# yosungho/LineTR

Measured on AMD Instinct MI355X. Metric: line_descriptors_per_sec, higher is better.
Workload: dtype f32 in/out; GEMMs as 6 bf16-split MFMA products, fp32 accumulate (fp32-faithful); 1 GPU; cfg3: 64 pairs/GPU of 640x480, 200 lines/image -> 199 sub-lines x 21 tokens, d_model=256, seeded weights; pairs_per_gpu=64, collective=none

## Files before the change

### include/linetr_hip.h

```cpp
#ifndef LINETR_HIP_H
#define LINETR_HIP_H

#include <stdint.h>

#ifdef __cplusplus
extern "C" {
#endif

#define LINETR_ABI_VERSION 6

enum {
  LINETR_OK = 0,
  LINETR_E_ARG = -1,
  LINETR_E_HIP = -2,
  LINETR_E_WEIGHTS = -3,
  LINETR_E_ASSERT = -4,
  LINETR_E_WORKSPACE = -5,
  LINETR_E_CAPACITY = -6
};

typedef struct LinetrHandle LinetrHandle;

typedef struct {
  int32_t d_model;
// ... 256 lines not shown
                                int32_t Kin, float* d_dW, float* d_db, void* d_workspace, int64_t workspace_bytes, void* stream);

int64_t linetr_token_assemble_backward_workspace_bytes(int64_t L);
int linetr_token_assemble_forward(LinetrHandle* h, const float* d_desc, const float* d_pos, const float* d_cls, int64_t L, int32_t S,
                                  float* d_x, void* stream);
int linetr_token_assemble_backward(LinetrHandle* h, const float* d_dx, int64_t L, int32_t S, float* d_dtok, float* d_dcls,
                                   void* d_workspace, int64_t workspace_bytes, void* stream);


enum { LINETR_COORD_F32 = 0, LINETR_COORD_F64 = 1 };
int64_t linetr_gt_assign_workspace_bytes(int32_t B, int32_t n0, int32_t n1);
int linetr_gt_assign(LinetrHandle* h, int32_t coord_type, const void* d_lines0, int32_t n0, const void* d_lines1, int32_t n1,
                     const double* d_H, int32_t B, const int32_t* d_count0, const int32_t* d_count1, double thres_reprojected,
                     double thres_angdiff, double min_overlap_ratio, int32_t pad, float* d_assign, int32_t* d_lmatches, int32_t M,
                     int32_t* d_found, uint8_t* d_match_dir, void* d_overlap_dir, void* d_proj0, void* d_proj1, void* d_workspace,
                     int64_t workspace_bytes, void* stream);


int linetr_make_pseudo_lines(uint64_t seed, int32_t image_index, int32_t n, double shape0, double shape1, double min_length,
                             double* h_lines);

int linetr_find_line_attributes(const double* h_lines, int32_t n, double min_length, int32_t max_sublines, double* h_klines,
                                double* h_length, double* h_angles, int32_t* n_out);

int64_t linetr_fixed_size_workspace_bytes(int32_t n_images, int32_t height, int32_t width, int32_t dense_is_nhwc);
int linetr_fixed_size(LinetrHandle* h, const LinetrLineRec* d_recs, const int32_t* h_cu_k, const int32_t* h_cu_n,
                      const LinetrLineRec* d_pseudo, const LinetrLineRec* h_pseudo, const int32_t* h_cu_p, int32_t n_images,
                      int32_t max_sublines, int32_t max_tokens, double token_distance, const float* d_dense_desc,
                      const float* d_dense_score, int32_t height, int32_t width, int32_t clip_height, int32_t clip_width,
                      int32_t pseudo_clip_height, int32_t pseudo_clip_width, int32_t align_corners, int32_t dense_is_nhwc,
                      LinetrTokens out, int32_t* d_num_klns, int32_t* d_num_slns, void* d_workspace, int64_t workspace_bytes,
                      void* stream);


typedef struct {
  float* p;
  const float* g;
  float* m;
  float* v;
  int64_t n;
  float step_size;
  float bc2_sqrt;
} LinetrAdamTensor;
typedef struct {
  double beta1, beta2, eps, weight_decay, lr;
  int32_t decoupled;
} LinetrAdamHyper;

int64_t linetr_adam_workspace_bytes(int32_t n_tensors, int64_t n_total);
int linetr_adam_step(LinetrHandle* h, const LinetrAdamTensor* h_table, int32_t n_tensors, const LinetrAdamHyper* hyper,
                     const float* d_grad_scale, void* d_workspace, int64_t workspace_bytes, void* stream);

int64_t linetr_grad_norm_workspace_bytes(int32_t n_tensors, int64_t n_total);
int linetr_grad_norm(LinetrHandle* h, const LinetrAdamTensor* h_table, int32_t n_tensors, double max_norm, double* d_norm,
                     float* d_scale, void* d_workspace, int64_t workspace_bytes, void* stream);


int linetr_superpoint_heads(LinetrHandle* h, const float* d_score_logits, const float* d_desc_raw, int32_t B,
                            int32_t Hc, int32_t Wc, float* d_dense_score, float* d_dense_desc_nhwc,
                            float* d_dense_desc_nchw, void* stream);


int64_t linetr_superpoint_keypoints_workspace_bytes(int32_t B, int32_t H, int32_t W, int32_t cap_per_image);
int linetr_superpoint_keypoints(LinetrHandle* h, const float* d_dense_score, int32_t B, int32_t H, int32_t W, int32_t nms_radius,
                                float keypoint_threshold, int32_t remove_borders, int32_t max_keypoints, int32_t cap_per_image,
                                float* d_keypoints, float* d_scores, int32_t* d_cu_kp, int32_t* d_found, void* d_workspace,
                                int64_t workspace_bytes, void* stream);

int64_t linetr_point_descriptors_workspace_bytes(int32_t B, int32_t Hc, int32_t Wc, int32_t dense_is_nhwc);
int linetr_point_descriptors(LinetrHandle* h, const float* d_keypoints, const int32_t* d_cu_kp, int32_t B, int64_t n_total,
                             const float* d_dense_desc, int32_t Hc, int32_t Wc, int32_t align_corners, int32_t dense_is_nhwc,
                             float* d_desc_cn, void* d_workspace, int64_t workspace_bytes, void* stream);

int linetr_superpoint_heads_rows(LinetrHandle* h, const float* d_score_rows, int64_t ld_score, const float* d_desc_rows, int64_t ld_desc,
                                 int32_t B, int32_t Hc, int32_t Wc, float* d_dense_score, float* d_dense_desc_nhwc,
                                 float* d_dense_desc_nchw, void* stream);


int linetr_warp_images(LinetrHandle* h, const float* d_src, int32_t B, int32_t C, int32_t H, int32_t W, const double* h_mat, int32_t mode,
                       float* d_dst, uint8_t* d_valid, void* stream);
int linetr_warp_tile(int32_t* tile_h, int32_t* tile_w, int32_t* erode_tile_h, int32_t* erode_tile_w);

int linetr_mask_erode(LinetrHandle* h, const uint8_t* d_mask, int32_t B, int32_t H, int32_t W, int32_t radius, uint8_t* d_out, void* stream);


typedef struct LinetrDetectConfig {
  int32_t n_octaves;
  int32_t scale;
  int32_t grad_threshold;
  int32_t min_region_size;
  double density;
} LinetrDetectConfig;

int64_t linetr_detect_lines_workspace_bytes(int32_t B, int32_t H, int32_t W, int32_t n_octaves);
int linetr_detect_lines(LinetrHandle* h, const void* d_images, int32_t images_are_float, int32_t B, int32_t H, int32_t W,
                        const LinetrDetectConfig* cfg, int32_t capacity, double* d_rows, int32_t* h_counts, int64_t* d_debug_regions,
                        void* d_workspace, int64_t workspace_bytes, void* stream);
int linetr_detect_tile(int32_t* tile_h, int32_t* tile_w);

int64_t linetr_detect_debug_labels_workspace_bytes(int32_t B, int32_t H, int32_t W);
int linetr_detect_debug_labels(LinetrHandle* h, const int8_t* d_buckets, int32_t B, int32_t H, int32_t W, int32_t* d_labels, void* d_workspace,
                               int64_t workspace_bytes, void* stream);
int linetr_detect_debug_gradient(LinetrHandle* h, const void* d_images, int32_t images_are_float, int32_t B, int32_t H, int32_t W,
                                 const LinetrDetectConfig* cfg, int32_t octave, int32_t* d_m2, int8_t* d_bucket_a, int8_t* d_bucket_b,
                                 void* d_workspace, int64_t workspace_bytes, void* stream);


int linetr_sp_conv3x3_tile(int32_t* tile_h, int32_t* tile_w);
int64_t linetr_sp_conv3x3_pack_bytes(int32_t Cin, int32_t Cout);
int linetr_sp_conv3x3_pack(const float* d_w, int32_t Cin, int32_t Cout, float* d_packed, void* stream);
int linetr_sp_conv3x3(LinetrHandle* h, const float* d_x, int32_t B, int32_t H, int32_t W, int32_t Cin, const float* d_packed_w,
                      const float* d_bias, int32_t Cout, int32_t pool, float* d_y, void* stream);
int linetr_sp_conv1a(LinetrHandle* h, const float* d_image, int32_t B, int32_t H, int32_t W, const float* d_w, const float* d_bias,
                     float* d_y, void* stream);

#define LINETR_SP_SCORE_LD 68
typedef struct LinetrSpEncoder LinetrSpEncoder;
int linetr_sp_encoder_create(int32_t device, LinetrSpEncoder** out);
void linetr_sp_encoder_destroy(LinetrSpEncoder* enc);
int linetr_sp_encoder_set_weights(LinetrSpEncoder* enc, const float* const* d_weights, const float* const* d_biases, void* stream);
int64_t linetr_sp_encoder_workspace_bytes(int32_t B, int32_t H, int32_t W);
int linetr_sp_encoder_forward(LinetrSpEncoder* enc, const float* d_image, int32_t B, int32_t H, int32_t W, float* d_score_rows,
                              float* d_desc_rows, float* d_feat, void* d_workspace, int64_t workspace_bytes, void* stream);


enum { LINETR_PREC_F32 = 0, LINETR_PREC_BF16X3 = 1, LINETR_PREC_BF16X6 = 2, LINETR_PREC_F16X3 = 3 };
int linetr_set_precision(LinetrHandle* h, int32_t mode);
int linetr_get_precision(const LinetrHandle* h);


int linetr_debug_posenc(LinetrHandle* h, int32_t which, const float* d_in0, const float* d_in1, const float* d_in2,
                           int64_t rows, float* d_out, void* stream);

int linetr_debug_gemm(LinetrHandle* h, const float* d_A, int32_t lda, const float* d_W, const float* d_bias,
                      const float* d_residual, float* d_Y, int32_t ldy, int32_t M, int32_t N, int32_t K,
                      int32_t act, int32_t cache_weights, void* stream);

#define LINETR_GEMM_TILE_WS 100
typedef struct {
  const float* A;   int32_t lda;
  const float* A2;  int32_t lda2;  int32_t K1;
  const float* W;
  const float* bias;
  const float* R;
  float* Y;         int32_t ldy;
  int32_t M, N, K, act;
  int32_t groups;   int64_t gA, gY;
  int32_t norm;     const float* gamma;  const float* beta;  const float* add2;  float eps;
  int32_t via_row_norm;
  int32_t tile;
} LinetrGemmCase;
int linetr_debug_gemm_case(LinetrHandle* h, const LinetrGemmCase* c, int32_t* tile_used, void* stream);

int linetr_debug_sig_attention(LinetrHandle* h, int32_t kernel, int32_t layer, const float* d_in, int32_t ld_in,
                               const int32_t* h_cu_sub, int32_t n_images, float* d_msg, int32_t* kernel_used, void* stream);

int linetr_debug_tok_mlp(LinetrHandle* h, int32_t variant, const float* d_pnt, const float* d_score, int64_t rows_word,
                         const float* d_sublines, const float* d_resp, const float* d_angle, int64_t rows_line,
                         float* d_out_word, float* d_out_line, int32_t max_blocks, int32_t* variant_used, void* stream);

int64_t linetr_debug_bn_train_workspace_bytes(const LinetrHandle* h, int32_t which, int64_t rows);
int linetr_debug_bn_train(LinetrHandle* h, int32_t which, float* d_z, int64_t rows, int32_t C, int32_t ld, const float* d_gamma,
                          const float* d_beta, const float* d_in0, const float* d_in1, const float* d_in2, float* d_out,
                          float momentum, float* d_running, float* d_batch, float* d_affine, int32_t* nb_used, void* d_ws,
                          int64_t ws_bytes, void* stream);

int linetr_debug_cls_pool(LinetrHandle* h, int32_t kernel, const LinetrLineRec* d_recs, int32_t K, const int32_t* d_sub2line,
                          int32_t N, int32_t T, const float* d_cpnt, const float* d_a4, int64_t first_pad, int32_t n_images,
                          const float* d_map, int32_t dense_is_nhwc, int32_t Hc, int32_t Wc, int32_t align_corners,
                          const float* d_desc_dense, float* d_pooled, int32_t* kernel_used, void* stream);

int linetr_debug_match(LinetrHandle* h, int32_t P, const int32_t* dims, const float* d_desc0, const int64_t* off_n0,
                       const int32_t* d_s2l0, const float* d_desc1, const int64_t* off_n1, const int32_t* d_s2l1, float thr,
                       int32_t mutual, float* d_dk, const int64_t* off_dk, int32_t* d_match01, const int64_t* off_k0, void* d_ws,
                       int64_t ws_bytes, int32_t path, int32_t seg1_global, int32_t cache_dk, int32_t device_table,
                       int32_t* path_used, void* stream);

enum { LINETR_STAGE_TAIL = 0, LINETR_STAGE_SIG = 1, LINETR_STAGE_FOLD_NEXT = 8 };
int64_t linetr_debug_stage_workspace_bytes(const LinetrHandle* h, int32_t N, int32_t n_images);
int linetr_debug_stage(LinetrHandle* h, int32_t stage, int32_t N, const float* d_in0, const float* d_in1, const int32_t* h_cu_sub,
                       int32_t n_images, int32_t plan, float* d_out0, float* d_out1, float* d_out2, int32_t* plan_used, void* d_ws,
                       int64_t ws_bytes, void* stream);

#ifdef LINETR_EXPERIMENTS
int64_t linetr_st_bytes(int64_t rows, int32_t K);
int linetr_debug_to_st(LinetrHandle* h, const float* d_X, int32_t ld, int32_t rows, int32_t K, void* d_st, void* stream);
int linetr_debug_from_st(LinetrHandle* h, const void* d_st, int32_t rows, int32_t K, float* d_X, int32_t ld, void* stream);
int linetr_debug_gemm_st(LinetrHandle* h, const void* d_A1, int32_t K1, const void* d_A2, int32_t K2, const void* d_W,
                         const float* d_bias, const void* d_R, void* d_Yst, float* d_Y, int32_t ldy, int32_t M, int32_t N,
                         int32_t act, void* stream);
int linetr_debug_pairnet_stamps(LinetrHandle* h, unsigned long long* d_buf);
#endif

int linetr_allgather_desc(void* nccl_comm, const void* d_slab, void* d_out, int64_t slab_bytes, void* stream);

int linetr_set_allgather_fn(void* nccl_allgather_fn);

int linetr_pack_slab(const float* d_line_desc, int32_t N, const int32_t* d_cu_n, const int32_t* d_cu_k, int32_t n_images,
                     const int32_t* d_sub2line, int32_t n_images_cap, int32_t rows_cap, int32_t zero_tail, float* d_slab,
                     void* stream);


typedef struct {
  const char* name;
  int32_t calls;
  float ms;
  double flops;
  double bytes;
} LinetrProfileEntry;
int linetr_set_profiling(LinetrHandle* h, int32_t on);
int linetr_get_profile(LinetrHandle* h, LinetrProfileEntry* out, int32_t max_entries, int32_t* n_out);

#ifdef __cplusplus
}
#endif
#endif
```

### linetr_amd/_native.py

```python
from __future__ import annotations

import ctypes as C
import os

import numpy as np

_HERE = os.path.dirname(os.path.abspath(__file__))
LIB_PATH = os.path.join(_HERE, "csrc", "liblinetr_hip.so")
EXPERIMENTS_LIB_PATH = os.path.join(os.path.dirname(_HERE), "experiments", "liblinetr_hip_experiments.so")

E_ARG, E_ASSERT, E_WORKSPACE = -1, -4, -5


class ModelConfig(C.Structure):
    _fields_ = [("d_model", C.c_int32), ("n_heads", C.c_int32), ("d_inner", C.c_int32),
                ("n_sig_layers", C.c_int32), ("n_desc_layers", C.c_int32), ("enc_channels", C.c_int32 * 4),
                ("norm_height", C.c_int32), ("norm_width", C.c_int32), ("bn_batch_stats", C.c_int32)]


class LineRec(C.Structure):
    _fields_ = [("sp", C.c_double * 2), ("ep", C.c_double * 2), ("length", C.c_double),
                ("angle", C.c_double * 2), ("first_sub", C.c_int32), ("n_tok", C.c_int32),
                ("n_sub", C.c_int32), ("image", C.c_int32), ("line_local", C.c_int32), ("first_tok", C.c_int32)]

# ... 29 lines not shown
            raise ValueError(f"dropout seed {seed} / call {call}: a 64-bit seed and a 32-bit call index")
        return cls(int(seed), int(call), int(p * 4294967296.0), 1.0 / (1.0 - p))


ADAM_TENSOR_DTYPE = np.dtype([("p", "<u8"), ("g", "<u8"), ("m", "<u8"), ("v", "<u8"), ("n", "<i8"), ("step_size", "<f4"), ("bc2_sqrt", "<f4")])
assert ADAM_TENSOR_DTYPE.itemsize == 48


def adam_bias_corrections(lr: float, beta1: float, beta2: float, step: float):
    step = float(step)
    return float(lr) / (1.0 - float(beta1) ** step), (1.0 - float(beta2) ** step) ** 0.5


class AdamHyper(C.Structure):
    _fields_ = [("beta1", C.c_double), ("beta2", C.c_double), ("eps", C.c_double), ("weight_decay", C.c_double), ("lr", C.c_double),
                ("decoupled", C.c_int32)]


class DetectConfig(C.Structure):
    _fields_ = [("n_octaves", C.c_int32), ("scale", C.c_int32), ("grad_threshold", C.c_int32), ("min_region_size", C.c_int32),
                ("density", C.c_double)]


class ProfileEntry(C.Structure):
    _fields_ = [("name", C.c_char_p), ("calls", C.c_int32), ("ms", C.c_float), ("flops", C.c_double),
                ("bytes", C.c_double)]


vp, i32, i64, f64, f32 = C.c_void_p, C.c_int32, C.c_int64, C.c_double, C.c_float
_P = C.POINTER

ABI = {
    "linetr_abi_version": (i32, []),
    "linetr_last_error": (C.c_char_p, []),
    "linetr_create": (i32, [_P(ModelConfig), i32, _P(C.c_char_p), _P(vp), _P(i64), i32, _P(vp)]),
    "linetr_destroy": (None, [vp]),
    "linetr_prefilter": (i32, [vp, i32, i32, i32, i32, f64, i32, vp, f64, i32, i32, i32, i32, vp, i32, _P(i32), _P(i32)]),
    "linetr_prefilter_batch": (i32, [vp, vp, i32, i32, i32, i32, f64, i32, vp, f64, i32, i32, vp, i32, vp, vp]),
    "linetr_prefilter_tied_images": (i32, [vp, i32]),
    "linetr_pack_lines": (i32, [vp, vp, vp, i32, f64, i32, i32, i32, i32, vp, _P(i32)]),
    "linetr_tokenize_workspace_bytes": (i64, [i32, i32, i32, i32]),
    "linetr_tokenize": (i32, [vp, vp, i32, i32, f64, i32, vp, vp, i32, i32, i32, i32, i32, i32, i32, Tokens, vp, vp, i64, vp]),
    "linetr_sample_descriptors_workspace_bytes": (i64, [i32, i32, i32]),
    "linetr_sample_descriptors": (i32, [vp, vp, i64, vp, i32, i32, i32, i32, vp, vp, i64, vp]),
    "linetr_forward_workspace_bytes": (i64, [vp, i32, i32]),
    "linetr_forward": (i32, [vp, _P(Tokens), vp, vp, i32, i32, vp, vp, i64, vp]),
    "linetr_bn_stats_floats": (i64, [vp]),
    "linetr_forward_train_workspace_bytes": (i64, [vp, i32, i32]),
    "linetr_forward_train": (i32, [vp, _P(Tokens), vp, vp, i32, i32, f32, vp, vp, vp, vp, i64, vp]),
    "linetr_describe_workspace_bytes": (i64, [vp, i32, i32, i32, i32, i64]),
    "linetr_describe": (i32, [vp, vp, i32, i32, i64, vp, vp, i32, f64, i32, vp, vp, i32, i32, i32, i32, Tokens, vp, vp, vp, i64, vp]),
    "linetr_describe_submit": (i32, [vp, vp, i32, i32, i64, vp, vp, i32, f64, i32, vp, vp, i32, i32, i32, i32, Tokens, vp, vp, vp, i64, i32,
                                     i32, vp]),
    "linetr_pipeline_max_slots": (i32, []),
    "linetr_describe_join": (i32, [vp, i32, vp]),
    "linetr_match_workspace_bytes": (i64, [i32, i64, i64, i64]),
    "linetr_match": (i32, [vp, i32, vp, vp, vp, vp, vp, vp, vp, f32, i32, vp, vp, vp, vp, vp, i64, vp]),
    "linetr_match_gathered": (i32, [vp, i32, vp, vp, vp, vp, vp, vp, vp, vp, vp, f32, i32, vp, vp, vp, vp, vp, i64, vp]),
    "linetr_match_distmat_workspace_bytes": (i64, [i32, i32]),
    "linetr_match_distmat": (i32, [vp, vp, i32, i32, f32, i32, vp, vp, i64, vp]),
    "linetr_match_distmat_f64_workspace_bytes": (i64, [i32, i32]),
    "linetr_match_distmat_f64": (i32, [vp, vp, i32, i32, f64, i32, vp, vp, i64, vp]),
    "linetr_pool_distmat_workspace_bytes": (i64, [i32, i32]),
    "linetr_pool_distmat": (i32, [vp, vp, i32, i32, vp, i32, vp, i32, vp, vp, i64, vp]),
    "linetr_pool_distmat_dense_workspace_bytes": (i64, [i32, i32, i32, i32]),
    "linetr_pool_distmat_dense": (i32, [vp, vp, i32, i32, vp, i32, vp, i32, vp, vp, i64, vp]),
    "linetr_match_points_workspace_bytes": (i64, [i32, i32]),
    "linetr_match_points": (i32, [vp, vp, i32, vp, i32, f32, i32, vp, vp, vp, i64, vp]),
    "linetr_pair_tail_workspace_bytes": (i64, [i32, i32, i32, i32, i32, i32]),
    "linetr_pair_tail_output_bytes": (i64, [i32, i32, i32, i32, vp]),
    "linetr_pair_tail": (i32, [vp, vp, i32, vp, i32, f32, vp, i32, vp, i32, vp, i32, vp, i32, f32, i32, vp, i64, vp, i64, vp]),
    "linetr_val_step_workspace_bytes": (i64, [i32, i32]),
    "linetr_val_step_output_bytes": (i64, [i32, vp]),
    "linetr_val_step": (i32, [vp, vp, i32, vp, i32, vp, i32, f64, i32, vp, vp, vp, vp, i64, vp, i64, vp]),
    "linetr_assign_from_matches": (i32, [vp, vp, i32, i32, i32, vp, vp]),
    "linetr_desc_loss_grad_workspace_bytes": (i64, [i32, i32]),
    "linetr_desc_loss_grad": (i32, [vp, vp, i32, vp, i32, vp, i32, vp, vp, vp, vp, i64, vp, i64, vp]),
    "linetr_linear_backward_chunk_rows": (i32, []),
    "linetr_linear_backward_workspace_bytes": (i64, [i64, i32, i32]),
    "linetr_linear_forward": (i32, [vp, vp, i64, vp, vp, i64, i32, i32, i32, vp, i64, vp]),
    "linetr_linear_backward": (i32, [vp, vp, i64, vp, vp, i64, vp, i64, i32, i32, vp, vp, vp, vp, i64, vp]),
    "linetr_head_backward_workspace_bytes": (i64, [i64]),
    "linetr_head_forward": (i32, [vp, vp, vp, vp, i64, vp, vp]),
    "linetr_head_backward": (i32, [vp, vp, vp, vp, vp, i64, vp, vp, vp, vp, i64, vp]),
    "linetr_sig_attention_backward_workspace_bytes": (i64, [i64]),
    "linetr_sig_attention_forward": (i32, [vp, vp, i64, vp, i64, vp, i64, vp, i32, i64, vp, i64, vp, vp]),
    "linetr_sig_attention_backward": (i32, [vp, vp, i64, vp, i64, vp, i64, vp, i64, vp, vp, i64, vp, i32, i64, vp, i64, vp, i64, vp, i64, vp, i64,
                                            vp]),
    "linetr_bn_forward_workspace_bytes": (i64, [i64, i32]),
    "linetr_bn_forward": (i32, [vp, vp, i64, i64, i32, vp, vp, f32, f32, vp, i32, i32, vp, i64, vp, vp, i64, vp]),
    "linetr_bn_backward_workspace_bytes": (i64, [i64, i32]),
    "linetr_bn_backward": (i32, [vp, vp, i64, vp, i64, vp, i64, vp, vp, i64, i32, i32, vp, i64, vp, vp, vp, i64, vp]),
    "linetr_cls_pool_train_forward": (i32, [vp, vp, i64, vp, i64, i64, i32, vp, vp, vp]),
    "linetr_cls_pool_train_backward": (i32, [vp, vp, i64, vp, i64, vp, vp, vp, i64, i32, vp, i64, vp, i64, vp]),
    "linetr_layer_norm_backward_workspace_bytes": (i64, [i64, i32]),
    "linetr_layer_norm_forward": (i32, [vp, vp, i64, vp, i64, vp, vp, f32, i64, i32, vp, i64, vp, vp]),
    "linetr_layer_norm_backward": (i32, [vp, vp, i64, vp, i64, vp, vp, vp, i64, i64, i32, vp, i64, vp, vp, vp, i64, vp]),
    "linetr_cls_pool_dropout_forward": (i32, [vp, vp, i64, vp, i64, i64, i32, _P(Dropout), vp, vp, vp, vp]),
    "linetr_cls_pool_dropout_backward": (i32, [vp, vp, i64, vp, i64, vp, vp, vp, vp, vp, i64, i32, _P(Dropout), vp, i64, vp, i64, vp]),
    "linetr_layer_norm_dropout_forward": (i32, [vp, vp, i64, vp, i64, vp, vp, f32, i64, i32, _P(Dropout), i32, vp, i64, vp, vp]),
    "linetr_layer_norm_dropout_backward": (i32, [vp, vp, i64, vp, i64, vp, vp, vp, i64, i64, i32, _P(Dropout), i32, vp, i64, vp, i64, vp, vp, vp,
                                                 i64, vp]),
    "linetr_dropout_factors": (i32, [vp, _P(Dropout), i32, i64, i64, vp, vp]),
    "linetr_gelu_forward": (i32, [vp, vp, i64, i64, i32, vp, i64, vp]),
    "linetr_gelu_backward": (i32, [vp, vp, i64, vp, i64, i64, i32, vp, i64, vp]),
    "linetr_input_layer_chunk_rows": (i32, []),
    "linetr_input_layer_backward_workspace_bytes": (i64, [i64, i32, i32]),
    "linetr_input_layer_forward": (i32, [vp, vp, i64, vp, vp, i64, i32, i32, vp, i64, vp]),
    "linetr_input_layer_backward": (i32, [vp, vp, i64, vp, i64, i64, i32, i32, vp, vp, vp, i64, vp]),
    "linetr_token_assemble_backward_workspace_bytes": (i64, [i64]),
    "linetr_token_assemble_forward": (i32, [vp, vp, vp, vp, i64, i32, vp, vp]),
    "linetr_token_assemble_backward": (i32, [vp, vp, i64, i32, vp, vp, vp, i64, vp]),
    "linetr_gt_assign_workspace_bytes": (i64, [i32, i32, i32]),
    "linetr_gt_assign": (i32, [vp, i32, vp, i32, vp, i32, vp, i32, vp, vp, f64, f64, f64, i32, vp, vp, i32, vp, vp, vp, vp, vp, vp, i64, vp]),
    "linetr_make_pseudo_lines": (i32, [C.c_uint64, i32, i32, f64, f64, f64, vp]),
    "linetr_find_line_attributes": (i32, [vp, i32, f64, i32, vp, vp, vp, _P(i32)]),
    "linetr_fixed_size_workspace_bytes": (i64, [i32, i32, i32, i32]),
    "linetr_fixed_size": (i32, [vp, vp, vp, vp, vp, vp, vp, i32, i32, i32, f64, vp, vp, i32, i32, i32, i32, i32, i32, i32, i32, Tokens, vp, vp,
                                vp, i64, vp]),
    "linetr_adam_workspace_bytes": (i64, [i32, i64]),
    "linetr_adam_step": (i32, [vp, vp, i32, _P(AdamHyper), vp, vp, i64, vp]),
    "linetr_grad_norm_workspace_bytes": (i64, [i32, i64]),
    "linetr_grad_norm": (i32, [vp, vp, i32, f64, vp, vp, vp, i64, vp]),
    "linetr_superpoint_heads": (i32, [vp, vp, vp, i32, i32, i32, vp, vp, vp, vp]),
    "linetr_superpoint_keypoints_workspace_bytes": (i64, [i32, i32, i32, i32]),
    "linetr_superpoint_keypoints": (i32, [vp, vp, i32, i32, i32, i32, f32, i32, i32, i32, vp, vp, vp, vp, vp, i64, vp]),
    "linetr_point_descriptors_workspace_bytes": (i64, [i32, i32, i32, i32]),
    "linetr_point_descriptors": (i32, [vp, vp, vp, i32, i64, vp, i32, i32, i32, i32, vp, vp, i64, vp]),
    "linetr_superpoint_heads_rows": (i32, [vp, vp, i64, vp, i64, i32, i32, i32, vp, vp, vp, vp]),
    "linetr_warp_images": (i32, [vp, vp, i32, i32, i32, i32, vp, i32, vp, vp, vp]),
    "linetr_warp_tile": (i32, [_P(i32), _P(i32), _P(i32), _P(i32)]),
    "linetr_mask_erode": (i32, [vp, vp, i32, i32, i32, i32, vp, vp]),
    "linetr_detect_lines_workspace_bytes": (i64, [i32, i32, i32, i32]),
    "linetr_detect_lines": (i32, [vp, vp, i32, i32, i32, i32, _P(DetectConfig), i32, vp, vp, vp, vp, i64, vp]),
    "linetr_detect_tile": (i32, [_P(i32), _P(i32)]),
    "linetr_detect_debug_labels_workspace_bytes": (i64, [i32, i32, i32]),
    "linetr_detect_debug_labels": (i32, [vp, vp, i32, i32, i32, vp, vp, i64, vp]),
    "linetr_detect_debug_gradient": (i32, [vp, vp, i32, i32, i32, i32, _P(DetectConfig), i32, vp, vp, vp, vp, i64, vp]),
    "linetr_sp_conv3x3_tile": (i32, [_P(i32), _P(i32)]),
    "linetr_sp_conv3x3_pack_bytes": (i64, [i32, i32]),
    "linetr_sp_conv3x3_pack": (i32, [vp, i32, i32, vp, vp]),
    "linetr_sp_conv3x3": (i32, [vp, vp, i32, i32, i32, i32, vp, vp, i32, i32, vp, vp]),
    "linetr_sp_conv1a": (i32, [vp, vp, i32, i32, i32, vp, vp, vp, vp]),
    "linetr_sp_encoder_create": (i32, [i32, _P(vp)]),
    "linetr_sp_encoder_destroy": (None, [vp]),
    "linetr_sp_encoder_set_weights": (i32, [vp, _P(vp), _P(vp), vp]),
    "linetr_sp_encoder_workspace_bytes": (i64, [i32, i32, i32]),
    "linetr_sp_encoder_forward": (i32, [vp, vp, i32, i32, i32, vp, vp, vp, vp, i64, vp]),
    "linetr_set_precision": (i32, [vp, i32]),
    "linetr_get_precision": (i32, [vp]),
    "linetr_debug_posenc": (i32, [vp, i32, vp, vp, vp, i64, vp, vp]),
    "linetr_debug_gemm": (i32, [vp, vp, i32, vp, vp, vp, vp, i32, i32, i32, i32, i32, i32, vp]),
    "linetr_debug_gemm_case": (i32, [vp, _P(GemmCase), vp, vp]),
    "linetr_debug_sig_attention": (i32, [vp, i32, i32, vp, i32, vp, i32, vp, vp, vp]),
    "linetr_debug_tok_mlp": (i32, [vp, i32, vp, vp, i64, vp, vp, vp, i64, vp, vp, i32, vp, vp]),
    "linetr_debug_bn_train_workspace_bytes": (i64, [vp, i32, i64]),
    "linetr_debug_bn_train": (i32, [vp, i32, vp, i64, i32, i32, vp, vp, vp, vp, vp, vp, f32, vp, vp, vp, vp, vp, i64, vp]),
    "linetr_debug_cls_pool": (i32, [vp, i32, vp, i32, vp, i32, i32, vp, vp, i64, i32, vp, i32, i32, i32, i32, vp, vp, vp, vp]),
    "linetr_debug_match": (i32, [vp, i32, vp, vp, vp, vp, vp, vp, vp, f32, i32, vp, vp, vp, vp, vp, i64, i32, i32, i32, i32, vp, vp]),
    "linetr_debug_stage_workspace_bytes": (i64, [vp, i32, i32]),
    "linetr_debug_stage": (i32, [vp, i32, i32, vp, vp, vp, i32, i32, vp, vp, vp, vp, vp, i64, vp]),
    "linetr_allgather_desc": (i32, [vp, vp, vp, i64, vp]),
    "linetr_set_allgather_fn": (i32, [vp]),
    "linetr_pack_slab": (i32, [vp, i32, vp, vp, i32, vp, i32, i32, i32, vp, vp]),
    "linetr_set_profiling": (i32, [vp, i32]),
    "linetr_get_profile": (i32, [vp, _P(ProfileEntry), i32, _P(i32)]),
}
EXPERIMENT_ABI = {
    "linetr_st_bytes": (i64, [i64, i32]),
    "linetr_debug_to_st": (i32, [vp, vp, i32, i32, i32, vp, vp]),
    "linetr_debug_from_st": (i32, [vp, vp, i32, i32, vp, i32, vp]),
    "linetr_debug_gemm_st": (i32, [vp, vp, i32, vp, i32, vp, vp, vp, vp, vp, i32, i32, i32, i32, vp]),
    "linetr_debug_pairnet_stamps": (i32, [vp, vp]),
}
EXPORTS = list(ABI)
EXPERIMENT_EXPORTS = list(EXPERIMENT_ABI)

_libs = {}


def lib(path=None):
    import torch
    path = os.path.abspath(path or os.environ.get("LINETR_LIB", LIB_PATH))
    if path in _libs:
        return _libs[path]
    if not os.path.exists(path):
        raise RuntimeError(
            f"{path} is missing: the HIP extension has not been built (run `python -m linetr_amd.build`). "
            "linetr_amd has no CPU fallback.")
    L = C.CDLL(path)
    table = {**ABI, **EXPERIMENT_ABI} if hasattr(L, "linetr_debug_gemm_st") else ABI
    for name, (restype, argtypes) in table.items():
        fn = getattr(L, name)
        fn.restype, fn.argtypes = restype, argtypes
    if L.linetr_abi_version() != 6:
        raise RuntimeError("liblinetr_hip.so ABI version mismatch")
    _libs[path] = L
    return L


class NativeError(RuntimeError):
    pass


def check(code: int, L=None):
    if code == 0:
        return
    msg = (L if L is not None else lib()).linetr_last_error().decode("utf-8", "replace")
    if code == E_ASSERT:
        raise AssertionError(msg)
    raise NativeError(f"liblinetr_hip error {code}: {msg}")


def np_ptr(a: np.ndarray):
    return a.ctypes.data_as(C.c_void_p)
```

### linetr_amd/csrc/linetr_core.hip

```cpp
#include <dlfcn.h>

#include <algorithm>
#include <condition_variable>
#include <functional>
#include <numeric>
#include <thread>

#include "lt_handle.h"

using namespace lt;

namespace {

class WorkPool {
 public:
  static WorkPool& get() {
    static WorkPool* p = new WorkPool();
    return *p;
  }
  int size() const { return n_workers_ + 1; }
  void run(int n, const std::function<void(int)>& fn) {
    if (n <= 0) return;
    if (n == 1 || n_workers_ == 0) { for (int i = 0; i < n; ++i) fn(i); return; }
    std::lock_guard<std::mutex> region(region_);
// ... 18 lines not shown
  }
  void drain() {
    for (;;) {
      int i;
      const std::function<void(int)>* f;
      {
        std::lock_guard<std::mutex> lk(m_);
        if (!job_ || next_ >= n_jobs_) return;
        i = next_++;
        f = job_;
      }
      (*f)(i);
      std::lock_guard<std::mutex> lk(m_);
      if (--pending_ == 0) cv_done_.notify_all();
    }
  }
  void loop() {
    uint64_t seen = 0;
    for (;;) {
      {
        std::unique_lock<std::mutex> lk(m_);
        cv_work_.wait(lk, [&] { return gen_ != seen; });
        seen = gen_;
      }
      drain();
    }
  }
  std::mutex m_, region_;
  std::condition_variable cv_work_, cv_done_;
  const std::function<void(int)>* job_ = nullptr;
  int n_jobs_ = 0, next_ = 0, pending_ = 0, n_workers_ = 0;
  uint64_t gen_ = 0;
};


struct TensorMap {
  std::map<std::string, std::pair<const float*, int64_t>> t;
  const float* get(const std::string& k, int64_t numel, int& err) const {
    auto it = t.find(k);
    if (it == t.end() || it->second.first == nullptr) {
      err = fail(LINETR_E_WEIGHTS, "state_dict tensor '%s' missing", k.c_str());
      return nullptr;
    }
    if (it->second.second != numel) {
      err = fail(LINETR_E_WEIGHTS, "state_dict tensor '%s' has %lld elements, expected %lld", k.c_str(),
                 (long long)it->second.second, (long long)numel);
      return nullptr;
    }
    return it->second.first;
  }
};

struct Arena {
  std::vector<float> host;
  size_t put(const std::vector<double>& v) {
    size_t off = (host.size() + 63) / 64 * 64;
    host.resize(off + v.size());
    for (size_t i = 0; i < v.size(); ++i) host[off + i] = (float)v[i];
    return off;
  }
};

void fold_bn(const float* W, const float* b, const float* g, const float* beta, const float* mean,
             const float* var, int out, int in, std::vector<double>& Wf, std::vector<double>& bf) {
  Wf.resize((size_t)out * in);
  bf.resize(out);
  for (int o = 0; o < out; ++o) {
    const double s = (double)g[o] / std::sqrt((double)var[o] + 1e-5);
    for (int i = 0; i < in; ++i) Wf[(size_t)o * in + i] = (double)W[(size_t)o * in + i] * s;
    bf[o] = ((double)b[o] - (double)mean[o]) * s + (double)beta[o];
  }
}

std::vector<double> to_d(const float* p, size_t n) { return std::vector<double>(p, p + n); }

}


extern "C" int linetr_abi_version(void) { return LINETR_ABI_VERSION; }
extern "C" const char* linetr_last_error(void) { return g_err.c_str(); }

extern "C" int linetr_create(const LinetrModelConfig* cfg, int32_t n_tensors, const char* const* names,
                             const float* const* h_data, const int64_t* numel, int32_t device,
                             LinetrHandle** out) {
  if (!cfg || !out || !names || !h_data || !numel) return fail(LINETR_E_ARG, "null argument");
  if (cfg->d_model != D || cfg->n_heads != HEADS)
    return fail(LINETR_E_ARG, "only descriptor_dim=256 / n_heads=4 are supported");
  if (cfg->d_inner % 128 != 0 || cfg->n_sig_layers < 0 || cfg->n_desc_layers < 1)
    return fail(LINETR_E_ARG, "bad d_inner / layer counts");
  const int e0 = cfg->enc_channels[0], e1 = cfg->enc_channels[1], e2 = cfg->enc_channels[2], e3 = cfg->enc_channels[3];
  if (e0 != 32 || e1 % 64 || e2 % 64 || e3 % 64 || e3 != D)
    return fail(LINETR_E_ARG, "keyline_encoder must be [32, 64k, 64k, 256] (got %d,%d,%d,%d)", e0, e1, e2, e3);
  int ndev = 0;
  LT_HIP(hipGetDeviceCount(&ndev));
  if (ndev <= 0 || device >= ndev) return fail(LINETR_E_HIP, "no usable HIP device (count=%d)", ndev);
  LT_HIP(hipSetDevice(device));

  TensorMap tm;
  for (int i = 0; i < n_tensors; ++i) tm.t[names[i]] = {h_data[i], numel[i]};
  int err = 0;
  Arena ar;
  auto H = std::make_unique<LinetrHandle>();
  H->cfg = *cfg;
  H->device = device;
  struct Fix { const float** dst; size_t off; };
  std::vector<Fix> fix;
  auto place = [&](const float** dst, const std::vector<double>& v) { fix.push_back({dst, ar.put(v)}); };
  std::vector<GemmWSpec> gemm_w;
  auto place_w = [&](GemmW* dst, const std::vector<double>& W, const std::vector<double>& b, int rows, int K, bool st = false) {
    place(&dst->W, W);
    place(&dst->b, b);
    dst->rows = rows; dst->K = K;
    gemm_w.push_back({dst, st});
  };

  int bn_slot = 0;
  if (cfg->bn_batch_stats) {
    if (std::max(std::max(e0, e1), std::max(std::max(e2, e3), 2 * D)) > lt::BN_MAX_CHANNELS)
      return fail(LINETR_E_ARG, "create: a training-mode handle (bn_batch_stats = 1) takes keyline_encoder widths up to %d (got %d, %d, %d, %d)",
                  lt::BN_MAX_CHANNELS, e0, e1, e2, e3);
    H->bn_g.reserve(8 + cfg->n_sig_layers); H->bn_b.reserve(8 + cfg->n_sig_layers); H->bn_c.reserve(8 + cfg->n_sig_layers);
  }
  const int ch_w[6] = {3, e0, e1, e2, e3, D}, ch_l[6] = {5, e0, e1, e2, e3, D};
  std::vector<double> W5w, b5w;
  for (int enc = 0; enc < 2; ++enc) {
    const std::string pre = enc == 0 ? "klenc.word_position_enc.encoder." : "klenc.line_position_enc.encoder.";
    const int* ch = enc == 0 ? ch_w : ch_l;
    PosEncoder& E = H->enc[enc];
    GemmW* const Wdst[4] = {nullptr, &E.W2, &E.W3, &E.W4};
    for (int i = 0; i < 4; ++i) {
      const std::string c = pre + std::to_string(3 * i), bn = pre + std::to_string(3 * i + 1);
      const float* W = tm.get(c + ".weight", (int64_t)ch[i + 1] * ch[i], err);
      const float* b = tm.get(c + ".bias", ch[i + 1], err);
      const float* g = tm.get(bn + ".weight", ch[i + 1], err);
      const float* be = tm.get(bn + ".bias", ch[i + 1], err);
      const float* mu = tm.get(bn + ".running_mean", ch[i + 1], err);
      const float* va = tm.get(bn + ".running_var", ch[i + 1], err);
      if (err) return err;
      std::vector<double> Wf, bf;
      if (cfg->bn_batch_stats) {
        Wf = to_d(W, (size_t)ch[i + 1] * ch[i]); bf = to_d(b, ch[i + 1]);
        H->bn_g.push_back(nullptr); H->bn_b.push_back(nullptr); H->bn_c.push_back(ch[i + 1]);
        place(&H->bn_g[bn_slot], to_d(g, ch[i + 1])); place(&H->bn_b[bn_slot], to_d(be, ch[i + 1]));
        ++bn_slot;
      } else
      fold_bn(W, b, g, be, mu, va, ch[i + 1], ch[i], Wf, bf);
      if (i == 0) { place(&E.W1, Wf); place(&E.b1, bf); }
      else place_w(Wdst[i], Wf, bf, ch[i + 1], ch[i], true);
    }
    const float* W = tm.get(pre + "12.weight", (int64_t)D * e3, err);
    const float* b = tm.get(pre + "12.bias", D, err);
    if (err) return err;
    if (enc == 0) { W5w = to_d(W, (size_t)D * D); b5w = to_d(b, D); }
    else place_w(&H->lW5, to_d(W, (size_t)D * D), to_d(b, D), D, e3);
  }

  {
    const std::string p = "klenc.desc_layers." + std::to_string(cfg->n_desc_layers - 1) + ".";
    const float* cls = tm.get("klenc.cls_token", D, err);
    const float* Wq = tm.get(p + "slf_attn.w_qs.weight", D * D, err);
    const float* bq = tm.get(p + "slf_attn.w_qs.bias", D, err);
    const float* Wk = tm.get(p + "slf_attn.w_ks.weight", D * D, err);
    const float* bk = tm.get(p + "slf_attn.w_ks.bias", D, err);
    const float* Wv = tm.get(p + "slf_attn.w_vs.weight", D * D, err);
    const float* bv = tm.get(p + "slf_attn.w_vs.bias", D, err);
    const float* Wfc = tm.get(p + "slf_attn.fc.weight", D * D, err);
    const float* bfc = tm.get(p + "slf_attn.fc.bias", D, err);
    const float* g1 = tm.get(p + "slf_attn.layer_norm.weight", D, err);
    const float* b1 = tm.get(p + "slf_attn.layer_norm.bias", D, err);
    const int DI = cfg->d_inner;
    const float* W1 = tm.get(p + "pos_ffn.w_1.weight", (int64_t)DI * D, err);
    const float* bb1 = tm.get(p + "pos_ffn.w_1.bias", DI, err);
    const float* W2 = tm.get(p + "pos_ffn.w_2.weight", (int64_t)D * DI, err);
    const float* bb2 = tm.get(p + "pos_ffn.w_2.bias", D, err);
    const float* g2 = tm.get(p + "pos_ffn.layer_norm.weight", D, err);
    const float* b2 = tm.get(p + "pos_ffn.layer_norm.bias", D, err);
    if (err) return err;
    std::vector<double> q(D);
    for (int o = 0; o < D; ++o) {
      double s = bq[o];
      for (int i = 0; i < D; ++i) s += (double)Wq[o * D + i] * cls[i];
      q[o] = s / 8.0;
    }
    std::vector<double> U(HEADS * D, 0.0), U2(HEADS * D, 0.0);
    for (int h = 0; h < HEADS; ++h) {
      double c = 0.0;
      for (int d = 0; d < DH; ++d) {
        const int o = h * DH + d;
        c += q[o] * bk[o];
        for (int i = 0; i < D; ++i) U[h * D + i] += q[o] * Wk[o * D + i];
      }
      for (int i = 0; i < D; ++i) {
        double s = 0.0;
        for (int o = 0; o < D; ++o) s += W5w[(size_t)o * D + i] * U[h * D + o];
        U2[h * D + i] = s;
      }
      double ub5 = 0.0, ucls = 0.0;
      for (int i = 0; i < D; ++i) { ub5 += U[h * D + i] * b5w[i]; ucls += U[h * D + i] * cls[i]; }
      H->pool.c_tok[h] = (float)(ub5 + c);
      H->pool.s_cls[h] = (float)(ucls + c);
    }
    place(&H->pool.U, U);
    place(&H->pool.U2, U2);
    std::vector<double> Watt((size_t)HEADS * DH * POOLW, 0.0), batt(HEADS * DH);
    for (int h = 0; h < HEADS; ++h)
      for (int d = 0; d < DH; ++d) {
        const int o = h * DH + d;
        double* row = &Watt[((size_t)h * DH + d) * POOLW];
        double r = 0.0, bb = bv[o];
        for (int i = 0; i < D; ++i) {
          row[i] = Wv[o * D + i];
          r += (double)Wv[o * D + i] * ((double)cls[i] - b5w[i]);
          bb += (double)Wv[o * D + i] * b5w[i];
        }
        for (int i = 0; i < D; ++i) {
          double s = 0.0;
          for (int m = 0; m < D; ++m) s += (double)Wv[o * D + m] * W5w[(size_t)m * D + i];
          row[D + i] = s;
        }
        row[2 * D] = r;
        batt[o] = bb;
      }
    place_w(&H->Watt, Watt, batt, HEADS * DH, POOLW);
    std::vector<double> bfc2(D);
    for (int i = 0; i < D; ++i) bfc2[i] = (double)bfc[i] + cls[i];
    place_w(&H->Wfc, to_d(Wfc, D * D), bfc2, D, D);
    place(&H->ln1g, to_d(g1, D)); place(&H->ln1b, to_d(b1, D));
    place_w(&H->Wf1, to_d(W1, (size_t)DI * D), to_d(bb1, DI), DI, D);
    place_w(&H->Wf2, to_d(W2, (size_t)D * DI), to_d(bb2, D), D, DI);
    place(&H->ln2g, to_d(g2, D)); place(&H->ln2b, to_d(b2, D));
  }

  H->sig.resize(cfg->n_sig_layers);
  std::vector<std::vector<double>> sig_qkv_d, sig_bqkv_d, sig_w2_d, sig_b2_d;
  for (int l = 0; l < cfg->n_sig_layers; ++l) {
    const std::string p = "selfattn.layers." + std::to_string(l) + ".";
    const float* Wp[3];
    const float* bp[3];
    for (int j = 0; j < 3; ++j) {
      Wp[j] = tm.get(p + "attn.proj." + std::to_string(j) + ".weight", D * D, err);
      bp[j] = tm.get(p + "attn.proj." + std::to_string(j) + ".bias", D, err);
    }
    const float* Wm = tm.get(p + "attn.merge.weight", D * D, err);
    const float* bm = tm.get(p + "attn.merge.bias", D, err);
    const float* W1 = tm.get(p + "mlp.0.weight", 4 * D * D, err);
    const float* b1 = tm.get(p + "mlp.0.bias", 2 * D, err);
    const float* g = tm.get(p + "mlp.1.weight", 2 * D, err);
    const float* be = tm.get(p + "mlp.1.bias", 2 * D, err);
    const float* mu = tm.get(p + "mlp.1.running_mean", 2 * D, err);
    const float* va = tm.get(p + "mlp.1.running_var", 2 * D, err);
    const float* W2 = tm.get(p + "mlp.3.weight", 2 * D * D, err);
    const float* b2 = tm.get(p + "mlp.3.bias", D, err);
    if (err) return err;
    std::vector<double> Wqkv((size_t)3 * D * D), bqkv(3 * D);
    for (int j = 0; j < 3; ++j)
      for (int h = 0; h < HEADS; ++h)
        for (int d = 0; d < DH; ++d) {
          const int src = d * HEADS + h, dst = j * D + h * DH + d;
          const double sc = j == 0 ? 0.125 : 1.0;
          for (int i = 0; i < D; ++i) Wqkv[(size_t)dst * D + i] = (double)Wp[j][src * D + i] * sc;
          bqkv[dst] = (double)bp[j][src] * sc;
        }
    std::vector<double> Wm2((size_t)D * D);
    for (int o = 0; o < D; ++o)
      for (int h = 0; h < HEADS; ++h)
        for (int d = 0; d < DH; ++d) Wm2[(size_t)o * D + h * DH + d] = Wm[o * D + d * HEADS + h];
    std::vector<double> W1f, b1f;
    if (cfg->bn_batch_stats) {
      W1f = to_d(W1, (size_t)4 * D * D); b1f = to_d(b1, 2 * D);
      H->bn_g.push_back(nullptr); H->bn_b.push_back(nullptr); H->bn_c.push_back(2 * D);
      place(&H->bn_g[bn_slot], to_d(g, 2 * D)); place(&H->bn_b[bn_slot], to_d(be, 2 * D));
      ++bn_slot;
    } else
    fold_bn(W1, b1, g, be, mu, va, 2 * D, 2 * D, W1f, b1f);
    std::vector<double> W1m((size_t)2 * D * 2 * D);
    for (int o = 0; o < 2 * D; ++o) {
      const double* w1b = &W1f[(size_t)o * 2 * D + D];
      for (int i = 0; i < D; ++i) W1m[(size_t)o * 2 * D + i] = W1f[(size_t)o * 2 * D + i];
      for (int i = 0; i < D; ++i) {
        double sacc = 0.0;
        for (int m = 0; m < D; ++m) sacc += w1b[m] * Wm2[(size_t)m * D + i];
        W1m[(size_t)o * 2 * D + D + i] = sacc;
      }
      double bacc = b1f[o];
      for (int m = 0; m < D; ++m) bacc += w1b[m] * (double)bm[m];
      b1f[o] = bacc;
    }
    SigLayer& S = H->sig[l];
    sig_qkv_d.push_back(Wqkv); sig_bqkv_d.push_back(bqkv);
    sig_w2_d.push_back(to_d(W2, (size_t)2 * D * D)); sig_b2_d.push_back(to_d(b2, D));
    place_w(&S.Wqkv, Wqkv, bqkv, 3 * D, D, true);
    place_w(&S.W1, W1m, b1f, 2 * D, 2 * D);
    place_w(&S.W2, to_d(W2, (size_t)2 * D * D), to_d(b2, D), D, 2 * D);
  }
  for (int l = 0; l + 1 < cfg->n_sig_layers; ++l) {
    const std::vector<double>&W2 = sig_w2_d[l], &b2 = sig_b2_d[l], &Wq = sig_qkv_d[l + 1], &bq = sig_bqkv_d[l + 1];
    std::vector<double> Wn((size_t)4 * D * 3 * D, 0.0), bn(4 * D);
    for (int o = 0; o < D; ++o) {
      Wn[(size_t)o * 3 * D + o] = 1.0;
      for (int j = 0; j < 2 * D; ++j) Wn[(size_t)o * 3 * D + D + j] = W2[(size_t)o * 2 * D + j];
      bn[o] = b2[o];
    }
    for (int r = 0; r < 3 * D; ++r) {
      double* row = &Wn[(size_t)(D + r) * 3 * D];
      const double* wq = &Wq[(size_t)r * D];
      for (int i = 0; i < D; ++i) row[i] = wq[i];
      double bacc = bq[r];
      for (int m2 = 0; m2 < D; ++m2) {
        const double a = wq[m2];
        const double* w2r = &W2[(size_t)m2 * 2 * D];
        for (int j = 0; j < 2 * D; ++j) row[D + j] += a * w2r[j];
        bacc += a * b2[m2];
      }
      bn[D + r] = bacc;
    }
    place_w(&H->sig[l].Wnext, Wn, bn, 4 * D, 3 * D);
  }
  {
    const float* W = tm.get("final_proj.weight", D * D, err);
    const float* b = tm.get("final_proj.bias", D, err);
    if (err) return err;
    place_w(&H->Wfin, to_d(W, D * D), to_d(b, D), D, D);
    if (cfg->n_sig_layers > 0) {
      const std::string p = "selfattn.layers." + std::to_string(cfg->n_sig_layers - 1) + ".";
      const float* W2 = tm.get(p + "mlp.3.weight", 2 * D * D, err);
      const float* b2 = tm.get(p + "mlp.3.bias", D, err);
      if (err) return err;
      std::vector<double> Wf((size_t)D * 3 * D), bf(D);
      for (int o = 0; o < D; ++o) {
        for (int i = 0; i < D; ++i) Wf[(size_t)o * 3 * D + i] = W[o * D + i];
        for (int j = 0; j < 2 * D; ++j) {
          double sacc = 0.0;
          for (int m = 0; m < D; ++m) sacc += (double)W[o * D + m] * (double)W2[(size_t)m * 2 * D + j];
          Wf[(size_t)o * 3 * D + D + j] = sacc;
        }
        double bacc = b[o];
        for (int m = 0; m < D; ++m) bacc += (double)W[o * D + m] * (double)b2[m];
        bf[o] = bacc;
      }
      place_w(&H->Wfin2, Wf, bf, D, 3 * D);
    }
  }

  LT_HIP(hipMalloc((void**)&H->arena, ar.host.size() * sizeof(float)));
  LT_HIP(hipMemcpy(H->arena, ar.host.data(), ar.host.size() * sizeof(float), hipMemcpyHostToDevice));
  for (auto& f : fix) *f.dst = H->arena + f.off;
  if (int e = make_split_copies(H.get(), gemm_w)) return e;
  if (const char* e = getenv("LINETR_PRECISION")) {
    if (!strcmp(e, "f32")) H->precision = LINETR_PREC_F32;
    else if (!strcmp(e, "bf16x3")) H->precision = LINETR_PREC_BF16X3;
    else if (!strcmp(e, "bf16x6")) H->precision = LINETR_PREC_BF16X6;
    else if (!strcmp(e, "f16x3")) H->precision = LINETR_PREC_F16X3;
    else return fail(LINETR_E_ARG, "LINETR_PRECISION must be f32, bf16x3, bf16x6 or f16x3 (got '%s')", e);
  }
  *out = H.release();
  return LINETR_OK;
}

extern "C" int linetr_set_precision(LinetrHandle* h, int32_t mode) {
  if (!h || mode < LINETR_PREC_F32 || mode > LINETR_PREC_F16X3) return fail(LINETR_E_ARG, "bad precision mode");
  h->precision = mode;
  return LINETR_OK;
}
extern "C" int linetr_get_precision(const LinetrHandle* h) { return h ? h->precision : LINETR_E_ARG; }

extern "C" void linetr_destroy(LinetrHandle* h) {
  if (!h) return;
  (void)hipSetDevice(h->device);
  for (auto& p : h->pending) { (void)hipEventDestroy(p.a); (void)hipEventDestroy(p.b); }
  for (auto e : h->event_pool) (void)hipEventDestroy(e);
  for (hipStream_t x : h->pipe.stream)
    if (x) { (void)hipStreamSynchronize(x); (void)hipStreamDestroy(x); }
  for (int s = 0; s < LinetrHandle::PIPE_SLOTS; ++s) {
    for (hipEvent_t e : {h->pipe.fork[s], h->pipe.done[s]})
      if (e) (void)hipEventDestroy(e);
    for (hipEvent_t e : h->pipe.cut[s])
      if (e) (void)hipEventDestroy(e);
  }
  if (h->arena) (void)hipFree(h->arena);
  if (h->split_arena) (void)hipFree(h->split_arena);
  if (h->zeros) (void)hipFree(h->zeros);
  if (h->w2p_arena) (void)hipFree(h->w2p_arena);
  if (h->sk_ws) (void)hipFree(h->sk_ws);
  if (h->sk_flags) (void)hipFree(h->sk_flags);
  if (h->pn_abort) (void)hipHostFree(h->pn_abort);
  for (auto& kv : h->debug_split) (void)hipFree(kv.second);
  delete h;
}


static int pack_one(LinetrLineRec& r, double td, int T, int image, int line_local, int& sub_cursor, int& tok_cursor) {
  if (!(td > 0) || T < 1) return fail(LINETR_E_ARG, "token_distance must be > 0 and max_tokens >= 1");
  const double nt = std::ceil(r.length / td);
  if (!(nt >= 1) || nt > 1e7) return fail(LINETR_E_ARG, "key-line %d has a non-positive / absurd token count", line_local);
  r.n_tok = (int)nt;
  r.n_sub = (r.n_tok + T - 1) / T;
  r.first_sub = sub_cursor;
  r.image = image;
  r.line_local = line_local;
  r.first_tok = tok_cursor;
  sub_cursor += r.n_sub;
  tok_cursor += r.n_tok;
  if (r.n_tok >= 2) {
    const double dx = r.ep[0] - r.sp[0], dy = r.ep[1] - r.sp[1];
    const double geo = std::sqrt(dx * dx + dy * dy);
    if (!(geo >= (double)(r.n_tok - 2) * td))
      return fail(LINETR_E_ASSERT, "distance should be smaller than line length! (key-line %d)", line_local);
  }
  return 0;
}

static void angle_of(LinetrLineRec& r) {
  double th = std::atan2(r.ep[0] - r.sp[0], r.ep[1] - r.sp[1]);
  if (th < 0) th += M_PI;
#ifdef __GLIBC__
  ::sincos(2 * th, &r.angle[1], &r.angle[0]);
#else
  r.angle[0] = std::cos(2 * th);
  r.angle[1] = std::sin(2 * th);
#endif
}

extern "C" int linetr_pack_lines(const double* h_klines, const double* h_length, const double* h_angles, int32_t K,
                                 double td, int32_t T, int32_t image_index, int32_t sub_base, int32_t tok_base,
                                 LinetrLineRec* h_recs, int32_t* n_out) {
  if (K < 0 || (K > 0 && (!h_klines || !h_length || !h_angles || !h_recs))) return fail(LINETR_E_ARG, "null argument");
  int cur = sub_base, tcur = tok_base;
  for (int k = 0; k < K; ++k) {
    LinetrLineRec& r = h_recs[k];
    r.sp[0] = h_klines[k * 4 + 0]; r.sp[1] = h_klines[k * 4 + 1];
    r.ep[0] = h_klines[k * 4 + 2]; r.ep[1] = h_klines[k * 4 + 3];
    r.length = h_length[k];
    r.angle[0] = h_angles[k * 2]; r.angle[1] = h_angles[k * 2 + 1];
    if (int e = pack_one(r, td, T, image_index, k, cur, tcur)) return e;
  }
  if (n_out) *n_out = cur - sub_base;
  return LINETR_OK;
}


struct KeptLineAttr { double sp[2], ep[2], length; };
static double philox_u01(uint32_t hi, uint32_t lo) { return ((double)(hi >> 5) * 67108864.0 + (double)(lo >> 6)) / 9007199254740992.0; }

extern "C" int linetr_make_pseudo_lines(uint64_t seed, int32_t image_index, int32_t n, double shape0, double shape1, double min_length,
                                        double* h_lines) {
#pragma clang fp contract(off)
  constexpr double MASK = 15.0, MAX_RAND = 160.0;
  constexpr int MAX_ATTEMPTS = 64;
  if (n < 0 || (n > 0 && !h_lines) || image_index < 0 || seed >> 32) return fail(LINETR_E_ARG, "make_pseudo_lines: bad argument (a 32-bit seed, n >= 0)");
  if (!(min_length > 0) || !(min_length < MAX_RAND) || !(shape0 - MASK >= MASK + 2 * min_length) || !(shape1 - MASK >= MASK + 2 * min_length))
    return fail(LINETR_E_ARG, "make_pseudo_lines: image_shape (%g, %g) has no room for lines of min_length %g", shape0, shape1, min_length);
  const double area0 = shape0 - min_length - MASK, area1 = shape1 - min_length - MASK;
  for (int i = 0; i < n; ++i) {
    double* l = h_lines + (size_t)i * 4;
    int attempt = 0;
    for (; attempt < MAX_ATTEMPTS; ++attempt) {
      uint32_t a[4], b[4];
      philox4x32_10((uint32_t)i, (uint32_t)attempt, 0u, 0u, (uint32_t)seed, (uint32_t)image_index, a);
      philox4x32_10((uint32_t)i, (uint32_t)attempt, 1u, 0u, (uint32_t)seed, (uint32_t)image_index, b);
      const double sx = area0 * philox_u01(a[0], a[1]), sy = area1 * philox_u01(a[2], a[3]);
      const double ang = 2 * M_PI * philox_u01(b[0], b[1]);
      const double len = (MAX_RAND - min_length) * philox_u01(b[2], b[3]) + min_length;
      const double ex = sx + len * std::cos(ang), ey = sy + len * std::sin(ang);
      l[0] = std::min(std::max(sx, MASK), shape0 - MASK);
      l[1] = std::min(std::max(sy, MASK), shape1 - MASK);
      l[2] = std::min(std::max(ex, MASK), shape0 - MASK);
      l[3] = std::min(std::max(ey, MASK), shape1 - MASK);
      const double dx = l[2] - l[0], dy = l[3] - l[1];
      const double length = std::sqrt(dx * dx + dy * dy);
      if (attempt == 0 ? !(length < min_length) : length > min_length) break;
    }
    if (attempt == MAX_ATTEMPTS) {
      l[0] = MASK; l[1] = MASK; l[2] = MASK + 2 * min_length; l[3] = MASK;
    }
  }
  return LINETR_OK;
}

extern "C" int linetr_find_line_attributes(const double* h_lines, int32_t n, double min_length, int32_t max_sublines, double* h_klines,
                                           double* h_length, double* h_angles, int32_t* n_out) {
#pragma clang fp contract(off)
  if (n < 0 || (n > 0 && (!h_lines || !h_klines || !h_length || !h_angles)) || !n_out) return fail(LINETR_E_ARG, "find_line_attributes: null argument");
  std::vector<KeptLineAttr> keep;
  keep.reserve(n);
  for (int i = 0; i < n; ++i) {
    const double* l = h_lines + (size_t)i * 4;
    KeptLineAttr r;
    if (l[0] < l[2]) { r.sp[0] = l[0]; r.sp[1] = l[1]; r.ep[0] = l[2]; r.ep[1] = l[3]; }
    else { r.sp[0] = l[2]; r.sp[1] = l[3]; r.ep[0] = l[0]; r.ep[1] = l[1]; }
    const double dx = r.ep[0] - r.sp[0], dy = r.ep[1] - r.sp[1];
    r.length = std::sqrt(dx * dx + dy * dy);
    if (r.length < min_length) continue;
    keep.push_back(r);
// ... 232 lines not shown
```

### linetr_amd/csrc/linetr_net.hip

```cpp
#include <algorithm>
#include <array>
#include <numeric>
#include <set>

#include "lt_handle.h"
#include "lt_gemm.h"
#include "lt_gemm_split.h"
#include "lt_gemm_split16.h"
#include "lt_st_image.h"
#include "lt_gemm_small.h"
#include "lt_model.h"
#include "lt_attn.h"
#include "lt_attn_fused.h"
#include "lt_gemm_ws.h"
#include "lt_tokmlp.h"
#include "lt_token.h"
#include "lt_bntrain.h"

using namespace lt;

namespace {

const char* gemm_class_name(int precision, int tile, const GemmArgs& g, int groups) {
  static const auto names = [] {
    const char* kind[4] = {"gemm_f32", "gemm_bf16x3", "gemm_bf16x6", "gemm_f16x3"};
    std::array<std::array<std::string, (int)SplitTile::count>, 4> n;
    for (int p = 0; p < 4; ++p)
      for (int t = 0; t < (p ? (int)SplitTile::count : (int)F32Tile::count); ++t)
        n[p][t] = std::string(kind[p]) + "_" + (p ? tile_name((SplitTile)t) : tile_name((F32Tile)t));
    return n;
  }();
  const std::string& name = names[precision][tile];
  static const bool by_shape = LT_XENV("LINETR_PROFILE_SHAPES") != nullptr;
  if (!by_shape) return name.c_str();
  static std::mutex mu;
  static std::set<std::string> shapes;
  char buf[160];
  snprintf(buf, sizeof buf, "%s[M=%d,N=%d,K=%d,g=%d]", name.c_str(), g.M, g.N, g.K, groups);
  std::lock_guard<std::mutex> lock(mu);
  return shapes.insert(buf).first->c_str();
}

struct GemmA { const float* p; int ld; const float* p2 = nullptr; int ld2 = 0, K1 = 0; };
struct GemmY { float* p; int ld; };
struct GemmGroups { int n, N; int64_t gA, gY; };

struct NormSpec {
  int mode = 0;
  const float* gamma = nullptr;
  const float* beta = nullptr;
  const float* add2 = nullptr;
  float eps = 0.f;
};

#ifdef LINETR_EXPERIMENTS
int x_gemm(LinetrHandle*, hipStream_t, SplitGemmArgs& sa, const GemmW& w, int groups, const NormSpec*, double fl, double by, bool& done);
int x_split_weights(LinetrHandle* H, std::vector<GemmWSpec>& weights);
int64_t x_ws_bytes(const LinetrHandle* h, int N);
#endif

int gemm_args(const GemmW& w, int M, const GemmA& A, const GemmY& Y, int act, const float* R, const GemmGroups* grp,
              const NormSpec* ns, GemmArgs& g) {
  const int groups = grp ? grp->n : 1, N = grp ? grp->N : w.rows;
  if (A.p2 && (A.K1 <= 0 || A.K1 >= w.K)) return fail(LINETR_E_ARG, "gemm: split point K1 = %d outside (0, K = %d)", A.K1, w.K);
  if ((int64_t)N * groups > w.rows) return fail(LINETR_E_ARG, "gemm: %d groups of %d rows exceed the weight's %d", groups, N, w.rows);
  if (groups > 1 && (R || ns)) return fail(LINETR_E_ARG, "gemm: a grouped launch takes no residual and no row normalisation");
  g = GemmArgs{};
  g.A = A.p; g.lda = A.ld; g.A2 = A.p2; g.lda2 = A.ld2; g.K1 = A.K1;
  g.W = w.W; g.ldw = w.K; g.bias = w.b; g.R = R; g.ldr = Y.ld; g.Y = Y.p; g.ldy = Y.ld;
  g.M = M; g.N = N; g.K = w.K; g.act = act;
  if (grp) { g.gA = grp->gA; g.gW = (int64_t)N * w.K; g.gBias = N; g.gY = grp->gY; }
  if (ns) { g.norm = ns->mode; g.gamma = ns->gamma; g.beta = ns->beta; g.add2 = ns->add2; g.ldadd2 = D; g.eps = ns->eps; }
  return LINETR_OK;
}

bool gemm_ws_able(const LinetrHandle* h, const GemmArgs& g, const GemmW& w, int groups, const NormSpec* fused_norm) {
  return h->precision == LINETR_PREC_BF16X6 && groups == 1 && !g.A2 && !g.R && !fused_norm && w.st &&
         gemm_ws_can(g.N, g.K, g.lda, g.ldy, g.act);
}
bool gemm_ws_takes(const LinetrHandle* h, const GemmArgs& g, const GemmW& w, int groups, const NormSpec* fused_norm) {
  return gemm_ws_able(h, g, w, groups, fused_norm) && gemm_ws_fits(g.M, g.N, g.K, g.lda, g.ldy, g.act) && !LT_XENV("LINETR_NO_GEMM_WS");
}

struct GemmForce { int tile = -1; int* used = nullptr; bool launch = true; };

int run_gemm(LinetrHandle* h, hipStream_t st, const GemmW& w, int M, const GemmA& A, const GemmY& Y, int act, const float* R = nullptr,
             const GemmGroups* grp = nullptr, const NormSpec* fused_norm = nullptr, const GemmForce* force = nullptr) {
  GemmArgs g;
  if (int e = gemm_args(w, M, A, Y, act, R, grp, fused_norm, g)) return e;
  const int groups = grp ? grp->n : 1;
  const int forced = force ? force->tile : -1;
  const bool launch = !force || force->launch;
  auto report = [&](int tile) { if (force && force->used) *force->used = tile; };
  const double fl = 2.0 * M * (double)g.N * g.K * groups;
  const double by = 4.0 * groups * ((double)M * g.K + (double)g.N * g.K + (double)M * g.N);
  if (h->precision == LINETR_PREC_F32) {
    if (forced >= (int)F32Tile::count) return fail(LINETR_E_ARG, "gemm: the f32 mode has no tile %d", forced);
    if (fused_norm) return fail(LINETR_E_ARG, "gemm: the f32 kernels have no fused row normalisation");
    const F32Tile tile = f32_tile_launched(g, forced < 0 ? f32_tile(g, groups) : (F32Tile)forced);
    report((int)tile);
    if (!launch) return LINETR_OK;
    ProfScope ps(h, st, gemm_class_name(LINETR_PREC_F32, (int)tile, g, groups), fl, by);
    return gemm_launch(g, groups, tile, st);
  }
  SplitGemmArgs sa;
  sa.g = g;
#ifdef LINETR_EXPERIMENTS
  if (!force) {
    bool done = false;
    if (int e = x_gemm(h, st, sa, w, groups, fused_norm, fl, by, done); e || done) return e;
  }
#endif
  if (forced == LINETR_GEMM_TILE_WS && !gemm_ws_able(h, g, w, groups, fused_norm))
    return fail(LINETR_E_ARG, "gemm: the weight-stationary kernel runs act(A[M,128] W[256,128]^T + b) in bf16x6 only, act none / ReLU");
  if (forced == LINETR_GEMM_TILE_WS || (forced < 0 && gemm_ws_takes(h, g, w, groups, fused_norm))) {
    report(LINETR_GEMM_TILE_WS);
    if (!launch) return LINETR_OK;
    WsGemmArgs a;
    a.A = A.p; a.lda = A.ld; a.Wst = w.st; a.bias = w.b ? w.b : h->zeros; a.Y = Y.p; a.ldy = Y.ld; a.M = M; a.act = act;
    ProfScope ps(h, st, "gemm_bf16x6_ws64x256", fl, by);
    return gemm_ws_launch(a, st);
  }
  const int pl = h->precision == LINETR_PREC_BF16X6 ? 3 : 2;
  SplitTile tile;
  if (forced >= (int)SplitTile::count) return fail(LINETR_E_ARG, "gemm: no split tile %d", forced);
  if (forced >= 0) tile = (SplitTile)forced;
  else if (int e = pick_split_tile(g, groups, pl, tile)) return e;
  if (int e = split_tile_launched(g, groups, pl, tile)) return e;
  report((int)tile);
  if (!launch) return LINETR_OK;
  ProfScope ps(h, st, gemm_class_name(h->precision, (int)tile, g, groups), fl, by);
  switch (h->precision) {
    case LINETR_PREC_BF16X3: sa.Wsp = w.s2; sa.gWsp = g.gW * 4; return gemm_split_launch<2>(sa, groups, tile, st);
    case LINETR_PREC_F16X3: sa.Wsp = w.h2; sa.gWsp = g.gW * 4; return gemm_split_launch<2, 1>(sa, groups, tile, st);
    default: sa.Wsp = w.s3; sa.gWsp = g.gW * 6; return gemm_split_launch<3>(sa, groups, tile, st);
  }
}

bool gemm_norm_fuses(const LinetrHandle* h, const GemmW& w, int M, const GemmA& A, const float* R, float* Y) {
  GemmArgs g;
  return !LT_XENV("LINETR_NO_FUSED_NORM") && h->precision != LINETR_PREC_F32 && !LT_XENV("LINETR_GEMM_TILE") &&
         !gemm_args(w, M, A, {Y, D}, ACT_NONE, R, nullptr, nullptr, g) &&
         split_tile(g, 1, h->precision == LINETR_PREC_BF16X6 ? 3 : 2) == SplitTile::t128x256;
}

int row_norm(LinetrHandle* h, hipStream_t st, const float* x, int M, const NormSpec& ns, float* Y) {
  ProfScope ps(h, st, "row_norm", 0, (double)M * D * (ns.add2 ? 12 : 8));
  hipLaunchKernelGGL(row_norm_kernel, dim3(cdiv(M, 4)), dim3(256), 0, st, x, M, ns.mode == 2 ? 1 : 0, ns.gamma, ns.beta,
                     ns.add2, ns.eps, Y);
  LT_LAUNCH_CHECK();
  return 0;
}

int run_gemm_norm(LinetrHandle* h, hipStream_t st, const GemmW& w, int M, const GemmA& A, const float* R, float* tmp, float* Y,
                  const NormSpec& ns) {
  if (w.rows != D) return fail(LINETR_E_ARG, "gemm_norm: the weight has %d rows, not %d", w.rows, D);
  if (gemm_norm_fuses(h, w, M, A, R, Y)) return run_gemm(h, st, w, M, A, {Y, D}, ACT_NONE, R, nullptr, &ns);
  if (int e = run_gemm(h, st, w, M, A, {tmp, D}, ACT_NONE, R)) return e;
  return row_norm(h, st, tmp, M, ns, Y);
}

struct SplitOffsets { int64_t s2, s3, h2, st = -1; };
SplitOffsets split_offsets(int64_t rows, int K, bool with_st, int64_t& off) {
  SplitOffsets o;
  o.s2 = off; off += align_up(rows * K * 4, 256);
  o.s3 = off; off += align_up(rows * K * 6, 256);
  o.h2 = off; off += align_up(rows * K * 4, 256);
  if (with_st) { off = align_up(off, 1024); o.st = off; off += st_bytes(rows, K); }
  return o;
}

void split_copies(GemmW& w, unsigned char* base, const SplitOffsets& o, bool make, hipStream_t st) {
  w.s2 = base + o.s2; w.s3 = base + o.s3; w.h2 = base + o.h2;
  w.st = o.st >= 0 ? base + o.st : nullptr;
  if (!make) return;
  const dim3 grid((unsigned)cdiv((int)((int64_t)w.rows * w.K / 4), 256));
  hipLaunchKernelGGL(split_rows_kernel<2>, grid, dim3(256), 0, st, w.W, base + o.s2, (int64_t)w.rows, w.K);
  hipLaunchKernelGGL(split_rows_kernel<3>, grid, dim3(256), 0, st, w.W, base + o.s3, (int64_t)w.rows, w.K);
  hipLaunchKernelGGL((split_rows_kernel<2, 1>), grid, dim3(256), 0, st, w.W, base + o.h2, (int64_t)w.rows, w.K);
  if (o.st >= 0) {
    const int64_t thr = st_row_blocks(w.rows) * (w.K / 16) * 32;
    hipLaunchKernelGGL(to_st_kernel, dim3((unsigned)((thr + 255) / 256)), dim3(256), 0, st, w.W, w.K, w.rows, w.K / 16, base + o.st);
  }
}

}

int lt::make_split_copies(LinetrHandle* H, std::vector<GemmWSpec> weights) {
#ifdef LINETR_EXPERIMENTS
  if (int e = x_split_weights(H, weights)) return e;
#endif
  int64_t total = 0;
  std::vector<SplitOffsets> at;
  for (auto& s : weights) at.push_back(split_offsets(s.w->rows, s.w->K, s.st && s.w->rows % 16 == 0 && s.w->K % 32 == 0, total));
  LT_HIP(hipMalloc((void**)&H->split_arena, total));
  LT_HIP(hipMalloc((void**)&H->zeros, 4096 * sizeof(float)));
  LT_HIP(hipMemset(H->zeros, 0, 4096 * sizeof(float)));
  for (size_t i = 0; i < weights.size(); ++i) split_copies(*weights[i].w, H->split_arena, at[i], true, 0);
  LT_LAUNCH_CHECK();
  LT_HIP(hipDeviceSynchronize());
  return LINETR_OK;
}


namespace {
int k2s_table(const LinetrTokens& out, int n_images, int K, int N, const int32_t* h_cu_sub, K2sTable& tab, const char* who) {
  tab = K2sTable{};
  if (!out.mat) return 0;
  if (n_images > K2S_MAX_IMAGES) return fail(LINETR_E_ARG, "%s: mat_klines2sublines is written for calls of up to %d images", who, K2S_MAX_IMAGES);
  if (n_images == 1) {
    for (int i = 0; i < K2S_MAX_IMAGES; ++i) tab.img[i] = K2sImage{0, N, 0};
    return 0;
  }
  if (!out.h_cu_klines || !h_cu_sub) return fail(LINETR_E_ARG, "%s: mat_klines2sublines of several images needs the host prefix sums of key-lines and sub-lines", who);
  if (out.h_cu_klines[n_images] != K) return fail(LINETR_E_ARG, "%s: h_cu_klines does not end at K", who);
  int64_t off = 0;
  for (int i = 0; i < n_images; ++i) {
    const int ki = out.h_cu_klines[i + 1] - out.h_cu_klines[i], ni = h_cu_sub[i + 1] - h_cu_sub[i];
    if (ki < 0 || ni < 0) return fail(LINETR_E_ARG, "%s: prefix sums not monotone", who);
    tab.img[i] = K2sImage{off, ni, h_cu_sub[i]};
    off += (int64_t)ki * ni;
  }
  return 0;
}

int nhwc_map(LinetrHandle* h, hipStream_t st, const float* dense_desc, int dense_is_nhwc, int n_images, int P, float* buf,
             const float*& nhwc) {
  nhwc = dense_desc;
  if (dense_is_nhwc) return LINETR_OK;
  ProfScope ps(h, st, "nchw_to_nhwc", 0, 2.0 * n_images * P * D * 4);
  hipLaunchKernelGGL(nchw_to_nhwc_kernel, dim3(cdiv(P, 64), D / 64, n_images), dim3(256), 0, st, dense_desc, buf, D, P);
  LT_LAUNCH_CHECK();
  nhwc = buf;
  return LINETR_OK;
}

struct TokenFront {
  const LinetrLineRec* recs; int K, N; double td; int T;
  const float *dense_desc, *dense_score;
  int n_images, height, width, align_corners, dense_is_nhwc;
  double clip_x, clip_y;
  float *sublines, *resp, *angle_sub;
  int* s2l_g;
  float* nhwc_buf;
  bool map_always;
  double tokenize_bytes;
  float *cpnt = nullptr, *cscore = nullptr; int n_pad_images = 0; int64_t first_pad = 0;
};
int token_front(LinetrHandle* h, hipStream_t st, const TokenFront& a, const LinetrTokens& out, const K2sTable& k2s, int32_t* d_sub2line,
                const float*& nhwc) {
  {
    ProfScope ps(h, st, "line_fill", 0, (double)a.K * 80 + (double)a.N * 8);
    hipLaunchKernelGGL(line_fill_kernel, dim3(cdiv(a.K, 256)), dim3(256), 0, st, a.recs, a.K, a.clip_x, a.clip_y, out.klines, out.length,
                       out.angles, a.s2l_g, d_sub2line);
    LT_LAUNCH_CHECK();
  }
  {
    ProfScope ps(h, st, "tokenize", 0, a.tokenize_bytes);
    hipLaunchKernelGGL(tokenize_kernel, dim3(a.N + cdiv(a.n_pad_images, 64) + (out.mat ? a.K : 0)), dim3(64), 0, st, a.recs, a.s2l_g, a.N,
                       a.td, a.T, a.height, a.width, a.clip_x, a.clip_y, a.dense_score, a.sublines, out.pnt, out.mask, a.resp, a.angle_sub,
                       out.score, a.cpnt, a.cscore, a.n_pad_images, a.first_pad, out.mat, k2s);
    LT_LAUNCH_CHECK();
  }
  const int Hc = a.height / 8, Wc = a.width / 8;
  nhwc = nullptr;
  if (a.map_always || out.desc)
    if (int e = nhwc_map(h, st, a.dense_desc, a.dense_is_nhwc, a.n_images, Hc * Wc, a.nhwc_buf, nhwc)) return e;
  if (out.desc) {
    const int64_t ntok = (int64_t)a.N * a.T;
    ProfScope ps(h, st, "sample_desc", 0, (double)ntok * D * 4 * 2);
    hipLaunchKernelGGL(sample_desc_kernel, dim3((unsigned)((ntok + 3) / 4)), dim3(256), 0, st, out.pnt, a.s2l_g, a.recs, ntok, a.T, nhwc,
                       Hc, Wc, a.align_corners, out.desc);
    LT_LAUNCH_CHECK();
  }
  return LINETR_OK;
}

struct TokLayout { int64_t o_nhwc, o_s2l, total; };
TokLayout tok_layout(int n_images, int height, int width, int N) {
  TokLayout L{};
  const int64_t P = (int64_t)(height / 8) * (width / 8);
  Carve c;
  L.o_nhwc = c.take(n_images * P * D * 4);
  L.o_s2l = c.take((int64_t)std::max(N, 1) * 4);
  L.total = c.o + 256;
  return L;
}
}
// ... 603 lines not shown
  K2sTable k2s;
  if (int e = k2s_table(out, n_images, K, N, h_cu, k2s, "describe")) return e;
  if (ws_bytes < linetr_describe_workspace_bytes(h, n_images, height, width, N, n_real))
    return fail(LINETR_E_WORKSPACE, "describe: workspace too small");
  const int64_t rows = n_real + n_images;
  if (rows > INT32_MAX / 8) return fail(LINETR_E_ARG, "describe: batch too large");
  LT_HIP(hipSetDevice(h->device));
  DescWs dw = desc_layout(n_images, height, width, N, rows, (char*)d_ws);
  FwdWs w = fwd_layout(h, N, rows, n_images, (char*)d_ws + dw.fwd_off);
  const int* cu_dev;
  if (int e = cu_on_device(h_cu, d_cu, n_images, w, st, cu_dev)) return e;
  TokenFront f{d_recs, K, N, td, T, d_dense_desc, d_dense_score, n_images, height, width, align_corners, dense_is_nhwc,
               (double)width - 0.6, (double)height - 0.6, out.sublines ? out.sublines : dw.sublines, out.resp ? out.resp : dw.resp,
               out.angle_sub ? out.angle_sub : dw.angle_sub};
  f.s2l_g = dw.s2l_g; f.nhwc_buf = dw.nhwc;
  f.map_always = true;
  f.tokenize_bytes = (double)n_real * 16;
  f.cpnt = dw.cpnt; f.cscore = dw.cscore; f.n_pad_images = n_images; f.first_pad = n_real;
  const float* nhwc_map;
  if (int e = token_front(h, st, f, out, k2s, d_sub2line, nhwc_map)) return e;
  TokenStage ts;
  ts.cpnt = dw.cpnt; ts.cscore = dw.cscore; ts.nhwc = nhwc_map; ts.recs = d_recs; ts.sub2line_g = dw.s2l_g;
  ts.rows = rows; ts.first_pad = n_real; ts.Hc = height / 8; ts.Wc = width / 8; ts.align_corners = align_corners;
  ts.pipe = pipe;
  if (int e = pipe_boundary(pipe, CUT_TOKENS, st)) return e;
  return forward_core(h, st, ts, f.sublines, f.resp, f.angle_sub, h_cu, cu_dev, n_images, N, T, d_line_desc, w);
}

int pipe_ready(LinetrHandle* h) {
  LinetrHandle::Pipe& p = h->pipe;
  if (p.stream[0]) return LINETR_OK;
  if (p.failed) return fail(LINETR_E_HIP, "describe_submit: the pipeline's streams could not be created");
  constexpr int NS = LinetrHandle::PIPE_STREAMS, NL = LinetrHandle::PIPE_SLOTS, NE = NL * (NS + 1);
  hipStream_t s[NS] = {};
  hipEvent_t ev[NE] = {};
  bool ok = true;
  for (int i = 0; ok && i < NS; ++i) ok = hipStreamCreateWithFlags(&s[i], hipStreamNonBlocking) == hipSuccess;
  for (int i = 0; ok && i < NE; ++i) ok = hipEventCreateWithFlags(&ev[i], hipEventDisableTiming) == hipSuccess;
  if (!ok) {
    for (hipEvent_t e : ev) if (e) (void)hipEventDestroy(e);
    for (hipStream_t x : s) if (x) (void)hipStreamDestroy(x);
    (void)hipGetLastError();
    p.failed = true;
    return fail(LINETR_E_HIP, "describe_submit: the pipeline's streams could not be created");
  }
  for (int i = 0; i < NS; ++i) p.stream[i] = s[i];
  for (int l = 0, k = 0; l < NL; ++l) {
    p.fork[l] = ev[k++]; p.done[l] = ev[k++];
    for (int c = 0; c < NS - 1; ++c) p.cut[l][c] = ev[k++];
  }
  return LINETR_OK;
}

struct PipePlan { int n_cuts = 0; int cut[LinetrHandle::PIPE_STREAMS - 1] = {0, 0, 0}; };
PipePlan pipe_plan(const LinetrHandle* h, int n_slots) {
  PipePlan pl;
  const int n_sig = (int)h->sig.size();
  if (n_slots == 2 || n_sig < 5) { pl.n_cuts = 1; pl.cut[0] = n_sig >= 3 ? CUT_SIG0 + 2 : CUT_SENTENCE; }
  else { pl.n_cuts = 2; pl.cut[0] = CUT_SIG0; pl.cut[1] = CUT_SIG0 + 3; }
  return pl;
}
}

extern "C" int linetr_describe(LinetrHandle* h, const LinetrLineRec* d_recs, int32_t K, int32_t N, int64_t n_real,
                               const int32_t* h_cu, const int32_t* d_cu, int32_t n_images, double td, int32_t T,
                               const float* d_dense_desc, const float* d_dense_score, int32_t height, int32_t width,
                               int32_t align_corners, int32_t dense_is_nhwc, LinetrTokens out, int32_t* d_sub2line,
                               float* d_line_desc, void* d_ws, int64_t ws_bytes, void* stream) {
  return describe_impl(h, d_recs, K, N, n_real, h_cu, d_cu, n_images, td, T, d_dense_desc, d_dense_score, height, width, align_corners,
                       dense_is_nhwc, out, d_sub2line, d_line_desc, d_ws, ws_bytes, (hipStream_t)stream, nullptr);
}

extern "C" int32_t linetr_pipeline_max_slots(void) { return LinetrHandle::PIPE_SLOTS; }

extern "C" int linetr_describe_submit(LinetrHandle* h, const LinetrLineRec* d_recs, int32_t K, int32_t N, int64_t n_real,
                                      const int32_t* h_cu, const int32_t* d_cu, int32_t n_images, double td, int32_t T,
                                      const float* d_dense_desc, const float* d_dense_score, int32_t height, int32_t width,
                                      int32_t align_corners, int32_t dense_is_nhwc, LinetrTokens out, int32_t* d_sub2line,
                                      float* d_line_desc, void* d_ws, int64_t ws_bytes, int32_t slot, int32_t n_slots, void* stream) {
  if (!h) return fail(LINETR_E_ARG, "describe_submit: null handle");
  if (n_slots < 1 || n_slots > LinetrHandle::PIPE_SLOTS || slot < 0 || slot >= n_slots)
    return fail(LINETR_E_ARG, "describe_submit: need 0 <= slot < n_slots <= %d", LinetrHandle::PIPE_SLOTS);
  LT_HIP(hipSetDevice(h->device));
  if (int e = pipe_ready(h)) return e;
  LinetrHandle::Pipe& p = h->pipe;
  hipStream_t st = (hipStream_t)stream;
  if (p.submitted[slot]) LT_HIP(hipEventSynchronize(p.done[slot]));
  const PipePlan plan = pipe_plan(h, n_slots);
  PipeStages stg;
  for (int i = 0; i < LinetrHandle::PIPE_STREAMS; ++i) stg.stream[i] = p.stream[i];
  stg.n_cuts = plan.n_cuts;
  for (int i = 0; i < plan.n_cuts; ++i) { stg.cut[i] = plan.cut[i]; stg.ev[i] = p.cut[slot][i]; }
  LT_HIP(hipEventRecord(p.fork[slot], st));
  LT_HIP(hipStreamWaitEvent(stg.stream[0], p.fork[slot], 0));
  const int e = describe_impl(h, d_recs, K, N, n_real, h_cu, d_cu, n_images, td, T, d_dense_desc, d_dense_score, height, width,
                              align_corners, dense_is_nhwc, out, d_sub2line, d_line_desc, d_ws, ws_bytes, stg.stream[0], &stg);
  if (e) {
    for (hipStream_t x : p.stream) (void)hipStreamSynchronize(x);
    p.submitted[slot] = false;
    return e;
  }
  LT_HIP(hipEventRecord(p.done[slot], stg.stream[stg.next]));
  p.submitted[slot] = true;
  return LINETR_OK;
}

extern "C" int linetr_describe_join(LinetrHandle* h, int32_t slot, void* stream) {
  if (!h) return fail(LINETR_E_ARG, "describe_join: null handle");
  if (slot < 0 || slot >= LinetrHandle::PIPE_SLOTS) return fail(LINETR_E_ARG, "describe_join: bad slot");
  if (!h->pipe.stream[0] || !h->pipe.submitted[slot]) return fail(LINETR_E_ARG, "describe_join: nothing was submitted to this slot");
  LT_HIP(hipStreamWaitEvent((hipStream_t)stream, h->pipe.done[slot], 0));
  return LINETR_OK;
}

extern "C" int linetr_debug_posenc(LinetrHandle* h, int32_t which, const float* d_in0, const float* d_in1,
                                      const float* d_in2, int64_t rows, float* d_out, void* stream) {
  if (!h || !d_in0 || !d_in1 || !d_out || (which == 1 && !d_in2) || which < 0 || which > 1)
    return fail(LINETR_E_ARG, "debug_posenc: bad argument");
  if (!fused_mlp_enabled(h->cfg)) return fail(LINETR_E_ARG, "debug_posenc: needs keyline_encoder [32,64,128,256]");
  if (rows <= 0) return LINETR_OK;
  LT_HIP(hipSetDevice(h->device));
  return enc_mlp123(h, (hipStream_t)stream, EncCall{which, d_in0, d_in1, which == ENC_WORD ? nullptr : d_in2, rows, nullptr}, d_out);
}

extern "C" int linetr_debug_gemm(LinetrHandle* h, const float* A, int32_t lda, const float* W, const float* bias,
                                 const float* R, float* Y, int32_t ldy, int32_t M, int32_t N, int32_t K, int32_t act,
                                 int32_t cache_weights, void* stream) {
  if (lda < K || ldy < N || lda % 4 || ldy % 4) return fail(LINETR_E_ARG, "debug_gemm: bad leading dimension");
  if (!h || !A || !W || !Y) return fail(LINETR_E_ARG, "debug_gemm: null argument");
  if (K % 32 || N % 64) return fail(LINETR_E_ARG, "debug_gemm: N %% 64 == 0 and K %% 32 == 0 required");
  LT_HIP(hipSetDevice(h->device));
  hipStream_t st = (hipStream_t)stream;
  GemmW w;
  w.W = W; w.b = bias; w.rows = N; w.K = K;
  unsigned char* buf = nullptr;
  if (h->precision != LINETR_PREC_F32) {
    int64_t bytes = 0;
    const SplitOffsets at = split_offsets(N, K, N == WS_N && K == WS_K, bytes);
    auto it = h->debug_split.find(W);
    const bool make = it == h->debug_split.end();
    if (make) LT_HIP(hipMalloc((void**)&buf, bytes));
    split_copies(w, make ? buf : it->second, at, make, st);
    LT_LAUNCH_CHECK();
    if (make && cache_weights) { h->debug_split[W] = buf; buf = nullptr; }
  }
  const int e = run_gemm(h, st, w, M, {A, lda}, {Y, ldy}, act, R);
  if (buf) {
    (void)hipStreamSynchronize(st);
    (void)hipFree(buf);
  }
  return e;
}

extern "C" int linetr_debug_gemm_case(LinetrHandle* h, const LinetrGemmCase* c, int32_t* tile_used, void* stream) {
  if (!h || !c) return fail(LINETR_E_ARG, "debug_gemm_case: null argument");
  const bool query = !c->A && !c->W && !c->Y;
  const int M = c->M, N = c->N, K = c->K, groups = c->groups;
  if (M < 0 || N <= 0 || K <= 0 || groups < 1) return fail(LINETR_E_ARG, "debug_gemm_case: bad shape M=%d N=%d K=%d groups=%d", M, N, K, groups);
  if (K % 32 || N % 64) return fail(LINETR_E_ARG, "debug_gemm_case: N %% 64 == 0 and K %% 32 == 0 required");
  if (c->lda % 4 || c->ldy % 4 || c->ldy < N || (c->A2 && (c->lda2 % 4 || c->lda2 < K - c->K1)) || c->lda < (c->A2 ? c->K1 : K))
    return fail(LINETR_E_ARG, "debug_gemm_case: bad leading dimension");
  if (c->A2 && (c->K1 <= 0 || c->K1 >= K || c->K1 % 32))
    return fail(LINETR_E_ARG, "debug_gemm_case: the split point K1 = %d must be a multiple of 32 inside (0, K = %d)", c->K1, K);
  if (c->gA % 4 || c->gY % 4 || c->gA < 0 || c->gY < 0) return fail(LINETR_E_ARG, "debug_gemm_case: group strides must be non-negative multiples of 4 floats");
  if (c->act < ACT_NONE || c->act > ACT_DIST) return fail(LINETR_E_ARG, "debug_gemm_case: act must be 0 .. 3");
  if (c->tile < -1 || (c->tile >= (int)SplitTile::count && c->tile != LINETR_GEMM_TILE_WS))
    return fail(LINETR_E_ARG, "debug_gemm_case: no tile %d", c->tile);
  NormSpec ns;
  if (c->norm) {
    if (c->norm != 1 && c->norm != 2) return fail(LINETR_E_ARG, "debug_gemm_case: norm must be 0, 1 (LayerNorm) or 2 (L2)");
    if (N != D || c->ldy != D || groups != 1) return fail(LINETR_E_ARG, "debug_gemm_case: a row normalisation needs N = ldy = 256 and one group");
    if (!query && c->norm == 1 && (!c->gamma || !c->beta)) return fail(LINETR_E_ARG, "debug_gemm_case: LayerNorm needs gamma and beta");
    ns.mode = c->norm; ns.gamma = c->gamma; ns.beta = c->beta; ns.add2 = c->add2; ns.eps = c->eps;
  } else if (c->via_row_norm) {
    return fail(LINETR_E_ARG, "debug_gemm_case: via_row_norm without a norm");
  }
  if (!query) {
    if (!c->A || !c->W || !c->Y) return fail(LINETR_E_ARG, "debug_gemm_case: null tensor");
    uintptr_t al = (uintptr_t)c->A | (uintptr_t)c->A2 | (uintptr_t)c->W | (uintptr_t)c->bias | (uintptr_t)c->R | (uintptr_t)c->Y |
                   (uintptr_t)c->gamma | (uintptr_t)c->beta | (uintptr_t)c->add2;
    if (al % 16) return fail(LINETR_E_ARG, "debug_gemm_case: tensors must be 16-byte aligned");
  }
  const int64_t rows = (int64_t)N * groups;
  const bool with_st = groups == 1 && N == WS_N && K == WS_K;
  GemmW w;
  w.W = c->W; w.b = c->bias; w.rows = (int)rows; w.K = K;
  const GemmA A{c->A, c->lda, c->A2, c->lda2, c->A2 ? c->K1 : 0};
  const GemmGroups grp{groups, N, c->gA, c->gY};
  const GemmGroups* pg = groups > 1 ? &grp : nullptr;
  GemmForce force;
  force.tile = c->tile; force.used = tile_used; force.launch = false;
  const bool fuse = c->norm && !c->via_row_norm && (c->tile >= 0 || gemm_norm_fuses(h, w, M, A, c->R, c->Y));
  if (with_st) w.st = reinterpret_cast<const unsigned char*>(h);
  if (int e = run_gemm(h, nullptr, w, M, A, {c->Y, c->ldy}, c->act, c->R, pg, fuse ? &ns : nullptr, &force)) return e;
  if (query || M == 0) return LINETR_OK;
  LT_HIP(hipSetDevice(h->device));
  hipStream_t st = (hipStream_t)stream;
  unsigned char* buf = nullptr;
  int64_t bytes = 0;
  SplitOffsets at{};
  if (h->precision != LINETR_PREC_F32) at = split_offsets(rows, K, with_st, bytes);
  bytes = align_up(bytes, 256);
  const int64_t tmp_at = bytes;
  if (c->norm && !fuse) bytes += (int64_t)M * D * sizeof(float);
  if (bytes > 0) LT_HIP(hipMalloc((void**)&buf, bytes));
  if (h->precision != LINETR_PREC_F32) split_copies(w, buf, at, true, st);
  int e = LINETR_OK;
  if (hipGetLastError() != hipSuccess) e = fail(LINETR_E_HIP, "debug_gemm_case: splitting the weights failed");
  force.launch = true;
  if (!e && c->norm && !fuse) {
    float* tmp = reinterpret_cast<float*>(buf + tmp_at);
    e = run_gemm(h, st, w, M, A, {tmp, D}, c->act, c->R, nullptr, nullptr, &force);
    if (!e) e = row_norm(h, st, tmp, M, ns, c->Y);
  } else if (!e) {
    e = run_gemm(h, st, w, M, A, {c->Y, c->ldy}, c->act, c->R, pg, fuse ? &ns : nullptr, &force);
  }
  (void)hipStreamSynchronize(st);
  if (buf) (void)hipFree(buf);
  return e;
}

extern "C" int linetr_debug_sig_attention(LinetrHandle* h, int32_t kernel, int32_t layer, const float* d_in, int32_t ld_in,
                                          const int32_t* h_cu, int32_t n_images, float* d_msg, int32_t* kernel_used, void* stream) {
  if (!h) return fail(LINETR_E_ARG, "debug_sig_attention: null handle");
  if (h->cfg.bn_batch_stats) return fail(LINETR_E_ARG, "debug_sig_attention: a training-mode handle (bn_batch_stats = 1) is not served");
  if (kernel < -1 || kernel > SIGK_FUSED) return fail(LINETR_E_ARG, "debug_sig_attention: kernel must be -1 .. 4");
  if (int e = check_cu(h_cu, n_images)) return e;
  const int N = h_cu[n_images];
  int max_n = 0;
  for (int i = 0; i < n_images; ++i) max_n = std::max(max_n, h_cu[i + 1] - h_cu[i]);
  const bool query_only = kernel == -1 && !d_in && !d_msg;
  if (kernel == -1) kernel = sig_attn_plan(h, n_images, N, max_n).kernel();
  if (kernel_used) *kernel_used = kernel;
  if (query_only) return LINETR_OK;
  if (kernel == SIGK_FUSED) {
    if (h->precision != LINETR_PREC_BF16X6) return fail(LINETR_E_ARG, "debug_sig_attention: the fused kernel runs in bf16x6 mode only");
    if (max_n > 256) return fail(LINETR_E_ARG, "debug_sig_attention: the fused kernel takes images of up to 256 sub-lines");
    if (layer < 0 || layer >= (int)h->sig.size()) return fail(LINETR_E_ARG, "debug_sig_attention: layer out of range");
    if (!h->sig[layer].Wqkv.st) return fail(LINETR_E_ARG, "debug_sig_attention: the layer has no split-tile weight image");
    if (ld_in != D) return fail(LINETR_E_ARG, "debug_sig_attention: the fused kernel reads z rows, ld_in must be 256");
  } else if (ld_in != 3 * D && !(kernel == SIGK_SMALL && ld_in == 4 * D)) {
    return fail(LINETR_E_ARG, "debug_sig_attention: ld_in must be 768 (or 1024, sig_attn_small only)");
  }
  if (N <= 0) return LINETR_OK;
  if (!d_in || !d_msg) return fail(LINETR_E_ARG, "debug_sig_attention: null tensor");
  if (((uintptr_t)d_in | (uintptr_t)d_msg) % 16) return fail(LINETR_E_ARG, "debug_sig_attention: tensors must be 16-byte aligned");
  LT_HIP(hipSetDevice(h->device));
  hipStream_t st = (hipStream_t)stream;
  int* cu_dev = nullptr;
  LT_HIP(hipMalloc((void**)&cu_dev, (n_images + 1) * sizeof(int)));
  int e = LINETR_OK;
  if (hipMemcpyAsync(cu_dev, h_cu, (n_images + 1) * sizeof(int), hipMemcpyHostToDevice, st) != hipSuccess)
    e = fail(LINETR_E_HIP, "debug_sig_attention: cu_sub upload failed");
  const double fl = attn_flops(h_cu, n_images);
  if (!e)
    e = kernel == SIGK_FUSED ? sig_qkv_attention(h, st, h->sig[layer], d_in, cu_dev, n_images, N, fl, d_msg)
                             : sig_attention(h, st, kernel, d_in, ld_in, cu_dev, n_images, N, max_n, fl, d_msg);
  (void)hipStreamSynchronize(st);
  (void)hipFree(cu_dev);
  return e;
}

extern "C" int linetr_debug_tok_mlp(LinetrHandle* h, int32_t variant, const float* d_pnt, const float* d_score, int64_t rows_word,
                                    const float* d_sublines, const float* d_resp, const float* d_angle, int64_t rows_line,
                                    float* d_out_word, float* d_out_line, int32_t max_blocks, int32_t* variant_used, void* stream) {
  if (!h) return fail(LINETR_E_ARG, "debug_tok_mlp: null handle");
  if (h->cfg.bn_batch_stats) return fail(LINETR_E_ARG, "debug_tok_mlp: a training-mode handle (bn_batch_stats = 1) is not served");
  if (variant < -1 || variant > TOKV_CHAIN) return fail(LINETR_E_ARG, "debug_tok_mlp: variant must be -1 .. 4");
  if (rows_word < 0 || rows_line < 0 || rows_word > INT32_MAX / 8 || rows_line > INT32_MAX / 8)
    return fail(LINETR_E_ARG, "debug_tok_mlp: row counts must be 0 .. %d", INT32_MAX / 8);
  if (max_blocks < 0) return fail(LINETR_E_ARG, "debug_tok_mlp: max_blocks must be 0 (one block per compute unit) or positive");
  if (!fused_mlp_enabled(h->cfg) || h->cfg.enc_channels[0] != 32 || h->cfg.enc_channels[3] != D)
    return fail(LINETR_E_ARG, "debug_tok_mlp: needs keyline_encoder [32,64,128,256]");
  const bool query_only = variant == -1 && !d_out_word && !d_out_line;
  bool word = rows_word > 0 && variant != TOKV_LINE, line = rows_line > 0 && variant != TOKV_WORD;
  if (variant == -1) {
    const TokMlpPlan plan = tok_mlp_plan(h, rows_word, rows_line);
    variant = plan.both >= 0 ? plan.both : (word && !plan.word) || (line && !plan.line) ? (int)TOKV_CHAIN : word ? (int)TOKV_WORD : line ? (int)TOKV_LINE : -1;
  }
  if (variant_used) *variant_used = variant;
  if (query_only || variant < 0) return LINETR_OK;
  if (variant == TOKV_DUAL || variant == TOKV_SEQ) {
    if (rows_word <= 0 || rows_line <= 0) return fail(LINETR_E_ARG, "debug_tok_mlp: the two-encoder launches need rows of both encoders");
    if (variant == TOKV_DUAL && !tok_mlp_dual_fits(rows_word, rows_line))
      return fail(LINETR_E_ARG, "debug_tok_mlp: %lld + %lld rows do not fit the chip side by side (one block per 64-row tile, %d compute units)",
                  (long long)rows_word, (long long)rows_line, cu_count());
  }
  if (variant != TOKV_CHAIN && ((word && !tok_mlp_has_images(h->enc[ENC_WORD])) || (line && !tok_mlp_has_images(h->enc[ENC_LINE]))))
    return fail(LINETR_E_ARG, "debug_tok_mlp: the encoder has no split-tile weight images");
  if (!word && !line) return LINETR_OK;
  if ((word && (!d_pnt || !d_score || !d_out_word)) || (line && (!d_sublines || !d_resp || !d_angle || !d_out_line)))
    return fail(LINETR_E_ARG, "debug_tok_mlp: null tensor");
  if (((uintptr_t)d_pnt | (uintptr_t)d_score | (uintptr_t)d_sublines | (uintptr_t)d_resp | (uintptr_t)d_angle) % 4 ||
      ((uintptr_t)d_out_word | (uintptr_t)d_out_line) % 16)
    return fail(LINETR_E_ARG, "debug_tok_mlp: outputs must be 16-byte aligned, inputs 4-byte aligned");
  LT_HIP(hipSetDevice(h->device));
  hipStream_t st = (hipStream_t)stream;
  float* scratch = nullptr;
  const int64_t off_line = align_up((word ? rows_word : 0) * h->cfg.enc_channels[2] * 4, 256);
  if (variant == TOKV_CHAIN) LT_HIP(hipMalloc((void**)&scratch, off_line + align_up((line ? rows_line : 0) * h->cfg.enc_channels[2] * 4, 256) + 256));
  float* act_w[4] = {nullptr, nullptr, scratch, d_out_word};
  float* act_l[4] = {nullptr, nullptr, scratch ? (float*)((char*)scratch + off_line) : nullptr, d_out_line};
  const EncCall cw{ENC_WORD, d_pnt, d_score, nullptr, rows_word, act_w};
  const EncCall cl{ENC_LINE, d_sublines, d_resp, d_angle, rows_line, act_l};
  int e = LINETR_OK;
  switch (variant) {
    case TOKV_WORD: e = tok_mlp_launch(tok_mlp_args(h, cw), true, st, max_blocks); break;
    case TOKV_LINE: e = tok_mlp_launch(tok_mlp_args(h, cl), false, st, max_blocks); break;
    case TOKV_DUAL: e = tok_mlp_launch_dual(tok_mlp_args(h, cw), tok_mlp_args(h, cl), st, max_blocks, 0); break;
    case TOKV_SEQ: e = tok_mlp_launch_dual(tok_mlp_args(h, cw), tok_mlp_args(h, cl), st, max_blocks, 1); break;
    default:
      if (word) e = pos_encoder(h, st, cw, false);
      if (!e && line) e = pos_encoder(h, st, cl, false);
  }
  (void)hipStreamSynchronize(st);
  if (scratch) (void)hipFree(scratch);
  return e;
}

namespace {
constexpr int64_t BN_PARTIAL_BYTES = (int64_t)BN_MAX_BLOCKS * 2 * BN_MAX_CHANNELS * 8, BN_AFFINE_BYTES = 2 * BN_MAX_CHANNELS * 4;
struct BnDebugWs { float* act[3]; double* partial; float* affine; int64_t total; };
BnDebugWs bn_debug_layout(const LinetrHandle* h, int which, int64_t rows, char* base) {
  BnDebugWs w;
  int64_t off = 0;
  auto take = [&](int64_t bytes) { char* p = base + off; off += align_up(bytes, 256); return p; };
  for (int i = 0; i < 3; ++i) w.act[i] = (float*)take(which < 0 ? 0 : std::max<int64_t>(rows, 0) * h->cfg.enc_channels[i] * 4);
  w.partial = (double*)take(BN_PARTIAL_BYTES);
  w.affine = (float*)take(BN_AFFINE_BYTES);
  w.total = off;
  return w;
}
}

extern "C" int64_t linetr_debug_bn_train_workspace_bytes(const LinetrHandle* h, int32_t which, int64_t rows) {
  if (!h || which < -1 || which > 1 || rows < 0 || rows > INT32_MAX / 8) return -1;
  return bn_debug_layout(h, which, rows, nullptr).total;
}

extern "C" int linetr_debug_bn_train(LinetrHandle* h, int32_t which, float* d_z, int64_t rows, int32_t C, int32_t ld,
                                     const float* d_gamma, const float* d_beta, const float* d_in0, const float* d_in1,
                                     const float* d_in2, float* d_out, float momentum, float* d_running, float* d_batch,
                                     float* d_affine, int32_t* nb_used, void* d_ws, int64_t ws_bytes, void* stream) {
  if (!h) return fail(LINETR_E_ARG, "debug_bn_train: null handle");
  if (!h->cfg.bn_batch_stats) return fail(LINETR_E_ARG, "debug_bn_train: the handle was created for inference (bn_batch_stats = 0)");
  if (which < -1 || which > 1) return fail(LINETR_E_ARG, "debug_bn_train: which must be -1 (one layer), 0 (word encoder) or 1 (line encoder)");
  if (rows < 0 || rows > INT32_MAX / 8) return fail(LINETR_E_ARG, "debug_bn_train: row count must be 0 .. %d", INT32_MAX / 8);
  if (!(momentum >= 0.f && momentum <= 1.f)) return fail(LINETR_E_ARG, "debug_bn_train: momentum out of [0, 1]");
  if (nb_used) *nb_used = 0;
  if (which < 0) {
    if (!bn_channels_ok(C)) return fail(LINETR_E_ARG, "debug_bn_train: %d channels (4 .. %d, multiples of 4)", C, BN_MAX_CHANNELS);
    if (!bn_rows_ok(d_z, ld, C))
      return fail(LINETR_E_ARG, "debug_bn_train: row stride %d (at least the %d channels, a multiple of 4) on a 16-byte aligned z", ld, C);
    if (!d_z || !d_gamma || !d_beta || !d_running) return fail(LINETR_E_ARG, "debug_bn_train: null tensor");
    if (((uintptr_t)d_gamma | (uintptr_t)d_beta | (uintptr_t)d_running | (uintptr_t)d_batch | (uintptr_t)d_affine) % 4)
      return fail(LINETR_E_ARG, "debug_bn_train: the vectors must be 4-byte aligned");
  } else {
    if (!d_in0 || !d_in1 || (which == ENC_LINE && !d_in2) || !d_out || !d_running) return fail(LINETR_E_ARG, "debug_bn_train: null tensor");
    if (((uintptr_t)d_in0 | (uintptr_t)d_in1 | (uintptr_t)d_in2 | (uintptr_t)d_running | (uintptr_t)d_batch) % 4 || (uintptr_t)d_out % 16)
      return fail(LINETR_E_ARG, "debug_bn_train: the output must be 16-byte aligned, the other tensors 4-byte aligned");
  }
  if (!d_ws || (uintptr_t)d_ws % 256) return fail(LINETR_E_ARG, "debug_bn_train: the workspace must be 256-byte aligned");
  const BnDebugWs w = bn_debug_layout(h, which, rows, (char*)d_ws);
  if (ws_bytes < w.total) return fail(LINETR_E_WORKSPACE, "debug_bn_train: workspace too small (%lld < %lld bytes)", (long long)ws_bytes, (long long)w.total);
  if (rows == 0) return LINETR_OK;
  LT_HIP(hipSetDevice(h->device));
  hipStream_t st = (hipStream_t)stream;
  BnTrain bt;
  bt.running = d_running; bt.batch = d_batch; bt.momentum = momentum; bt.partial = w.partial; bt.affine = w.affine;
  int e, nb = 0;
  if (which < 0) {
    e = bn_train_layer(st, bt, d_z, rows, C, ld, d_gamma, d_beta, 0, &nb);
// ... 139 lines not shown
```

### linetr_amd/csrc/lt_gemm_split.h

```cpp
#pragma once
#include "lt_gemm.h"

namespace lt {

typedef __bf16 bf16x8 __attribute__((ext_vector_type(8)));
typedef __bf16 bf16x2 __attribute__((ext_vector_type(2)));
typedef float f32x2 __attribute__((ext_vector_type(2)));
typedef unsigned u32x2 __attribute__((ext_vector_type(2)));

typedef _Float16 f16x8 __attribute__((ext_vector_type(8)));
typedef _Float16 f16x2 __attribute__((ext_vector_type(2)));

template <int PL, int FMT = 0>
__device__ __forceinline__ void split_pair(float x0, float x1, unsigned (&out)[PL]) {
  float r0 = x0, r1 = x1;
#pragma unroll
  for (int p = 0; p < PL; ++p) {
    if constexpr (FMT == 0) {
      const bf16x2 h = __builtin_convertvector(f32x2{r0, r1}, bf16x2);
      const unsigned u = __builtin_bit_cast(unsigned, h);
      out[p] = u;
      if (p + 1 < PL) {
        r0 -= __builtin_bit_cast(float, u << 16);
        r1 -= __builtin_bit_cast(float, u & 0xffff0000u);
      }
    } else {
      const f16x2 h = __builtin_convertvector(f32x2{r0, r1}, f16x2);
      out[p] = __builtin_bit_cast(unsigned, h);
      if (p + 1 < PL) {
        const f32x2 hf = __builtin_convertvector(h, f32x2);
        r0 -= hf[0];
        r1 -= hf[1];
      }
    }
  }
}

template <int FMT>
__device__ __forceinline__ f32x16 mfma_split(const bf16x8& a, const bf16x8& b, const f32x16& c) {
  if constexpr (FMT == 0) return __builtin_amdgcn_mfma_f32_32x32x16_bf16(a, b, c, 0, 0, 0);
  else return __builtin_amdgcn_mfma_f32_32x32x16_f16(__builtin_bit_cast(f16x8, a), __builtin_bit_cast(f16x8, b), c, 0, 0, 0);
}

template <int PL, int FMT = 0>
__global__ void split_rows_kernel(const float* __restrict__ W, unsigned char* __restrict__ out, int64_t rows, int K) {
  const int64_t gid = (int64_t)blockIdx.x * blockDim.x + threadIdx.x;
  const int kq = K / 4;
  if (gid >= rows * kq) return;
  const int64_t r = gid / kq;
  const int k = (int)(gid % kq) * 4;
  const f32x4 v = *reinterpret_cast<const f32x4*>(W + r * K + k);
  unsigned a[PL], b[PL];
  split_pair<PL, FMT>(v[0], v[1], a);
  split_pair<PL, FMT>(v[2], v[3], b);
  unsigned char* base = out + (r * (K / 32) + k / 32) * (PL * 64) + (k % 32) * 2;
#pragma unroll
  for (int p = 0; p < PL; ++p) *reinterpret_cast<u32x2*>(base + p * 64) = u32x2{a[p], b[p]};
}

struct SplitGemmArgs {
  GemmArgs g;
  const unsigned char* Wsp = nullptr;
  int64_t gWsp = 0;
  int wide_epi = 0;
  int sk_first = 0, sk_blocks = 0;
  float* sk_ws = nullptr;
  unsigned* sk_flags = nullptr;
  unsigned sk_epoch = 0;
};

__device__ __forceinline__ void store16_write_through(float* p, const f32x4& v) {
  asm volatile("global_store_dwordx4 %0, %1, off sc1\n\ts_nop 1" : : "v"(p), "v"(v) : "memory");
}
__device__ __forceinline__ f32x4 sk_load16(const float* p) {
  f32x4 v;
  asm volatile("global_load_dwordx4 %0, %1, off sc1" : "=v"(v) : "v"(p) : "memory");
  return v;
}
__device__ __forceinline__ void sk_publish(unsigned* flag, unsigned epoch) {
  asm volatile("s_waitcnt vmcnt(0)" ::: "memory");
  __syncthreads();
  if (threadIdx.x == 0) __hip_atomic_store(flag, epoch, __ATOMIC_RELAXED, __HIP_MEMORY_SCOPE_AGENT);
}
__device__ __forceinline__ void sk_wait(const unsigned* flag, unsigned epoch, unsigned* err) {
  if (threadIdx.x == 0) {
    int spins = 0;
    while (__hip_atomic_load(flag, __ATOMIC_RELAXED, __HIP_MEMORY_SCOPE_AGENT) != epoch) {
      __builtin_amdgcn_s_sleep(8);
      if (++spins > 400000) {
        __hip_atomic_store(err, 1u, __ATOMIC_RELAXED, __HIP_MEMORY_SCOPE_AGENT);
        break;
      }
    }
  }
  __syncthreads();
}

template <int BM, int BN, int WM, int WN, int PL, bool DB = true, int FMT = 0, int PFD = 1, bool PIPE = false, bool SKT = false>
__global__ __launch_bounds__(WM * WN * 64) void gemm_split_kernel(SplitGemmArgs sa) {
  const GemmArgs& g = sa.g;
  constexpr int NT = WM * WN * 64;
  constexpr int TM = BM / WM, TN = BN / WN;
  constexpr int MI = TM / 32, NI = TN / 32;
  constexpr int RS = PL * 64 + 16;
  constexpr int A_F4 = BM * 8 / NT;
  constexpr int B_PCS = BN * PL * 4 / NT;
  static_assert(A_F4 >= 1 && B_PCS >= 1 && (BM * 8) % NT == 0 && (BN * PL * 4) % NT == 0, "bad tiling");

  extern __shared__ __attribute__((aligned(16))) unsigned char smem_s[];
  constexpr int NBUF = DB ? 2 : 1;
  unsigned char* As = smem_s;
  unsigned char* Bs = smem_s + NBUF * BM * RS;

  const int tid = threadIdx.x, lane = tid & 63, wave = tid >> 6;
  const int wm = wave / WN, wn = wave % WN;
  constexpr bool SK = SKT;
  static_assert(!SKT || (PIPE && BM == 128 && BN == 256), "stream-K is built for the pipelined 128x256 tile only");
  const int gx = g.N / BN, gy = (g.M + BM - 1) / BM;
  const int ntile_all = gx * gy;
  const int ntile = (SK && sa.sk_blocks > 0) ? sa.sk_first : ntile_all;
  const int tile = xcd_tile(blockIdx.x, ntile);
  int m0 = (tile / gx) * BM, n0 = (tile % gx) * BN;
  const int grp = blockIdx.y;
  const float* A = g.A + grp * g.gA;
  const float* A2 = g.A2 ? g.A2 + grp * g.gA : nullptr;
  const unsigned char* Wsp = sa.Wsp + grp * sa.gWsp;
  const int K1 = g.A2 ? g.K1 : g.K;
  const int nkw = g.K / 32;
  int nk = nkw, kbase = 0;

  const int lrow = (tid >> 6) * 8 + (lane >> 4) + 4 * ((lane >> 3) & 1), lc4 = (tid & 7) * 4;
  constexpr int B_ROWPCS = PL == 3 ? BN * 8 / NT : B_PCS;
  static_assert(PL != 3 || ((BN * 8) % NT == 0 && (BN * 4) % NT == 0 && BN % 8 == 0), "W staging: whole 8-lane groups per thread slot");
  auto stage_piece = [&](int i, int& r, int& pc) {
    if constexpr (PL == 3) {
      if (i < B_ROWPCS) { const int a = tid + i * NT; r = a >> 3; pc = a & 7; }
      else { const int q = tid + (i - B_ROWPCS) * NT, gq = q >> 3, l = q & 7; r = (gq >> 2) * 8 + (gq & 3) + 4 * (l >> 2); pc = 8 + (l & 3); }
    } else { const int q = tid + i * NT; r = q / (PL * 4); pc = q % (PL * 4); }
  };
  static_assert(PFD >= 1 && (DB || PFD == 1) && (!PIPE || PFD <= 2), "deep prefetch needs the double-buffered LDS");
  f32x4 ra_[PFD][A_F4];
  f32x4 rb_[PFD][B_PCS];
  auto gload_set = [&](int kt, f32x4 (&ra)[A_F4], f32x4 (&rb)[B_PCS]) {
    const int k0 = (kbase + kt) * 32;
    const float* src = A; int ld = g.lda; int kk = k0;
    if (k0 >= K1) { src = A2; ld = g.lda2; kk = k0 - K1; }
#pragma unroll
    for (int i = 0; i < A_F4; ++i) {
      int r = m0 + lrow + i * (NT / 8);
      r = r < g.M ? r : g.M - 1;
      ra[i] = *reinterpret_cast<const f32x4*>(src + (int64_t)r * ld + kk + lc4);
    }
#pragma unroll
    for (int i = 0; i < B_PCS; ++i) {
      int r, pc;
      stage_piece(i, r, pc);
      rb[i] = *reinterpret_cast<const f32x4*>(Wsp + ((int64_t)(n0 + r) * nkw + kbase + kt) * (PL * 64) + pc * 16);
    }
  };
  auto lstore_set = [&](int buf, const f32x4 (&ra)[A_F4], const f32x4 (&rb)[B_PCS]) {
#pragma unroll
    for (int i = 0; i < A_F4; ++i) {
      unsigned a[PL], b[PL];
      split_pair<PL, FMT>(ra[i][0], ra[i][1], a);
      split_pair<PL, FMT>(ra[i][2], ra[i][3], b);
      unsigned char* dst = As + (buf * BM + lrow + i * (NT / 8)) * RS + lc4 * 2;
#pragma unroll
      for (int p = 0; p < PL; ++p) *reinterpret_cast<u32x2*>(dst + p * 64) = u32x2{a[p], b[p]};
    }
#pragma unroll
    for (int i = 0; i < B_PCS; ++i) {
      int r, pc;
      stage_piece(i, r, pc);
      *reinterpret_cast<f32x4*>(Bs + (buf * BN + r) * RS + pc * 16) = rb[i];
    }
  };
  auto gload = [&](int kt) { gload_set(kt, ra_[0], rb_[0]); };
  auto lstore = [&](int buf) { lstore_set(buf, ra_[0], rb_[0]); };

  f32x16 acc[MI][NI];

  const int frow = lane & 31, fk = (lane >> 5) * 16;
  auto read_frags = [&](int buf, int s, bf16x8 (&af)[MI][PL], bf16x8 (&bf)[NI][PL]) {
    const unsigned char* Ab = As + (buf * BM + wm * TM + frow) * RS + fk + s * 32;
    const unsigned char* Bb = Bs + (buf * BN + wn * TN + frow) * RS + fk + s * 32;
#pragma unroll
    for (int i = 0; i < MI; ++i)
#pragma unroll
      for (int p = 0; p < PL; ++p) af[i][p] = *reinterpret_cast<const bf16x8*>(Ab + i * 32 * RS + p * 64);
#pragma unroll
    for (int j = 0; j < NI; ++j)
#pragma unroll
      for (int p = 0; p < PL; ++p) bf[j][p] = *reinterpret_cast<const bf16x8*>(Bb + j * 32 * RS + p * 64);
  };
  using Terms = split_terms<PL>;
  auto mma = [&](const bf16x8 (&af)[MI][PL], const bf16x8 (&bf)[NI][PL]) {
#pragma unroll
    for (int t = 0; t < Terms::N; ++t)
#pragma unroll
      for (int i = 0; i < MI; ++i)
#pragma unroll
        for (int j = 0; j < NI; ++j)
          acc[i][j] = mfma_split<FMT>(af[i][Terms::pa(t)], bf[j][Terms::pb(t)], acc[i][j]);
  };
  auto compute = [&](int buf) {
#pragma unroll
    for (int s = 0; s < 2; ++s) {
      bf16x8 af[MI][PL], bf[NI][PL];
      read_frags(buf, s, af, bf);
      mma(af, bf);
    }
  };

  auto mainloop = [&]() {
#pragma unroll
  for (int i = 0; i < MI; ++i)
#pragma unroll
    for (int j = 0; j < NI; ++j)
#pragma unroll
      for (int r = 0; r < 16; ++r) acc[i][j][r] = 0.f;
  gload(0);
  lstore(0);
  if constexpr (PFD == 1 || PIPE) {
    if (nk > 1) gload_set(1, ra_[PFD - 1], rb_[PFD - 1]);
    if constexpr (PIPE && PFD == 2) gload_set(nk > 2 ? 2 : nk - 1, ra_[0], rb_[0]);
    __syncthreads();
    if constexpr (DB && PIPE) {
      bf16x8 af0[MI][PL], bf0[NI][PL], af1[MI][PL], bf1[NI][PL];
      constexpr int N_MMA = MI * NI * Terms::N;
      constexpr int N_FRAG = (MI + NI) * PL;
      constexpr int E1 = 2 * A_F4 + B_PCS;
#define FRAG_ORDER(k) (((k) / (MI + NI)) == 0 ? (((k) % (MI + NI)) < MI ? ((k) % (MI + NI)) * PL + (PL - 1) : MI * PL + (((k) % (MI + NI)) - MI) * PL) \
                     : ((k) / (MI + NI)) == PL - 1 ? (((k) % (MI + NI)) < MI ? ((k) % (MI + NI)) * PL : MI * PL + (((k) % (MI + NI)) - MI) * PL + (PL - 1)) \
                     : (((k) % (MI + NI)) < MI ? ((k) % (MI + NI)) * PL + 1 : MI * PL + (((k) % (MI + NI)) - MI) * PL + 1))
      auto step_mma = [&](int m, const bf16x8 (&af)[MI][PL], const bf16x8 (&bf)[NI][PL]) {
        const int t = m / (MI * NI), ij = m % (MI * NI), i = ij / NI, j = ij % NI;
        acc[i][j] = mfma_split<FMT>(af[i][Terms::pa(t)], bf[j][Terms::pb(t)], acc[i][j]);
      };
      auto step_read = [&](int k, int buf, int s, bf16x8 (&af)[MI][PL], bf16x8 (&bf)[NI][PL]) {
        const unsigned char* Ab = As + (buf * BM + wm * TM + frow) * RS + fk + s * 32;
        const unsigned char* Bb = Bs + (buf * BN + wn * TN + frow) * RS + fk + s * 32;
        if (k < MI * PL) { const int i = k / PL, pp = k % PL; af[i][pp] = *reinterpret_cast<const bf16x8*>(Ab + i * 32 * RS + pp * 64); }
        else { const int q = k - MI * PL, j = q / PL, pp = q % PL; bf[j][pp] = *reinterpret_cast<const bf16x8*>(Bb + j * 32 * RS + pp * 64); }
      };
      auto step_gload = [&](int u, int kt, f32x4 (&ra)[A_F4], f32x4 (&rb)[B_PCS]) {
        if (u < A_F4) {
          const int k0 = (kbase + kt) * 32;
          const float* src = A; int ld = g.lda; int kk = k0;
          if (k0 >= K1) { src = A2; ld = g.lda2; kk = k0 - K1; }
          int r = m0 + lrow + u * (NT / 8);
          r = r < g.M ? r : g.M - 1;
          ra[u] = *reinterpret_cast<const f32x4*>(src + (int64_t)r * ld + kk + lc4);
        } else {
          int r, pc;
          stage_piece(u - A_F4, r, pc);
          rb[u - A_F4] = *reinterpret_cast<const f32x4*>(Wsp + ((int64_t)(n0 + r) * nkw + kbase + kt) * (PL * 64) + pc * 16);
        }
      };
      auto step_store = [&](int u, int buf, const f32x4 (&ra)[A_F4], const f32x4 (&rb)[B_PCS]) {
        if (u < A_F4) {
          unsigned a[PL], b[PL];
          split_pair<PL, FMT>(ra[u][0], ra[u][1], a);
          split_pair<PL, FMT>(ra[u][2], ra[u][3], b);
          unsigned char* dst = As + (buf * BM + lrow + u * (NT / 8)) * RS + lc4 * 2;
#pragma unroll
          for (int pp = 0; pp < PL; ++pp) *reinterpret_cast<u32x2*>(dst + pp * 64) = u32x2{a[pp], b[pp]};
        } else {
          int r, pc;
          stage_piece(u - A_F4, r, pc);
          *reinterpret_cast<f32x4*>(Bs + (buf * BN + r) * RS + pc * 16) = rb[u - A_F4];
        }
      };
      constexpr int R_SPAN = N_MMA > N_FRAG ? N_MMA : N_FRAG;
      constexpr int S_SPAN = N_MMA;
      auto first_half = [&](int kt, f32x4 (&ra)[A_F4], f32x4 (&rb)[B_PCS]) {
        const int buf = kt & 1;
        const int ktn = kt + 1 + PFD < nk ? kt + 1 + PFD : nk - 1;
#pragma unroll
        for (int m = 0; m < N_MMA; ++m) {
          step_mma(m, af0, bf0);
#pragma unroll
          for (int k = 0; k < N_FRAG; ++k)
            if (k * R_SPAN / N_FRAG == m) step_read(FRAG_ORDER(k), buf, 1, af1, bf1);
#pragma unroll
          for (int e = 0; e < E1; ++e)
            if ((2 * e + 1) * S_SPAN / (2 * E1) == m) {
              if (e < 2 * A_F4) { if (e % 2 == 0) step_store(e / 2, buf ^ 1, ra, rb); else step_gload(e / 2, ktn, ra, rb); }
              else step_store(A_F4 + (e - 2 * A_F4), buf ^ 1, ra, rb);
            }
          __builtin_amdgcn_sched_barrier(0);
        }
      };
      auto second_half = [&](int kt, f32x4 (&ra)[A_F4], f32x4 (&rb)[B_PCS]) {
        const int buf = kt & 1;
        const int ktn = kt + 1 + PFD < nk ? kt + 1 + PFD : nk - 1;
#pragma unroll
        for (int m = 0; m < N_MMA; ++m) {
          step_mma(m, af1, bf1);
#pragma unroll
          for (int k = 0; k < N_FRAG; ++k)
            if (k * R_SPAN / N_FRAG == m) step_read(FRAG_ORDER(k), buf ^ 1, 0, af0, bf0);
#pragma unroll
          for (int e = 0; e < B_PCS; ++e)
            if ((2 * e + 1) * N_MMA / (2 * B_PCS) == m) step_gload(A_F4 + e, ktn, ra, rb);
          __builtin_amdgcn_sched_barrier(0);
        }
      };
#pragma unroll
      for (int k = 0; k < N_FRAG; ++k) step_read(FRAG_ORDER(k), 0, 0, af0, bf0);
      if constexpr (PFD == 1) {
        for (int kt = 0; kt < nk; ++kt) {
          first_half(kt, ra_[0], rb_[0]);
          __syncthreads();
          __builtin_amdgcn_sched_barrier(0);
          second_half(kt, ra_[0], rb_[0]);
        }
      } else {
        for (int kt = 0; kt < nk; kt += 2) {
          first_half(kt, ra_[1], rb_[1]);
          __syncthreads();
          __builtin_amdgcn_sched_barrier(0);
          second_half(kt, ra_[1], rb_[1]);
          if (kt + 1 < nk) {
            first_half(kt + 1, ra_[0], rb_[0]);
            __syncthreads();
            __builtin_amdgcn_sched_barrier(0);
            second_half(kt + 1, ra_[0], rb_[0]);
          }
        }
      }
    } else
    for (int kt = 0; kt < nk; ++kt) {
      const int buf = DB ? (kt & 1) : 0;
      if (DB) {
        lstore(buf ^ 1);
        if (kt + 2 < nk) gload(kt + 2);
      }
      compute(buf);
      if (!DB) {
        __syncthreads();
        lstore(0);
        if (kt + 2 < nk) gload(kt + 2);
      }
      __syncthreads();
    }
  } else {
#pragma unroll
    for (int u = 0; u < PFD; ++u)
      if (1 + u < nk) gload_set(1 + u, ra_[u], rb_[u]);
    __syncthreads();
    for (int kt0 = 0; kt0 < nk; kt0 += PFD) {
#pragma unroll
      for (int u = 0; u < PFD; ++u) {
        const int kt = kt0 + u;
        if (kt < nk) {
          const int buf = kt & 1;
          lstore_set(buf ^ 1, ra_[u], rb_[u]);
          if (kt + 1 + PFD < nk) gload_set(kt + 1 + PFD, ra_[u], rb_[u]);
          compute(buf);
          __syncthreads();
        }
      }
    }
  }

  };

  const float* bias = g.bias ? g.bias + grp * g.gBias : nullptr;
  float* Y = g.Y + grp * g.gY;
  auto epilogue = [&]() {
  if (sa.wide_epi) {
    constexpr int LPR = TN / 4;
    constexpr int RPI = 64 / LPR;
    constexpr int NIT = TM / RPI;
    __syncthreads();
    float* ep = reinterpret_cast<float*>(smem_s) + wave * (TM * TN);
    const int er = lane / LPR, ec = (lane % LPR) * 4;
    const int grow0 = m0 + wm * TM + er, gcol = n0 + wn * TN + ec;
    const bool row_norm = BN == 256 && g.norm != 0;
    f32x4 rres[NIT];
    if (g.R && !row_norm) {
#pragma unroll
      for (int it = 0; it < NIT; ++it) {
        const int row = grow0 + it * RPI;
        rres[it] = row < g.M ? *reinterpret_cast<const f32x4*>(g.R + (int64_t)row * g.ldr + gcol) : f32x4{0.f, 0.f, 0.f, 0.f};
      }
    }
#pragma unroll
    for (int j = 0; j < NI; ++j) {
      const float bv = bias ? bias[n0 + wn * TN + j * 32 + (lane & 31)] : 0.f;
#pragma unroll
      for (int i = 0; i < MI; ++i) {
#pragma unroll
        for (int r = 0; r < 16; ++r) {
          float v = apply_act(acc[i][j][r] + bv, g.act);
          ep[(i * 32 + (r & 3) + 8 * (r >> 2) + 4 * (lane >> 5)) * TN + j * 32 + (lane & 31)] = v;
        }
      }
    }
    if constexpr (BN == 256) {
      if (row_norm) {
        __syncthreads();
        constexpr int RPW = BM / (WM * WN);
        const float* epb = reinterpret_cast<const float*>(smem_s);
        const int c0 = lane * 4, wn_c = c0 / TN, cc = c0 % TN;
        for (int it = 0; it < RPW; ++it) {
          const int rl = wave * RPW + it;
          const int row = m0 + rl;
          if (row >= g.M) break;
          f32x4 v = *reinterpret_cast<const f32x4*>(epb + ((rl / TM) * WN + wn_c) * (TM * TN) + (rl % TM) * TN + cc);
          if (g.R) {
            const f32x4 rr = *reinterpret_cast<const f32x4*>(g.R + (int64_t)row * g.ldr + c0);
#pragma unroll
            for (int c = 0; c < 4; ++c) v[c] += rr[c];
          }
          f32x4 o;
          if (g.norm == 1) {
            const float mean = wave_sum(v[0] + v[1] + v[2] + v[3]) * (1.f / 256);
            float q = 0.f;
#pragma unroll
            for (int c = 0; c < 4; ++c) { const float d = v[c] - mean; q += d * d; }
            const float rstd = 1.f / sqrtf(wave_sum(q) * (1.f / 256) + g.eps);
            const f32x4 ga = *reinterpret_cast<const f32x4*>(g.gamma + c0);
            const f32x4 be = *reinterpret_cast<const f32x4*>(g.beta + c0);
#pragma unroll
            for (int c = 0; c < 4; ++c) o[c] = (v[c] - mean) * rstd * ga[c] + be[c];
          } else {
            float q = 0.f;
#pragma unroll
            for (int c = 0; c < 4; ++c) q += v[c] * v[c];
            const float nrm = fmaxf(sqrtf(wave_sum(q)), 1e-12f);
#pragma unroll
            for (int c = 0; c < 4; ++c) o[c] = v[c] / nrm;
          }
          if (g.add2) {
            const f32x4 a2 = *reinterpret_cast<const f32x4*>(g.add2 + (int64_t)row * g.ldadd2 + c0);
#pragma unroll
            for (int c = 0; c < 4; ++c) o[c] += a2[c];
          }
          *reinterpret_cast<f32x4*>(Y + (int64_t)row * g.ldy + c0) = o;
        }
        return;
      }
    }
#pragma unroll
    for (int it = 0; it < NIT; ++it) {
      const int row = grow0 + it * RPI;
      f32x4 v = *reinterpret_cast<const f32x4*>(ep + (er + it * RPI) * TN + ec);
      if (g.R) {
#pragma unroll
        for (int c = 0; c < 4; ++c) v[c] += rres[it][c];
      }
      if (row < g.M) store16_write_through(Y + (int64_t)row * g.ldy + gcol, v);
    }
    return;
  }
#pragma unroll
  for (int j = 0; j < NI; ++j) {
    const int col = n0 + wn * TN + j * 32 + (lane & 31);
    const float bv = bias ? bias[col] : 0.f;
#pragma unroll
    for (int i = 0; i < MI; ++i) {
#pragma unroll
      for (int r = 0; r < 16; ++r) {
        const int row = m0 + wm * TM + i * 32 + (r & 3) + 8 * (r >> 2) + 4 * (lane >> 5);
        if (row < g.M) {
          float v = apply_act(acc[i][j][r] + bv, g.act);
          if (g.R) v += g.R[(int64_t)row * g.ldr + col];
          Y[(int64_t)row * g.ldy + col] = v;
        }
      }
    }
  }
  };

  bool sk = false;
  int s_ = 0, S = 1;
  unsigned it_i = 0, it_hi = 1, I = 0;
  if constexpr (SK) {
    if (sa.sk_blocks > 0 && (int)blockIdx.x >= sa.sk_first) {
      sk = true;
      S = sa.sk_blocks; s_ = (int)blockIdx.x - sa.sk_first;
      I = (unsigned)(ntile_all - sa.sk_first) * (unsigned)nkw;
      it_i = I * (unsigned)(S - 1 - s_) / (unsigned)S;
      it_hi = I * (unsigned)(S - s_) / (unsigned)S;
      if (it_i >= it_hi) return;
    }
  }
  constexpr int SLOT = BM * BN;
  for (;;) {
    int kb = 0, ke = nkw;
    if (SK && sk) {
      const unsigned tq = it_i / (unsigned)nkw;
      const int t = sa.sk_first + (int)tq;
      kb = (int)(it_i - tq * (unsigned)nkw);
      ke = kb + (int)(it_hi - it_i) < nkw ? kb + (int)(it_hi - it_i) : nkw;
      m0 = (t / gx) * BM; n0 = (t % gx) * BN;
      __syncthreads();
    }
    kbase = kb; nk = ke - kb;
    mainloop();
    if (SK && sk && kb > 0) {
      float* slot = sa.sk_ws + (int64_t)s_ * SLOT;
#pragma unroll
      for (int a = 0; a < MI; ++a)
#pragma unroll
        for (int b = 0; b < NI; ++b)
#pragma unroll
          for (int q = 0; q < 4; ++q)
            store16_write_through(slot + ((((a * NI + b) * 4 + q) * NT) + tid) * 4,
                       f32x4{acc[a][b][4 * q], acc[a][b][4 * q + 1], acc[a][b][4 * q + 2], acc[a][b][4 * q + 3]});
      sk_publish(sa.sk_flags + s_, sa.sk_epoch);
    } else {
      if (SK && sk && ke < nkw) {
        int rem = nkw - ke;
        for (int j = s_ - 1; rem > 0 && j >= 0; --j) {
          const int len = (int)(I * (unsigned)(S - j) / (unsigned)S - I * (unsigned)(S - 1 - j) / (unsigned)S);
          if (len == 0) continue;
          sk_wait(sa.sk_flags + j, sa.sk_epoch, sa.sk_flags + S);
          const float* slot = sa.sk_ws + (int64_t)j * SLOT;
#pragma unroll
          for (int a = 0; a < MI; ++a) {
            f32x4 pv[NI][4];
#pragma unroll
            for (int b = 0; b < NI; ++b)
#pragma unroll
              for (int q = 0; q < 4; ++q) pv[b][q] = sk_load16(slot + ((((a * NI + b) * 4 + q) * NT) + tid) * 4);
            asm volatile("s_waitcnt vmcnt(0)" ::: "memory");
#pragma unroll
            for (int b = 0; b < NI; ++b)
#pragma unroll
              for (int q = 0; q < 4; ++q)
#pragma unroll
                for (int c = 0; c < 4; ++c) acc[a][b][4 * q + c] += pv[b][q][c];
          }
          rem -= len < rem ? len : rem;
        }
      }
      epilogue();
    }
    if (!(SK && sk)) break;
    it_i += (unsigned)(ke - kb);
    if (it_i >= it_hi) break;
  }
}

#undef FRAG_ORDER

template <int BM, int BN, int PL, bool DB>
struct SplitTileLds {
  static constexpr size_t main = (size_t)(DB ? 2 : 1) * (BM + BN) * (PL * 64 + 16);
  static constexpr size_t epi = (size_t)BM * BN * sizeof(float);
  static constexpr bool epi_fits = epi <= 160 * 1024;
  static constexpr size_t bytes = (epi_fits && epi > main) ? epi : main;
  static bool wide_epi(const GemmArgs& g) { return g.ldy % 4 == 0 && (!g.R || g.ldr % 4 == 0) && epi_fits; }
};

template <int BM, int BN, int WM, int WN, int PL, bool DB = true, int FMT = 0, int PFD = 1, bool PIPE = false>
inline int gemm_split_launch_t(const SplitGemmArgs& sa, int groups, hipStream_t st) {
  using Lds = SplitTileLds<BM, BN, PL, DB>;
  SplitGemmArgs sa2 = sa;
  sa2.wide_epi = Lds::wide_epi(sa.g);
  sa2.sk_first = sa2.sk_blocks = 0;
  LT_HIP((allow_dynamic_lds<gemm_split_kernel<BM, BN, WM, WN, PL, DB, FMT, PFD, PIPE>>((int)Lds::bytes)));
  dim3 grid((sa.g.N / BN) * cdiv(sa.g.M, BM), groups);
  hipLaunchKernelGGL((gemm_split_kernel<BM, BN, WM, WN, PL, DB, FMT, PFD, PIPE>), grid, dim3(WM * WN * 64), Lds::bytes, st, sa2);
  return 0;
}

template <int PL, int FMT>
inline int gemm_split16_launch(const SplitGemmArgs& sa, hipStream_t st);
inline bool split16_wins(const GemmArgs& g, int groups);
template <int PL, int FMT>
inline void gemm_split_small_launch(const SplitGemmArgs& sa, int groups, hipStream_t st);
inline bool small_gemm_wins(const GemmArgs& g, int groups);

enum class SplitTile { t32x32k4, t112x256, t128x64, t256x128, t128x256, t64x256, t128x128, t128x128s, t256x256, t64x64, t64x128, count };
inline const char* tile_name(SplitTile t) {
  static const char* const names[] = {"32x32k4", "112x256", "128x64", "256x128", "128x256", "64x256", "128x128", "128x128s", "256x256",
                                      "64x64", "64x128"};
  return names[(int)t];
}
inline SplitTile split_tile(const GemmArgs& g, int groups, int pl = 3) {
  if (small_gemm_wins(g, groups)) return SplitTile::t32x32k4;
  if (g.N % 128 != 0) return SplitTile::t128x64;
  if (pl == 2 && split16_wins(g, groups)) return SplitTile::t112x256;
  const int64_t r128 = cdiv(g.M, 128), r64 = cdiv(g.M, 64);
  const int64_t t128 = r128 * (g.N / 128) * groups;
  if (pl == 3 && ((g.K <= 256 && g.N >= 768 && t128 >= 400) || (g.K <= 128 && t128 >= 1024))) return SplitTile::t128x128s;
  if (g.N % 256 == 0 && r128 * (g.N / 256) * groups >= 140) return SplitTile::t128x256;
  if (pl == 3 && g.K <= 512 && t128 >= 140) return SplitTile::t128x128s;
  if (g.N % 256 != 0 && (int64_t)cdiv(g.M, 256) * (g.N / 128) * groups >= 192) return SplitTile::t256x128;
  if (r64 * (g.N / 64) * groups <= 768) return SplitTile::t64x64;
  if (r64 * (g.N / 128) * groups <= 512) return SplitTile::t64x128;
  if (g.N % 256 == 0) return r64 * (g.N / 256) * groups >= 140 ? SplitTile::t64x256 : SplitTile::t64x128;
  return SplitTile::t128x128;
}

inline int pick_split_tile(const GemmArgs& g, int groups, int pl, SplitTile& tile) {
  static const char* forced = LT_XENV("LINETR_GEMM_TILE");
  if (!forced) { tile = split_tile(g, groups, pl); return 0; }
  for (int i = 0; i < (int)SplitTile::count; ++i)
    if (!strcmp(forced, tile_name((SplitTile)i))) { tile = (SplitTile)i; return 0; }
  return fail(LINETR_E_ARG, "LINETR_GEMM_TILE: no tile is named '%s'", forced);
}

inline int split_tile_launched(const GemmArgs& g, int groups, int pl, SplitTile& tile) {
  if (g.N % 64 != 0 || g.K % 32 != 0 || (g.A2 && g.K1 % 32 != 0))
    return fail(LINETR_E_ARG, "gemm_split: unsupported shape M=%d N=%d K=%d", g.M, g.N, g.K);
  if (g.norm != 0) {
    if (tile != SplitTile::t128x256 || g.N != 256 || groups != 1 || g.ldy % 4 != 0 || (g.R && g.ldr % 4 != 0))
      return fail(LINETR_E_ARG, "gemm_split: fused row normalisation asked of tile %s (N=%d): dispatcher bug", tile_name(tile), g.N);
  }
  if (tile == SplitTile::t112x256 && groups != 1)
    return fail(LINETR_E_ARG, "gemm_split: tile 112x256 asked of a grouped launch (%d groups)", groups);
  if (g.N % 128 != 0 && tile != SplitTile::t32x32k4) tile = SplitTile::t128x64;
  if (g.N % 256 != 0 && (tile == SplitTile::t128x256 || tile == SplitTile::t64x256 || tile == SplitTile::t256x256 ||
                         tile == SplitTile::t112x256))
    tile = SplitTile::t64x128;
  bool has256 = pl == 2;
#ifndef LINETR_EXPERIMENTS
  has256 = false;
#endif
  if (!has256 && tile == SplitTile::t256x256) tile = SplitTile::t64x128;
  return 0;
}

template <int PL, int FMT = 0>
inline int gemm_split_launch(const SplitGemmArgs& sa, int groups, SplitTile tile, hipStream_t st) {
  const GemmArgs& g = sa.g;
  if (g.M <= 0) return 0;
  if (int e = split_tile_launched(g, groups, PL, tile)) return e;
  int e = 0;
  switch (tile) {
    case SplitTile::t32x32k4: gemm_split_small_launch<PL, FMT>(sa, groups, st); break;
    case SplitTile::t112x256: e = gemm_split16_launch<PL, FMT>(sa, st); break;
    case SplitTile::t128x64: e = gemm_split_launch_t<128, 64, 4, 1, PL, true, FMT>(sa, groups, st); break;
    case SplitTile::t256x128: e = gemm_split_launch_t<256, 128, 4, 2, PL, true, FMT, 1, true>(sa, groups, st); break;
    case SplitTile::t128x256: e = gemm_split_launch_t<128, 256, 2, 4, PL, true, FMT, PL == 3 ? 2 : 1, true>(sa, groups, st); break;
    case SplitTile::t64x256: e = gemm_split_launch_t<64, 256, 1, 4, PL, true, FMT, PL == 3 ? 2 : 1, true>(sa, groups, st); break;
    case SplitTile::t128x128: e = gemm_split_launch_t<128, 128, 2, 2, PL, true, FMT>(sa, groups, st); break;
    case SplitTile::t128x128s: e = gemm_split_launch_t<128, 128, 2, 4, PL, false, FMT>(sa, groups, st); break;
#ifdef LINETR_EXPERIMENTS
    case SplitTile::t256x256:
      if constexpr (PL == 2) e = gemm_split_launch_t<256, 256, 4, 2, 2, true, FMT>(sa, groups, st);
      break;
#endif
    case SplitTile::t64x64: e = gemm_split_launch_t<64, 64, 2, 2, PL, true, FMT, 3>(sa, groups, st); break;
    default: e = gemm_split_launch_t<64, 128, 2, 2, PL, true, FMT, 3>(sa, groups, st); break;
  }
  if (e) return e;
  LT_LAUNCH_CHECK();
  return 0;
}

}
```

### linetr_amd/csrc/lt_st_image.h

```cpp
#pragma once
#include <type_traits>

#include "lt_gemm_split.h"

namespace lt {

constexpr int ST_CHUNK = 512;
constexpr int ST_RB = 3 * ST_CHUNK;
inline __host__ __device__ int64_t st_row_blocks(int64_t rows) { return (rows + 127) / 128 * 8; }
inline int64_t st_bytes(int64_t rows, int K) { return st_row_blocks(rows) * (int64_t)(K / 16) * ST_RB; }

typedef unsigned u32x4 __attribute__((ext_vector_type(4)));

__global__ __launch_bounds__(256) void to_st_kernel(const float* __restrict__ X, int ld, int rows, int nkt,
                                                    unsigned char* __restrict__ out) {
  const int64_t gid = (int64_t)blockIdx.x * 256 + threadIdx.x;
  const int l = (int)(gid & 31);
  const int64_t c = gid >> 5;
  const int64_t RB = st_row_blocks(rows);
  if (c >= RB * nkt) return;
  const int kt = (int)(c / RB);
  const int64_t rb = c % RB;
  const int q = l >> 4, r = l & 15;
  const int64_t row = rb * 16 + r;
  f32x4 x0 = {0.f, 0.f, 0.f, 0.f}, x1 = x0;
  if (row < rows) {
    const float* p = X + row * ld + kt * 16 + q * 8;
    x0 = *reinterpret_cast<const f32x4*>(p);
    x1 = *reinterpret_cast<const f32x4*>(p + 4);
  }
  unsigned a[3], b[3], cc[3], d[3];
  split_pair<3>(x0[0], x0[1], a); split_pair<3>(x0[2], x0[3], b);
  split_pair<3>(x1[0], x1[1], cc); split_pair<3>(x1[2], x1[3], d);
  unsigned char* dst = out + c * ST_RB + l * 16;
#pragma unroll
  for (int p = 0; p < 3; ++p) *reinterpret_cast<u32x4*>(dst + p * ST_CHUNK) = u32x4{a[p], b[p], cc[p], d[p]};
}

__device__ __forceinline__ float bf_lo(unsigned u) { return __builtin_bit_cast(float, u << 16); }
__device__ __forceinline__ float bf_hi(unsigned u) { return __builtin_bit_cast(float, u & 0xffff0000u); }

__device__ __forceinline__ void st_piece_to_f32(const u32x4& p0, const u32x4& p1, const u32x4& p2, float (&v)[8]) {
#pragma unroll
  for (int e = 0; e < 4; ++e) {
    v[2 * e] = (bf_lo(p2[e]) + bf_lo(p1[e])) + bf_lo(p0[e]);
    v[2 * e + 1] = (bf_hi(p2[e]) + bf_hi(p1[e])) + bf_hi(p0[e]);
  }
}

__global__ __launch_bounds__(256) void from_st_kernel(const unsigned char* __restrict__ in, int rows, int nkt,
                                                      float* __restrict__ X, int ld) {
  const int64_t gid = (int64_t)blockIdx.x * 256 + threadIdx.x;
  const int l = (int)(gid & 31);
  const int64_t c = gid >> 5;
  const int64_t RB = st_row_blocks(rows);
  if (c >= RB * nkt) return;
  const int kt = (int)(c / RB);
  const int64_t rb = c % RB;
  const int q = l >> 4, r = l & 15;
  const int64_t row = rb * 16 + r;
  if (row >= rows) return;
  const unsigned char* src = in + c * ST_RB + l * 16;
  float v[8];
  st_piece_to_f32(*reinterpret_cast<const u32x4*>(src), *reinterpret_cast<const u32x4*>(src + ST_CHUNK),
                  *reinterpret_cast<const u32x4*>(src + 2 * ST_CHUNK), v);
  float* dst = X + row * ld + kt * 16 + q * 8;
  *reinterpret_cast<f32x4*>(dst) = f32x4{v[0], v[1], v[2], v[3]};
  *reinterpret_cast<f32x4*>(dst + 4) = f32x4{v[4], v[5], v[6], v[7]};
}

#define LT_GLDS(gp, lp, off)                                                                                      \
  __builtin_amdgcn_global_load_lds((const __attribute__((address_space(1))) void*)(gp),                           \
                                   (__attribute__((address_space(3))) void*)(lp), 16, (off), 0)

__device__ __forceinline__ void swap32(float& a, float& b) {
  unsigned x = __builtin_bit_cast(unsigned, a), y = __builtin_bit_cast(unsigned, b);
  asm volatile("s_nop 1\n\tv_permlane32_swap_b32 %0, %1\n\ts_nop 1" : "+v"(x), "+v"(y));
  a = __builtin_bit_cast(float, x);
  b = __builtin_bit_cast(float, y);
}

}
```

### linetr_amd/engine_debug.py

```python
from __future__ import annotations

import ctypes as C

import numpy as np
import torch

from . import _native as nat
from ._shapes import D, ptr


class _DebugSurface:
    def debug_posenc(self, which: str, in0, in1, in2=None):
        a, b = self._f32(in0), self._f32(in1)
        c = self._f32(in2) if in2 is not None else None
        rows = int(b.shape[0])
        out = torch.empty((rows, 128), dtype=torch.float32, device=self.device)
        self._call("linetr_debug_posenc", {"word": 0, "line": 1}[which], a.data_ptr(), b.data_ptr(), ptr(c), rows, out.data_ptr())
        return out

    def debug_gemm(self, A, W, bias=None, residual=None, act=0, cache_weights=False, out=None):
        W = self._f32(W)
        if A.dtype != torch.float32 or A.device != self.device or A.stride(1) != 1:
            A = self._f32(A)
        M, K = A.shape
        N = W.shape[0]
        Y = out if out is not None else torch.empty((M, N), dtype=torch.float32, device=self.device)
        b = self._f32(bias) if bias is not None else None
        r = residual
        if r is not None and (r.stride(0) != Y.stride(0) or r.stride(1) != 1):
            r = self._f32(r) if Y.stride(0) == N else None
            assert r is not None, "residual must share the output's row stride"
        self._call("linetr_debug_gemm", A.data_ptr(), A.stride(0), W.data_ptr(), ptr(b), ptr(r), Y.data_ptr(), Y.stride(0), M, N, K, int(act),
                   int(cache_weights))
        return Y

    GEMM_SPLIT_TILES = ("32x32k4", "112x256", "128x64", "256x128", "128x256", "64x256", "128x128", "128x128s", "256x256", "64x64",
                        "64x128")
    GEMM_F32_TILES = ("128x64", "128x128", "64x128")
    GEMM_WS = "ws64x256"
    _GEMM_TILE_WS = 100

    def _gemm_tile_code(self, tile):
        if tile is None or tile == -1:
            return -1
        if tile == self.GEMM_WS:
            return self._GEMM_TILE_WS
        names = self.GEMM_F32_TILES if self.get_precision() == "f32" else self.GEMM_SPLIT_TILES
        if tile not in names:
            raise ValueError(f"no GEMM tile {tile!r} in {self.get_precision()} mode")
        return names.index(tile)

    def _gemm_tile_name(self, code):
        if code == self._GEMM_TILE_WS:
            return self.GEMM_WS
        return (self.GEMM_F32_TILES if self.get_precision() == "f32" else self.GEMM_SPLIT_TILES)[code]

    def gemm_tile(self, M, N, K, *, groups=1, act=0, residual=False, concat=False, norm=0, lda=None, ldy=None, tile=-1) -> str:
        flag = C.c_void_p(16)
        c = nat.GemmCase(A=None, lda=int(lda or K), A2=flag if concat else None, lda2=int(K), K1=32 if concat else 0, W=None, bias=None,
                         R=flag if residual else None, Y=None, ldy=int(ldy or N), M=int(M), N=int(N), K=int(K), act=int(act),
                         groups=int(groups), gA=0, gY=0, norm=int(norm), gamma=None, beta=None, add2=None, eps=0.0, via_row_norm=0,
                         tile=self._gemm_tile_code(tile))
        used = C.c_int32(-1)
        nat.check(self._L.linetr_debug_gemm_case(self._h, C.byref(c), C.byref(used), None), self._L)
        return self._gemm_tile_name(used.value)

    def debug_gemm_case(self, A, W, bias=None, residual=None, act=0, *, A2=None, groups=1, gA=0, gY=None, norm=0, gamma=None,
                        beta=None, add2=None, eps=0.0, via_row_norm=False, tile=-1, out=None):
        W = self._f32(W)
        M, K1 = (int(v) for v in A.shape)
        K = K1 + (int(A2.shape[1]) if A2 is not None else 0)
        N = int(W.shape[0]) // groups
        if W.shape != (groups * N, K) or not W.is_contiguous():
            raise ValueError(f"W must be a contiguous [{groups} * N, {K}] tensor")
        if out is None:
            full = torch.empty((groups, M, N), dtype=torch.float32, device=self.device)
            out, gY = full[0], M * N
        else:
            full = out
        gY = int(gY or 0)

        def extent(t, rows, cols, gstride, what):
            if t.dtype != torch.float32 or t.device != self.device or t.dim() != 2 or t.stride(1) != 1:
                raise ValueError(f"{what}: a float32 matrix on the engine's device with unit column stride expected")
            if t.shape[0] < rows or t.shape[1] < cols:
                raise ValueError(f"{what}: shape {tuple(t.shape)} is smaller than [{rows}, {cols}]")
            have = t.untyped_storage().nbytes() // 4 - t.storage_offset()
            need = (groups - 1) * gstride + (rows - 1) * t.stride(0) + cols if rows > 0 else 0
            if need > have:
                raise ValueError(f"{what}: {need} floats needed behind its first element, the storage holds {have}")
            return t

        extent(A, M, K1, int(gA), "A")
        if A2 is not None:
            extent(A2, M, K - K1, int(gA), "A2")
        extent(out, M, N, gY, "out")
        if groups > 1 and gY < (M - 1) * out.stride(0) + N:
            raise ValueError("gY: the groups' outputs overlap")
        if residual is not None and extent(residual, M, N, 0, "residual").stride(0) != out.stride(0):
            raise ValueError("residual must share the output's row stride")
        vec = lambda t, n, what: None if t is None else extent(self._f32(t).reshape(1, -1), 1, n, 0, what)
        b, ga, be = vec(bias, groups * N, "bias"), vec(gamma, N, "gamma"), vec(beta, N, "beta")
        if add2 is not None and (extent(add2, M, N, 0, "add2").stride(0) != D or N != D):
            raise ValueError("add2 must have row stride 256")
        c = nat.GemmCase(A=ptr(A), lda=A.stride(0), A2=ptr(A2), lda2=A2.stride(0) if A2 is not None else 0, K1=K1 if A2 is not None else 0,
                         W=ptr(W), bias=ptr(b), R=ptr(residual), Y=ptr(out), ldy=out.stride(0), M=M, N=N, K=K, act=int(act),
                         groups=int(groups), gA=int(gA), gY=gY, norm=int(norm), gamma=ptr(ga), beta=ptr(be), add2=ptr(add2),
                         eps=float(eps), via_row_norm=int(bool(via_row_norm)), tile=self._gemm_tile_code(tile))
        used = C.c_int32(-1)
        self._call("linetr_debug_gemm_case", C.byref(c), C.byref(used))
        return (full if groups > 1 or full is out else out), self._gemm_tile_name(used.value)

    SIG_KERNELS = ("sig_attn", "sig_attn_small", "sig_attn_split4", "sig_attn_split8", "sig_qkv_attn")

    def sig_attention_kernel(self, cu_sub) -> int:
        cu = np.ascontiguousarray(np.asarray(cu_sub, dtype=np.int32))
        used = C.c_int32(-1)
        self._call("linetr_debug_sig_attention", -1, 0, None, 0, cu.ctypes.data, len(cu) - 1, None, C.byref(used))
        return used.value

    def debug_sig_attention(self, kernel, x, cu_sub, layer=0, out=None):
        if x.dtype != torch.float32 or x.device != self.device or x.stride(1) != 1:
            x = self._f32(x)
        cu = np.ascontiguousarray(np.asarray(cu_sub, dtype=np.int32))
        N = int(cu[-1]) if len(cu) else 0
        if int(x.shape[0]) < N:
            raise ValueError(f"{N} rows expected, got {int(x.shape[0])}")
        msg = out if out is not None else torch.empty((N, D), dtype=torch.float32, device=self.device)
        if msg.dtype != torch.float32 or msg.device != self.device or not msg.is_contiguous():
            raise ValueError("out must be a contiguous float32 tensor on the engine's device")
        used = C.c_int32(-1)
        self._call("linetr_debug_sig_attention", int(kernel), int(layer), x.data_ptr(), x.stride(0), cu.ctypes.data, len(cu) - 1, msg.data_ptr(),
                   C.byref(used))
        return msg, used.value

    TOK_MLP_VARIANTS = ("tok_mlp_word", "tok_mlp_line", "tok_mlp_dual", "tok_mlp_seq", "mlp123_gemm_chain")

    def tok_mlp_variant(self, rows_word, rows_line) -> int:
        used = C.c_int32(-1)
        self._call("linetr_debug_tok_mlp", -1, None, None, int(rows_word), None, None, None, int(rows_line), None, None, 0, C.byref(used))
        return used.value

    def debug_tok_mlp(self, variant, word=None, line=None, out_word=None, out_line=None, max_blocks=0):
        def f32(t, n, what):
            if t.dtype != torch.float32 or t.device != self.device or not t.is_contiguous() or t.numel() < n:
                raise ValueError(f"{what}: a contiguous float32 tensor of at least {n} elements on the engine's device expected")
            return t.data_ptr()
        pw = [None, None]; pl = [None, None, None]
        rw = rl = 0
        if word is not None:
            rw = int(word[2])
            pw = [f32(word[0], 2 * rw, "pnt"), f32(word[1], rw, "score")]
            if out_word is None:
                out_word = torch.empty((rw, D), dtype=torch.float32, device=self.device)
            f32(out_word, rw * D, "out_word")
        if line is not None:
            rl = int(line[3])
            pl = [f32(line[0], 4 * rl, "sublines"), f32(line[1], rl, "resp"), f32(line[2], 2 * rl, "angle")]
            if out_line is None:
                out_line = torch.empty((rl, D), dtype=torch.float32, device=self.device)
            f32(out_line, rl * D, "out_line")
        used = C.c_int32(-1)
        self._call("linetr_debug_tok_mlp", int(variant), pw[0], pw[1], rw, pl[0], pl[1], pl[2], rl, ptr(out_word), ptr(out_line), int(max_blocks),
                   C.byref(used))
        return out_word, out_line, used.value

    def debug_bn_train(self, which, *, z=None, rows=0, channels=0, ld=0, gamma=None, beta=None, word=None, line=None, out=None,
                       momentum=0.1, running=None, batch=None, affine=None):
        def f32(t, n, what):
            if t is None:
                return None
            if t.dtype != torch.float32 or t.device != self.device or not t.is_contiguous() or t.numel() < n:
                raise ValueError(f"{what}: a contiguous float32 tensor of at least {n} elements on the engine's device expected")
            return t.data_ptr()
        which = int(which)
        e = list(self.cfg["keyline_encoder"])
        ins = [None, None, None]
        if which < 0:
            rows, C_, ld = int(rows), int(channels), int(ld)
            n_stats = 2 * C_
            pz = f32(z, (rows - 1) * ld + C_ if rows > 0 else 0, "z")
            res = z
        else:
            C_, ld, pz = 0, 0, None
            n_stats = 2 * sum(e)
            if which == 0:
                rows = int(word[2])
                ins = [f32(word[0], 2 * rows, "pnt"), f32(word[1], rows, "score"), None]
            else:
                rows = int(line[3])
                ins = [f32(line[0], 4 * rows, "sublines"), f32(line[1], rows, "resp"), f32(line[2], 2 * rows, "angle")]
            if out is None:
                out = torch.empty((rows, e[3]), dtype=torch.float32, device=self.device)
            res = out
        nbytes = self._L.linetr_debug_bn_train_workspace_bytes(self._h, which, rows)
        if nbytes < 0:
            raise ValueError("debug_bn_train: which must be -1, 0 or 1 and rows non-negative")
        ws = self._workspace("bn_debug", nbytes)
        used = C.c_int32(-1)
        self._call("linetr_debug_bn_train", which, pz, rows, C_, ld, f32(gamma, C_, "gamma"), f32(beta, C_, "beta"), *ins,
                   f32(out, rows * e[3], "out") if which >= 0 else None, float(momentum), f32(running, n_stats, "running"),
                   f32(batch, n_stats, "batch"), f32(affine, n_stats, "affine"), C.byref(used), ws.data_ptr(), ws.numel())
        return res, used.value

    CLS_POOL_KERNELS = ("cls_pool", "cls_pool_online", "cls_pool_online_reverse", "cls_pool_online_split4")

    def cls_pool_kernel(self, N, dense=False) -> int:
        used = C.c_int32(-1)
        self._call("linetr_debug_cls_pool", -1, None, 0, None, int(N), 1, None, None, 0, 1, None, 1, 1, 1, 0, C.c_void_p(16) if dense else None,
                   None, C.byref(used))
        return used.value

    def debug_cls_pool(self, kernel, a4, out, N, T, *, recs=None, sub2line=None, cpnt=None, first_pad=0, n_images=1, dense_map=None,
                       nhwc=True, Hc=0, Wc=0, align_corners=False, desc_dense=None):
        for t in (a4, out, cpnt, dense_map, desc_dense):
            if t is not None and (t.dtype != torch.float32 or t.device != self.device or not t.is_contiguous()):
                raise ValueError("contiguous float32 tensors on the engine's device expected")
        if out.numel() < N * 4 * 544:
            raise ValueError("out is smaller than [N, 4, 544]")
        if desc_dense is None:
            if recs.dtype != torch.uint8 or sub2line.dtype != torch.int32 or sub2line.numel() < N:
                raise ValueError("recs: uint8 bytes of LineRec[K]; sub2line: int32 [N]")
            if a4.numel() < (first_pad + n_images) * D or cpnt.numel() < (first_pad + n_images) * 2 or dense_map.numel() < n_images * Hc * Wc * D:
                raise ValueError("a4 / cpnt / dense_map are smaller than first_pad + n_images rows / n_images maps")
        elif a4.numel() < N * T * D or desc_dense.numel() < N * T * D:
            raise ValueError("a4 / desc_dense are smaller than [N * T, 256]")
        used = C.c_int32(-1)
        self._call("linetr_debug_cls_pool", int(kernel), ptr(recs), recs.numel() // nat.REC_DTYPE.itemsize if recs is not None else 0,
                   ptr(sub2line), int(N), int(T), ptr(cpnt), ptr(a4), int(first_pad), int(n_images), ptr(dense_map), int(bool(nhwc)), int(Hc),
                   int(Wc), int(bool(align_corners)), ptr(desc_dense), ptr(out), C.byref(used))
        return out, used.value

    STAGES = ("tail", "sig")
    SIG_FOLD_NEXT = 8

    def debug_stage(self, stage, in0, in1=None, cu_sub=None, plan=-1, outs=(None, None, None)):
        sig = self.STAGES.index(stage) == 1
        cu = np.ascontiguousarray(np.asarray(cu_sub, dtype=np.int32)) if sig else None
        N = (int(cu[-1]) if len(cu) else 0) if sig else int(cu_sub)
        n_taps = max(int(self.cfg["n_sig_layers"]) - 1, 0)
        need = (N * D, 0, N * D, N * n_taps * D, 0) if sig else (N * 4 * 544, N * D, N * D, N * D, N * D)
        for t, n in zip((in0, in1, *outs), need):
            if t is not None and (t.dtype != torch.float32 or t.device != self.device or not t.is_contiguous() or t.numel() < n):
                raise ValueError(f"contiguous float32 tensors of at least {n} elements on the engine's device expected")
        n_images = len(cu) - 1 if sig else 1
        ws = self._workspace("stage", max(self._L.linetr_debug_stage_workspace_bytes(self._h, N, n_images), 0))
        used = C.c_int32(-1)
        self._call("linetr_debug_stage", int(sig), N, ptr(in0), ptr(in1), cu.ctypes.data if sig else None, n_images, int(plan),
                   ptr(outs[0]), ptr(outs[1]), ptr(outs[2]), C.byref(used), ws.data_ptr(), ws.numel())
        return used.value

    MATCH_PATHS = ("pair_dist + pair_pool + pair_final", "pair_match_fused<false>", "pair_match_fused<true>")

    def match_path(self, dims) -> int:
        dims = np.ascontiguousarray(dims, dtype=np.int32).reshape(-1, 4)
        used = C.c_int32(-1)
        self._call("linetr_debug_match", len(dims), dims.ctypes.data, None, None, None, None, None, None, 0.0, 0, None, None, None, None, None, 0,
                   -1, -1, -1, -1, C.byref(used))
        return used.value

    def debug_match(self, path, dims, desc0, off_n0, s2l0, desc1, off_n1, s2l1, thr, mutual, dk, off_dk, m01, off_k0, *,
                    seg1_global=-1, cache_dk=-1, device_table=-1) -> int:
        dims = np.ascontiguousarray(dims, dtype=np.int32).reshape(-1, 4)
        P = len(dims)
# ... 32 lines not shown
```

Before: 10.70 million line-descriptors/s.

## Stream pre-split weights into LDS via global_load_lds in bf16x6 128x256 GEMM

Adds a weight-by-DMA main loop to the pipelined bf16x6 128x256 split GEMM tile. B-panel data is copied straight from a pre-laid split-tile weight image into LDS with global_load_lds, so it no longer passes through registers. To make the path apply, several weights (Wfc, Wf2, Wfin, sig W1/W2, lW5) now get that image built at load time. The goal is to cut VGPR pressure and VALU store work in the main loop. In exchange it uses more LDS (four weight slots), hand-placed waitcnt/barrier scheduling, and extra weight memory.

```diff
diff --git a/include/linetr_hip.h b/include/linetr_hip.h
--- a/include/linetr_hip.h
+++ b/include/linetr_hip.h
@@ -432,6 +432,11 @@
 } LinetrGemmCase;
 int linetr_debug_gemm_case(LinetrHandle* h, const LinetrGemmCase* c, int32_t* tile_used, void* stream);
 
+#define LINETR_GEMM_LOOP_WDMA 1
+#define LINETR_GEMM_LOOP_REG 2
+int linetr_debug_gemm_loop(LinetrHandle* h, const LinetrGemmCase* c, int32_t loop, int32_t w_plain, int32_t* tile_used,
+                           int32_t* loop_used, void* stream);
+
 int linetr_debug_sig_attention(LinetrHandle* h, int32_t kernel, int32_t layer, const float* d_in, int32_t ld_in,
                                const int32_t* h_cu_sub, int32_t n_images, float* d_msg, int32_t* kernel_used, void* stream);
 
diff --git a/linetr_amd/_native.py b/linetr_amd/_native.py
--- a/linetr_amd/_native.py
+++ b/linetr_amd/_native.py
@@ -205,6 +205,7 @@
     "linetr_debug_posenc": (i32, [vp, i32, vp, vp, vp, i64, vp, vp]),
     "linetr_debug_gemm": (i32, [vp, vp, i32, vp, vp, vp, vp, i32, i32, i32, i32, i32, i32, vp]),
     "linetr_debug_gemm_case": (i32, [vp, _P(GemmCase), vp, vp]),
+    "linetr_debug_gemm_loop": (i32, [vp, _P(GemmCase), i32, i32, vp, vp, vp]),
     "linetr_debug_sig_attention": (i32, [vp, i32, i32, vp, i32, vp, i32, vp, vp, vp]),
     "linetr_debug_tok_mlp": (i32, [vp, i32, vp, vp, i64, vp, vp, vp, i64, vp, vp, i32, vp, vp]),
     "linetr_debug_bn_train_workspace_bytes": (i64, [vp, i32, i64]),
diff --git a/linetr_amd/csrc/linetr_core.hip b/linetr_amd/csrc/linetr_core.hip
--- a/linetr_amd/csrc/linetr_core.hip
+++ b/linetr_amd/csrc/linetr_core.hip
@@ -194,7 +194,7 @@
     const float* b = tm.get(pre + "12.bias", D, err);
     if (err) return err;
     if (enc == 0) { W5w = to_d(W, (size_t)D * D); b5w = to_d(b, D); }
-    else place_w(&H->lW5, to_d(W, (size_t)D * D), to_d(b, D), D, e3);
+    else place_w(&H->lW5, to_d(W, (size_t)D * D), to_d(b, D), D, e3, true);
   }
 
   {
@@ -266,10 +266,10 @@
     place_w(&H->Watt, Watt, batt, HEADS * DH, POOLW);
     std::vector<double> bfc2(D);
     for (int i = 0; i < D; ++i) bfc2[i] = (double)bfc[i] + cls[i];
-    place_w(&H->Wfc, to_d(Wfc, D * D), bfc2, D, D);
+    place_w(&H->Wfc, to_d(Wfc, D * D), bfc2, D, D, true);
     place(&H->ln1g, to_d(g1, D)); place(&H->ln1b, to_d(b1, D));
     place_w(&H->Wf1, to_d(W1, (size_t)DI * D), to_d(bb1, DI), DI, D);
-    place_w(&H->Wf2, to_d(W2, (size_t)D * DI), to_d(bb2, D), D, DI);
+    place_w(&H->Wf2, to_d(W2, (size_t)D * DI), to_d(bb2, D), D, DI, true);
     place(&H->ln2g, to_d(g2, D)); place(&H->ln2b, to_d(b2, D));
   }
 
@@ -332,8 +332,8 @@
     sig_qkv_d.push_back(Wqkv); sig_bqkv_d.push_back(bqkv);
     sig_w2_d.push_back(to_d(W2, (size_t)2 * D * D)); sig_b2_d.push_back(to_d(b2, D));
     place_w(&S.Wqkv, Wqkv, bqkv, 3 * D, D, true);
-    place_w(&S.W1, W1m, b1f, 2 * D, 2 * D);
-    place_w(&S.W2, to_d(W2, (size_t)2 * D * D), to_d(b2, D), D, 2 * D);
+    place_w(&S.W1, W1m, b1f, 2 * D, 2 * D, true);
+    place_w(&S.W2, to_d(W2, (size_t)2 * D * D), to_d(b2, D), D, 2 * D, true);
   }
   for (int l = 0; l + 1 < cfg->n_sig_layers; ++l) {
     const std::vector<double>&W2 = sig_w2_d[l], &b2 = sig_b2_d[l], &Wq = sig_qkv_d[l + 1], &bq = sig_bqkv_d[l + 1];
@@ -362,7 +362,7 @@
     const float* W = tm.get("final_proj.weight", D * D, err);
     const float* b = tm.get("final_proj.bias", D, err);
     if (err) return err;
-    place_w(&H->Wfin, to_d(W, D * D), to_d(b, D), D, D);
+    place_w(&H->Wfin, to_d(W, D * D), to_d(b, D), D, D, true);
     if (cfg->n_sig_layers > 0) {
       const std::string p = "selfattn.layers." + std::to_string(cfg->n_sig_layers - 1) + ".";
       const float* W2 = tm.get(p + "mlp.3.weight", 2 * D * D, err);
@@ -380,7 +380,7 @@
         for (int m = 0; m < D; ++m) bacc += (double)W[o * D + m] * (double)b2[m];
         bf[o] = bacc;
       }
-      place_w(&H->Wfin2, Wf, bf, D, 3 * D);
+      place_w(&H->Wfin2, Wf, bf, D, 3 * D, true);
     }
   }
 
diff --git a/linetr_amd/csrc/linetr_net.hip b/linetr_amd/csrc/linetr_net.hip
--- a/linetr_amd/csrc/linetr_net.hip
+++ b/linetr_amd/csrc/linetr_net.hip
@@ -82,7 +82,7 @@
   return gemm_ws_able(h, g, w, groups, fused_norm) && gemm_ws_fits(g.M, g.N, g.K, g.lda, g.ldy, g.act) && !LT_XENV("LINETR_NO_GEMM_WS");
 }
 
-struct GemmForce { int tile = -1; int* used = nullptr; bool launch = true; };
+struct GemmForce { int tile = -1; int* used = nullptr; bool launch = true; int loop = 0; int* loop_used = nullptr; };
 
 int run_gemm(LinetrHandle* h, hipStream_t st, const GemmW& w, int M, const GemmA& A, const GemmY& Y, int act, const float* R = nullptr,
              const GemmGroups* grp = nullptr, const NormSpec* fused_norm = nullptr, const GemmForce* force = nullptr) {
@@ -127,13 +127,22 @@
   if (forced >= 0) tile = (SplitTile)forced;
   else if (int e = pick_split_tile(g, groups, pl, tile)) return e;
   if (int e = split_tile_launched(g, groups, pl, tile)) return e;
+  const int loop = force ? force->loop : 0;
+  if (loop == LINETR_GEMM_LOOP_WDMA && !split_wdma_able(pl, groups, w.st, tile))
+    return fail(LINETR_E_ARG, "gemm: the weight-by-DMA loop runs the bf16x6 128x256 tile of one group on a weight with a split-tile image "
+                "(tile %s, %d groups, image %s)", tile_name(tile), groups, w.st ? "present" : "absent");
+  const bool wdma = loop == LINETR_GEMM_LOOP_WDMA || (loop == 0 && split_wdma(g, pl, groups, w.st, tile));
   report((int)tile);
+  if (force && force->loop_used) *force->loop_used = wdma ? LINETR_GEMM_LOOP_WDMA : LINETR_GEMM_LOOP_REG;
   if (!launch) return LINETR_OK;
   ProfScope ps(h, st, gemm_class_name(h->precision, (int)tile, g, groups), fl, by);
   switch (h->precision) {
     case LINETR_PREC_BF16X3: sa.Wsp = w.s2; sa.gWsp = g.gW * 4; return gemm_split_launch<2>(sa, groups, tile, st);
     case LINETR_PREC_F16X3: sa.Wsp = w.h2; sa.gWsp = g.gW * 4; return gemm_split_launch<2, 1>(sa, groups, tile, st);
-    default: sa.Wsp = w.s3; sa.gWsp = g.gW * 6; return gemm_split_launch<3>(sa, groups, tile, st);
+    default:
+      sa.Wsp = w.s3; sa.gWsp = g.gW * 6;
+      if (wdma) { sa.Wst = w.st; sa.st_rb = (int)st_row_blocks(w.rows); }
+      return gemm_split_launch<3>(sa, groups, tile, st, wdma);
   }
 }
 
@@ -1043,8 +1052,10 @@
   return e;
 }
 
-extern "C" int linetr_debug_gemm_case(LinetrHandle* h, const LinetrGemmCase* c, int32_t* tile_used, void* stream) {
+namespace {
+int debug_gemm_case(LinetrHandle* h, const LinetrGemmCase* c, int32_t* tile_used, void* stream, int loop, bool w_plain, int32_t* loop_used) {
   if (!h || !c) return fail(LINETR_E_ARG, "debug_gemm_case: null argument");
+  if (loop < 0 || loop > LINETR_GEMM_LOOP_REG) return fail(LINETR_E_ARG, "debug_gemm_case: loop must be 0 .. 2");
   const bool query = !c->A && !c->W && !c->Y;
   const int M = c->M, N = c->N, K = c->K, groups = c->groups;
   if (M < 0 || N <= 0 || K <= 0 || groups < 1) return fail(LINETR_E_ARG, "debug_gemm_case: bad shape M=%d N=%d K=%d groups=%d", M, N, K, groups);
@@ -1073,17 +1084,21 @@
     if (al % 16) return fail(LINETR_E_ARG, "debug_gemm_case: tensors must be 16-byte aligned");
   }
   const int64_t rows = (int64_t)N * groups;
-  const bool with_st = groups == 1 && N == WS_N && K == WS_K;
+  const bool with_st = groups == 1 && !w_plain && ((N == WS_N && K == WS_K) || (h->precision == LINETR_PREC_BF16X6 && N % 256 == 0));
   GemmW w;
   w.W = c->W; w.b = c->bias; w.rows = (int)rows; w.K = K;
   const GemmA A{c->A, c->lda, c->A2, c->lda2, c->A2 ? c->K1 : 0};
   const GemmGroups grp{groups, N, c->gA, c->gY};
   const GemmGroups* pg = groups > 1 ? &grp : nullptr;
   GemmForce force;
-  force.tile = c->tile; force.used = tile_used; force.launch = false;
+  int loop_ran = 0;
+  force.tile = c->tile; force.used = tile_used; force.launch = false; force.loop = loop; force.loop_used = &loop_ran;
   const bool fuse = c->norm && !c->via_row_norm && (c->tile >= 0 || gemm_norm_fuses(h, w, M, A, c->R, c->Y));
   if (with_st) w.st = reinterpret_cast<const unsigned char*>(h);
   if (int e = run_gemm(h, nullptr, w, M, A, {c->Y, c->ldy}, c->act, c->R, pg, fuse ? &ns : nullptr, &force)) return e;
+  if (loop == LINETR_GEMM_LOOP_WDMA && loop_ran != LINETR_GEMM_LOOP_WDMA)
+    return fail(LINETR_E_ARG, "debug_gemm_case: the weight-by-DMA loop belongs to the bf16x6 128x256 tile");
+  if (loop_used) *loop_used = loop_ran;
   if (query || M == 0) return LINETR_OK;
   LT_HIP(hipSetDevice(h->device));
   hipStream_t st = (hipStream_t)stream;
@@ -1109,6 +1124,16 @@
   (void)hipStreamSynchronize(st);
   if (buf) (void)hipFree(buf);
   return e;
+}
+}
+
+extern "C" int linetr_debug_gemm_case(LinetrHandle* h, const LinetrGemmCase* c, int32_t* tile_used, void* stream) {
+  return debug_gemm_case(h, c, tile_used, stream, 0, false, nullptr);
+}
+
+extern "C" int linetr_debug_gemm_loop(LinetrHandle* h, const LinetrGemmCase* c, int32_t loop, int32_t w_plain, int32_t* tile_used,
+                                      int32_t* loop_used, void* stream) {
+  return debug_gemm_case(h, c, tile_used, stream, loop, w_plain != 0, loop_used);
 }
 
 extern "C" int linetr_debug_sig_attention(LinetrHandle* h, int32_t kernel, int32_t layer, const float* d_in, int32_t ld_in,
diff --git a/linetr_amd/csrc/lt_gemm_split.h b/linetr_amd/csrc/lt_gemm_split.h
--- a/linetr_amd/csrc/lt_gemm_split.h
+++ b/linetr_amd/csrc/lt_gemm_split.h
@@ -10,6 +10,12 @@
 
 typedef _Float16 f16x8 __attribute__((ext_vector_type(8)));
 typedef _Float16 f16x2 __attribute__((ext_vector_type(2)));
+
+constexpr int ST_CHUNK = 512;
+constexpr int ST_RB = 3 * ST_CHUNK;
+#define LT_GLDS(gp, lp, off)                                                                                      \
+  __builtin_amdgcn_global_load_lds((const __attribute__((address_space(1))) void*)(gp),                           \
+                                   (__attribute__((address_space(3))) void*)(lp), 16, (off), 0)
 
 template <int PL, int FMT = 0>
 __device__ __forceinline__ void split_pair(float x0, float x1, unsigned (&out)[PL]) {
@@ -67,6 +73,8 @@
   float* sk_ws = nullptr;
   unsigned* sk_flags = nullptr;
   unsigned sk_epoch = 0;
+  const unsigned char* Wst = nullptr;
+  int st_rb = 0;
 };
 
 __device__ __forceinline__ void store16_write_through(float* p, const f32x4& v) {
@@ -96,7 +104,8 @@
   __syncthreads();
 }
 
-template <int BM, int BN, int WM, int WN, int PL, bool DB = true, int FMT = 0, int PFD = 1, bool PIPE = false, bool SKT = false>
+template <int BM, int BN, int WM, int WN, int PL, bool DB = true, int FMT = 0, int PFD = 1, bool PIPE = false, bool SKT = false,
+          bool WDMA = false>
 __global__ __launch_bounds__(WM * WN * 64) void gemm_split_kernel(SplitGemmArgs sa) {
   const GemmArgs& g = sa.g;
   constexpr int NT = WM * WN * 64;
@@ -111,6 +120,11 @@
   constexpr int NBUF = DB ? 2 : 1;
   unsigned char* As = smem_s;
   unsigned char* Bs = smem_s + NBUF * BM * RS;
+  static_assert(!WDMA || (DB && PIPE && !SKT && PL == 3 && FMT == 0 && PFD == 2 && BN % 128 == 0 && (BN / 16 * 3) % (2 * WM * WN) == 0 &&
+                          (NBUF * BM * RS) % 1024 == 0),
+                "the weight-by-DMA loop is built for the pipelined bf16x6 tiles whose panel is whole 1 KiB spans per wave");
+  constexpr int W_SLOT = BN / 16 * ST_RB;
+  constexpr int W_DMA = W_SLOT / 1024 / (WM * WN);
 
   const int tid = threadIdx.x, lane = tid & 63, wave = tid >> 6;
   const int wm = wave / WN, wn = wave % WN;
@@ -151,11 +165,13 @@
       r = r < g.M ? r : g.M - 1;
       ra[i] = *reinterpret_cast<const f32x4*>(src + (int64_t)r * ld + kk + lc4);
     }
+    if constexpr (!WDMA) {
 #pragma unroll
     for (int i = 0; i < B_PCS; ++i) {
       int r, pc;
       stage_piece(i, r, pc);
       rb[i] = *reinterpret_cast<const f32x4*>(Wsp + ((int64_t)(n0 + r) * nkw + kbase + kt) * (PL * 64) + pc * 16);
+    }
     }
   };
   auto lstore_set = [&](int buf, const f32x4 (&ra)[A_F4], const f32x4 (&rb)[B_PCS]) {
@@ -168,19 +184,29 @@
 #pragma unroll
       for (int p = 0; p < PL; ++p) *reinterpret_cast<u32x2*>(dst + p * 64) = u32x2{a[p], b[p]};
     }
+    if constexpr (!WDMA) {
 #pragma unroll
     for (int i = 0; i < B_PCS; ++i) {
       int r, pc;
       stage_piece(i, r, pc);
       *reinterpret_cast<f32x4*>(Bs + (buf * BN + r) * RS + pc * 16) = rb[i];
     }
+    }
   };
   auto gload = [&](int kt) { gload_set(kt, ra_[0], rb_[0]); };
   auto lstore = [&](int buf) { lstore_set(buf, ra_[0], rb_[0]); };
+  auto step_wdma = [&](int e, int kt, int buf) {
+    if constexpr (WDMA) {
+      const int s = e / W_DMA, x = __builtin_amdgcn_readfirstlane(wave) + WM * WN * (e % W_DMA);
+      const unsigned char* src = sa.Wst + ((int64_t)(2 * (kbase + kt) + s) * sa.st_rb + n0 / 16) * ST_RB + x * 1024 + lane * 16;
+      LT_GLDS(src, Bs + (2 * buf + s) * W_SLOT + x * 1024, 0);
+    }
+  };
 
   f32x16 acc[MI][NI];
 
   const int frow = lane & 31, fk = (lane >> 5) * 16;
+  const int wfrag = ((lane >> 4) & 1) * ST_RB + (lane >> 5) * 256 + (lane & 15) * 16;
   auto read_frags = [&](int buf, int s, bf16x8 (&af)[MI][PL], bf16x8 (&bf)[NI][PL]) {
     const unsigned char* Ab = As + (buf * BM + wm * TM + frow) * RS + fk + s * 32;
     const unsigned char* Bb = Bs + (buf * BN + wn * TN + frow) * RS + fk + s * 32;
@@ -219,17 +245,30 @@
     for (int j = 0; j < NI; ++j)
 #pragma unroll
       for (int r = 0; r < 16; ++r) acc[i][j][r] = 0.f;
+  if constexpr (WDMA) {
+#pragma unroll
+    for (int e = 0; e < 2 * W_DMA; ++e) step_wdma(e, 0, 0);
+#pragma unroll
+    for (int e = 0; e < 2 * W_DMA; ++e) step_wdma(e, nk > 1 ? 1 : 0, 1);
+  }
   gload(0);
   lstore(0);
   if constexpr (PFD == 1 || PIPE) {
     if (nk > 1) gload_set(1, ra_[PFD - 1], rb_[PFD - 1]);
     if constexpr (PIPE && PFD == 2) gload_set(nk > 2 ? 2 : nk - 1, ra_[0], rb_[0]);
+    if constexpr (WDMA) {
+      if (nk > 1) asm volatile("s_waitcnt vmcnt(%0)" :: "n"(2 * A_F4) : "memory");
+      else asm volatile("s_waitcnt vmcnt(%0)" :: "n"(A_F4) : "memory");
+      asm volatile("s_waitcnt lgkmcnt(0)" ::: "memory");
+      __builtin_amdgcn_s_barrier();
+      asm volatile("" ::: "memory");
+    } else
     __syncthreads();
     if constexpr (DB && PIPE) {
       bf16x8 af0[MI][PL], bf0[NI][PL], af1[MI][PL], bf1[NI][PL];
       constexpr int N_MMA = MI * NI * Terms::N;
       constexpr int N_FRAG = (MI + NI) * PL;
-      constexpr int E1 = 2 * A_F4 + B_PCS;
+      constexpr int E1 = 2 * A_F4 + (WDMA ? 0 : B_PCS);
 #define FRAG_ORDER(k) (((k) / (MI + NI)) == 0 ? (((k) % (MI + NI)) < MI ? ((k) % (MI + NI)) * PL + (PL - 1) : MI * PL + (((k) % (MI + NI)) - MI) * PL) \
                      : ((k) / (MI + NI)) == PL - 1 ? (((k) % (MI + NI)) < MI ? ((k) % (MI + NI)) * PL : MI * PL + (((k) % (MI + NI)) - MI) * PL + (PL - 1)) \
                      : (((k) % (MI + NI)) < MI ? ((k) % (MI + NI)) * PL + 1 : MI * PL + (((k) % (MI + NI)) - MI) * PL + 1))
@@ -241,6 +280,10 @@
         const unsigned char* Ab = As + (buf * BM + wm * TM + frow) * RS + fk + s * 32;
         const unsigned char* Bb = Bs + (buf * BN + wn * TN + frow) * RS + fk + s * 32;
         if (k < MI * PL) { const int i = k / PL, pp = k % PL; af[i][pp] = *reinterpret_cast<const bf16x8*>(Ab + i * 32 * RS + pp * 64); }
+        else if constexpr (WDMA) {
+          const int q = k - MI * PL, j = q / PL, pp = q % PL;
+          bf[j][pp] = *reinterpret_cast<const bf16x8*>(Bs + (2 * buf + s) * W_SLOT + (wn * (TN / 16) + 2 * j) * ST_RB + wfrag + pp * ST_CHUNK);
+        }
         else { const int q = k - MI * PL, j = q / PL, pp = q % PL; bf[j][pp] = *reinterpret_cast<const bf16x8*>(Bb + j * 32 * RS + pp * 64); }
       };
       auto step_gload = [&](int u, int kt, f32x4 (&ra)[A_F4], f32x4 (&rb)[B_PCS]) {
@@ -273,6 +316,8 @@
       };
       constexpr int R_SPAN = N_MMA > N_FRAG ? N_MMA : N_FRAG;
       constexpr int S_SPAN = N_MMA;
+      constexpr int WD_A0 = N_MMA - 4 * A_F4 - 1;
+      static_assert(!WDMA || (4 * W_DMA <= N_MMA && WD_A0 >= 1 && B_PCS >= 2 * W_DMA), "WDMA slots");
       auto first_half = [&](int kt, f32x4 (&ra)[A_F4], f32x4 (&rb)[B_PCS]) {
         const int buf = kt & 1;
         const int ktn = kt + 1 + PFD < nk ? kt + 1 + PFD : nk - 1;
@@ -284,7 +329,7 @@
             if (k * R_SPAN / N_FRAG == m) step_read(FRAG_ORDER(k), buf, 1, af1, bf1);
 #pragma unroll
           for (int e = 0; e < E1; ++e)
-            if ((2 * e + 1) * S_SPAN / (2 * E1) == m) {
+            if ((WDMA ? WD_A0 + 2 * e : (2 * e + 1) * S_SPAN / (2 * E1)) == m) {
               if (e < 2 * A_F4) { if (e % 2 == 0) step_store(e / 2, buf ^ 1, ra, rb); else step_gload(e / 2, ktn, ra, rb); }
               else step_store(A_F4 + (e - 2 * A_F4), buf ^ 1, ra, rb);
             }
@@ -294,6 +339,7 @@
       auto second_half = [&](int kt, f32x4 (&ra)[A_F4], f32x4 (&rb)[B_PCS]) {
         const int buf = kt & 1;
         const int ktn = kt + 1 + PFD < nk ? kt + 1 + PFD : nk - 1;
+        const int ktd = kt + 2 < nk ? kt + 2 : nk - 1;
 #pragma unroll
         for (int m = 0; m < N_MMA; ++m) {
           step_mma(m, af1, bf1);
@@ -302,12 +348,23 @@
             if (k * R_SPAN / N_FRAG == m) step_read(FRAG_ORDER(k), buf ^ 1, 0, af0, bf0);
 #pragma unroll
           for (int e = 0; e < B_PCS; ++e)
-            if ((2 * e + 1) * N_MMA / (2 * B_PCS) == m) step_gload(A_F4 + e, ktn, ra, rb);
+            if ((WDMA ? 2 * e + 1 : (2 * e + 1) * N_MMA / (2 * B_PCS)) == m) {
+              if constexpr (WDMA) { if (e < 2 * W_DMA) step_wdma(e, ktd, buf); }
+              else step_gload(A_F4 + e, ktn, ra, rb);
+            }
           __builtin_amdgcn_sched_barrier(0);
         }
       };
 #pragma unroll
       for (int k = 0; k < N_FRAG; ++k) step_read(FRAG_ORDER(k), 0, 0, af0, bf0);
+      auto tile_barrier = [&]() {
+        if constexpr (WDMA) {
+          asm volatile("s_waitcnt vmcnt(%0)" :: "n"(A_F4) : "memory");
+          asm volatile("s_waitcnt lgkmcnt(0)" ::: "memory");
+          __builtin_amdgcn_s_barrier();
+          asm volatile("" ::: "memory");
+        } else __syncthreads();
+      };
       if constexpr (PFD == 1) {
         for (int kt = 0; kt < nk; ++kt) {
           first_half(kt, ra_[0], rb_[0]);
@@ -318,16 +375,17 @@
       } else {
         for (int kt = 0; kt < nk; kt += 2) {
           first_half(kt, ra_[1], rb_[1]);
-          __syncthreads();
+          tile_barrier();
           __builtin_amdgcn_sched_barrier(0);
           second_half(kt, ra_[1], rb_[1]);
           if (kt + 1 < nk) {
             first_half(kt + 1, ra_[0], rb_[0]);
-            __syncthreads();
+            tile_barrier();
             __builtin_amdgcn_sched_barrier(0);
             second_half(kt + 1, ra_[0], rb_[0]);
           }
         }
+        if constexpr (WDMA) asm volatile("s_waitcnt vmcnt(0)" ::: "memory");
       }
     } else
     for (int kt = 0; kt < nk; ++kt) {
@@ -556,15 +614,19 @@
   static bool wide_epi(const GemmArgs& g) { return g.ldy % 4 == 0 && (!g.R || g.ldr % 4 == 0) && epi_fits; }
 };
 
-template <int BM, int BN, int WM, int WN, int PL, bool DB = true, int FMT = 0, int PFD = 1, bool PIPE = false>
+template <int BM, int BN, int WM, int WN, int PL, bool DB = true, int FMT = 0, int PFD = 1, bool PIPE = false, bool WDMA = false>
 inline int gemm_split_launch_t(const SplitGemmArgs& sa, int groups, hipStream_t st) {
   using Lds = SplitTileLds<BM, BN, PL, DB>;
+  constexpr size_t wdma_main = (size_t)2 * BM * (PL * 64 + 16) + (size_t)4 * (BN / 16) * ST_RB;
+  constexpr size_t lds = !WDMA ? Lds::bytes : (Lds::epi_fits && Lds::epi > wdma_main) ? Lds::epi : wdma_main;
+  if (WDMA && (groups != 1 || !sa.Wst || sa.st_rb < sa.g.N / 16))
+    return fail(LINETR_E_ARG, "gemm_split: the weight-by-DMA loop needs one group and the weight's split-tile image: dispatcher bug");
   SplitGemmArgs sa2 = sa;
   sa2.wide_epi = Lds::wide_epi(sa.g);
   sa2.sk_first = sa2.sk_blocks = 0;
-  LT_HIP((allow_dynamic_lds<gemm_split_kernel<BM, BN, WM, WN, PL, DB, FMT, PFD, PIPE>>((int)Lds::bytes)));
+  LT_HIP((allow_dynamic_lds<gemm_split_kernel<BM, BN, WM, WN, PL, DB, FMT, PFD, PIPE, false, WDMA>>((int)lds)));
   dim3 grid((sa.g.N / BN) * cdiv(sa.g.M, BM), groups);
-  hipLaunchKernelGGL((gemm_split_kernel<BM, BN, WM, WN, PL, DB, FMT, PFD, PIPE>), grid, dim3(WM * WN * 64), Lds::bytes, st, sa2);
+  hipLaunchKernelGGL((gemm_split_kernel<BM, BN, WM, WN, PL, DB, FMT, PFD, PIPE, false, WDMA>), grid, dim3(WM * WN * 64), lds, st, sa2);
   return 0;
 }
 
@@ -597,6 +659,14 @@
   return SplitTile::t128x128;
 }
 
+inline bool split_wdma_able(int pl, int groups, const unsigned char* wst, SplitTile tile) {
+  return pl == 3 && groups == 1 && wst != nullptr && tile == SplitTile::t128x256;
+}
+inline bool split_wdma(const GemmArgs& g, int pl, int groups, const unsigned char* wst, SplitTile tile) {
+  (void)g;
+  return split_wdma_able(pl, groups, wst, tile);
+}
+
 inline int pick_split_tile(const GemmArgs& g, int groups, int pl, SplitTile& tile) {
   static const char* forced = LT_XENV("LINETR_GEMM_TILE");
   if (!forced) { tile = split_tile(g, groups, pl); return 0; }
@@ -627,17 +697,24 @@
 }
 
 template <int PL, int FMT = 0>
-inline int gemm_split_launch(const SplitGemmArgs& sa, int groups, SplitTile tile, hipStream_t st) {
+inline int gemm_split_launch(const SplitGemmArgs& sa, int groups, SplitTile tile, hipStream_t st, bool wdma = false) {
   const GemmArgs& g = sa.g;
   if (g.M <= 0) return 0;
   if (int e = split_tile_launched(g, groups, PL, tile)) return e;
+  if (wdma && !split_wdma_able(PL, groups, sa.Wst, tile))
+    return fail(LINETR_E_ARG, "gemm_split: the weight-by-DMA loop asked of tile %s: dispatcher bug", tile_name(tile));
   int e = 0;
   switch (tile) {
     case SplitTile::t32x32k4: gemm_split_small_launch<PL, FMT>(sa, groups, st); break;
     case SplitTile::t112x256: e = gemm_split16_launch<PL, FMT>(sa, st); break;
     case SplitTile::t128x64: e = gemm_split_launch_t<128, 64, 4, 1, PL, true, FMT>(sa, groups, st); break;
     case SplitTile::t256x128: e = gemm_split_launch_t<256, 128, 4, 2, PL, true, FMT, 1, true>(sa, groups, st); break;
-    case SplitTile::t128x256: e = gemm_split_launch_t<128, 256, 2, 4, PL, true, FMT, PL == 3 ? 2 : 1, true>(sa, groups, st); break;
+    case SplitTile::t128x256:
+      if constexpr (PL == 3 && FMT == 0) {
+        if (wdma) { e = gemm_split_launch_t<128, 256, 2, 4, 3, true, 0, 2, true, true>(sa, groups, st); break; }
+      }
+      e = gemm_split_launch_t<128, 256, 2, 4, PL, true, FMT, PL == 3 ? 2 : 1, true>(sa, groups, st);
+      break;
     case SplitTile::t64x256: e = gemm_split_launch_t<64, 256, 1, 4, PL, true, FMT, PL == 3 ? 2 : 1, true>(sa, groups, st); break;
     case SplitTile::t128x128: e = gemm_split_launch_t<128, 128, 2, 2, PL, true, FMT>(sa, groups, st); break;
     case SplitTile::t128x128s: e = gemm_split_launch_t<128, 128, 2, 4, PL, false, FMT>(sa, groups, st); break;
diff --git a/linetr_amd/csrc/lt_st_image.h b/linetr_amd/csrc/lt_st_image.h
--- a/linetr_amd/csrc/lt_st_image.h
+++ b/linetr_amd/csrc/lt_st_image.h
@@ -5,8 +5,6 @@
 
 namespace lt {
 
-constexpr int ST_CHUNK = 512;
-constexpr int ST_RB = 3 * ST_CHUNK;
 inline __host__ __device__ int64_t st_row_blocks(int64_t rows) { return (rows + 127) / 128 * 8; }
 inline int64_t st_bytes(int64_t rows, int K) { return st_row_blocks(rows) * (int64_t)(K / 16) * ST_RB; }
 
@@ -69,10 +67,6 @@
   *reinterpret_cast<f32x4*>(dst + 4) = f32x4{v[4], v[5], v[6], v[7]};
 }
 
-#define LT_GLDS(gp, lp, off)                                                                                      \
-  __builtin_amdgcn_global_load_lds((const __attribute__((address_space(1))) void*)(gp),                           \
-                                   (__attribute__((address_space(3))) void*)(lp), 16, (off), 0)
-
 __device__ __forceinline__ void swap32(float& a, float& b) {
   unsigned x = __builtin_bit_cast(unsigned, a), y = __builtin_bit_cast(unsigned, b);
   asm volatile("s_nop 1\n\tv_permlane32_swap_b32 %0, %1\n\ts_nop 1" : "+v"(x), "+v"(y));
diff --git a/linetr_amd/engine_debug.py b/linetr_amd/engine_debug.py
--- a/linetr_amd/engine_debug.py
+++ b/linetr_amd/engine_debug.py
@@ -40,6 +40,17 @@
     GEMM_WS = "ws64x256"
     _GEMM_TILE_WS = 100
 
+    GEMM_LOOPS = (None, "dma", "reg")
+
+    def _gemm_tile_request(self, tile):
+        if not isinstance(tile, str) or "+" not in tile:
+            return self._gemm_tile_code(tile), 0, False, False
+        name, *opts = tile.split("+")
+        if any(o not in ("dma", "reg", "plain", "auto") for o in opts) or sum(o in opts for o in ("dma", "reg", "auto")) > 1:
+            raise ValueError(f"no GEMM tile request {tile!r}")
+        loop = 1 if "dma" in opts else 2 if "reg" in opts else 0
+        return self._gemm_tile_code(-1 if name == "-1" else name), loop, "plain" in opts, True
+
     def _gemm_tile_code(self, tile):
         if tile is None or tile == -1:
             return -1
@@ -64,6 +75,16 @@
         used = C.c_int32(-1)
         nat.check(self._L.linetr_debug_gemm_case(self._h, C.byref(c), C.byref(used), None), self._L)
         return self._gemm_tile_name(used.value)
+
+    def gemm_loop(self, M, N, K, *, groups=1, residual=False, concat=False, norm=0, tile=-1):
+        flag = C.c_void_p(16)
+        code, loop, plain, _ = self._gemm_tile_request(tile)
+        c = nat.GemmCase(A=None, lda=int(K), A2=flag if concat else None, lda2=int(K), K1=32 if concat else 0, W=None, bias=None,
+                         R=flag if residual else None, Y=None, ldy=int(N), M=int(M), N=int(N), K=int(K), act=0, groups=int(groups), gA=0,
+                         gY=0, norm=int(norm), gamma=None, beta=None, add2=None, eps=0.0, via_row_norm=0, tile=code)
+        ran = C.c_int32(0)
+        nat.check(self._L.linetr_debug_gemm_loop(self._h, C.byref(c), loop, int(plain), None, C.byref(ran), None), self._L)
+        return self.GEMM_LOOPS[ran.value]
 
     def debug_gemm_case(self, A, W, bias=None, residual=None, act=0, *, A2=None, groups=1, gA=0, gY=None, norm=0, gamma=None,
                         beta=None, add2=None, eps=0.0, via_row_norm=False, tile=-1, out=None):
@@ -103,13 +124,20 @@
         b, ga, be = vec(bias, groups * N, "bias"), vec(gamma, N, "gamma"), vec(beta, N, "beta")
         if add2 is not None and (extent(add2, M, N, 0, "add2").stride(0) != D or N != D):
             raise ValueError("add2 must have row stride 256")
+        code, loop, plain, asked = self._gemm_tile_request(tile)
         c = nat.GemmCase(A=ptr(A), lda=A.stride(0), A2=ptr(A2), lda2=A2.stride(0) if A2 is not None else 0, K1=K1 if A2 is not None else 0,
                          W=ptr(W), bias=ptr(b), R=ptr(residual), Y=ptr(out), ldy=out.stride(0), M=M, N=N, K=K, act=int(act),
                          groups=int(groups), gA=int(gA), gY=gY, norm=int(norm), gamma=ptr(ga), beta=ptr(be), add2=ptr(add2),
-                         eps=float(eps), via_row_norm=int(bool(via_row_norm)), tile=self._gemm_tile_code(tile))
-        used = C.c_int32(-1)
-        self._call("linetr_debug_gemm_case", C.byref(c), C.byref(used))
-        return (full if groups > 1 or full is out else out), self._gemm_tile_name(used.value)
+                         eps=float(eps), via_row_norm=int(bool(via_row_norm)), tile=code)
+        used = C.c_int32(-1)
+        if asked:
+            ran = C.c_int32(0)
+            self._call("linetr_debug_gemm_loop", C.byref(c), loop, int(plain), C.byref(used), C.byref(ran))
+            name = self._gemm_tile_name(used.value) + (f"+{self.GEMM_LOOPS[ran.value]}" if ran.value else "")
+        else:
+            self._call("linetr_debug_gemm_case", C.byref(c), C.byref(used))
+            name = self._gemm_tile_name(used.value)
+        return (full if groups > 1 or full is out else out), name
 
     SIG_KERNELS = ("sig_attn", "sig_attn_small", "sig_attn_split4", "sig_attn_split8", "sig_qkv_attn")
 
```

After: 10.94 million line-descriptors/s (median of 6 runs). 1.02x the previous value.
